# leonavery/KSFD

Measured on AMD Instinct MI355X. Metric: grid-point-updates/sec (implicit step), higher is better.
Workload: dtype f64

## Files before the change

ksfd_amd/csrc/handle.hip.h:

```cpp
#pragma once
#include "spectral_plan.h"
enum { KC_RHS = 0, KC_JVP, KC_MULTIDOT, KC_GSUPDATE, KC_LINCOMB, KC_BASISAXPY, KC_FINISH, KC_REDUCE,
       KC_GFIELD, KC_VELOCITY, KC_MISC, KC_HALO, KC_MG, KC_SPECTRAL };
static const char *kc_names[KSFD_NKCLASS] = { "rhs", "jvp", "multidot", "gs_update", "lincomb", "basis_axpy",
                                              "rosw_finish", "reduce", "gfield", "velocity", "misc", "halo", "mg", "spectral" };
extern "C" const char *ksfd_kernel_class_name(int32_t c) { return (c >= 0 && c < KSFD_NKCLASS) ? kc_names[c] : "?"; }

static thread_local std::string g_create_error;

struct EvPair { hipEvent_t a, b; int cls; };

template <typename T>
struct MGVecs { T *x = nullptr, *b = nullptr, *r = nullptr, *d = nullptr; };

struct MGLevel {
    KGeom G;
    KPhys P;
    KVec kv;
    int64_t vlen = 0;
    int nblk = 1;
    double *coef = nullptr;
    float *dinv = nullptr;
    MGVecs<double> v64;
    MGVecs<float> v32;
    template <typename T> MGVecs<T> &vecs() { if constexpr (std::is_same<T, float>::value) return v32; else return v64; }
    double *Ad = nullptr, *dG = nullptr;
    float *coef32 = nullptr;
    bool f32 = false;
    bool rep = false;
    double *pv = nullptr;
    double pv_norm = 0.0;
    double lam_max = 2.3;
    double ratio = 60.0;
};

struct SpecState {
    bool ok = false, means_valid = false;
    SpecShape shape;
    kcf *W = nullptr, *W2 = nullptr, *twx = nullptr, *twy = nullptr, *twz = nullptr;
    int *spos = nullptr, *skof = nullptr;
    int2 *ytab = nullptr;
    int4 *pairtab = nullptr;
    float *lx = nullptr, *ly = nullptr, *lz = nullptr;
    decltype(&k_spec_rows_fwd<double>) k_rows_fwd64 = nullptr;
    decltype(&k_spec_rows_fwd<float>) k_rows_fwd32 = nullptr;
    decltype(&k_spec_rows_inv) k_rows_inv = nullptr;
    decltype(&k_spec_cols<0>) k_cols = nullptr;
    decltype(&k_spec_cols_split<false>) k_cols_split = nullptr;
    decltype(&k_spec3_y_fwd<false>) k_y_fwd = nullptr;
    decltype(&k_spec3_y_inv<false>) k_y_inv = nullptr;
    decltype(&k_spec3_z<0, false>) k_z = nullptr;
    std::vector<A2APiece> a2a_fwd_s, a2a_fwd_r, a2a_back_s, a2a_back_r;
    double a_rr = 0.0, a_rU[KSFD_MAXL] = { 0 };
    bool user_off = false;
};

struct LUState {
    int64_t n = 0, nnz = 0;
    double *A = nullptr;
    int *piv = nullptr, *perm = nullptr, *info = nullptr;
    long long *col = nullptr;
    double *val = nullptr;
    double *y = nullptr, *z = nullptr;
    std::vector<int> piv_h, perm_h;
    bool valid = false;
    double shift = 0.0;
};

struct MGCoarse {
    int kind = 0;
    int max_unknowns = 0;
    int level = -1;
    LUState lu;
    double *inv = nullptr;
    bool ready = false;
    int info_h = 0;
    int32_t factorizations = 0, solves = 0, fallbacks = 0;
    int32_t graph_solves = 0;
};

struct BandState {
    BandPlan B = {};
    int64_t nnz = 0;
    double *AB = nullptr;
    int *piv = nullptr, *info = nullptr;
    long long *col = nullptr;
    double *val = nullptr;
    double *z = nullptr;
    int threads = 0;
    bool valid = false;
    double shift = 0.0;
};

struct ksfd_handle {
    ksfd_config cfg;
    int32_t lig_group[KSFD_MAXL];
    double lig_w[KSFD_MAXL], lig_s[KSFD_MAXL], lig_gamma[KSFD_MAXL], lig_D[KSFD_MAXL];
    double grp_alpha[KSFD_MAXL], grp_beta[KSFD_MAXL];
    KGeom G;
    KPhys P;
    KPhys Pst[4];
    bool Pst_valid[4] = { false, false, false, false };
    KVec kv;
    int rank = 0, size = 1, device = 0;
    bool ring = false;
    int64_t slow0 = 0;
    hipStream_t st = nullptr;
    hipStream_t st_comm = nullptr;
    hipEvent_t ev_ready = nullptr, ev_halo = nullptr;
    bool overlap = true;
    Transport *tr = nullptr;
    std::string err;

    int64_t vlen = 0;
    double *u = nullptr, *usave = nullptr, *Z = nullptr, *bvec = nullptr, *Y = nullptr, *V = nullptr;
    double *t1 = nullptr, *t2 = nullptr, *t3 = nullptr, *errv = nullptr;
    double *ckpt = nullptr;
    double *bstore = nullptr;
    bool spec_guess = true;
    int guess_max = getenv("KSFD_GUESS_MAX") ? std::max(1, std::min(atoi(getenv("KSFD_GUESS_MAX")), 3)) : 2;
    bool spec_predict = true;
    long long n_predicted = 0;
    long long n_residual = 0;
    long long n_host_sync = 0;
    SpecState spec;
    ksfd_ctl::StepMemo memo, ckpt_memo;
    double spec_from = 0.1;
    bool ckpt_valid = false;
    double *Gb = nullptr, *dGb = nullptr;
    double *coef = nullptr;
    bool use_frozen = true;
    bool coef_fresh = false;
    double *flat = nullptr;
    double *src[4][KSFD_MAXL + 1];
    double *part = nullptr;
    double *dres = nullptr;
    double *hres = nullptr;
    double *hres_dev = nullptr;
    unsigned long long *pub_flag = nullptr, *pub_flag_dev = nullptr, pub_seq = 0;
    unsigned int *pub_count = nullptr;
    bool zero_copy = true;
    int restart_alloc = 0;
    bool restart_grow = true;
    int nblk_vec = 0;
    bool have_err = false;

    int use_fused = 1;
    int yseg = 48;
    int yseg_jvp = 16;
    int zseg = 32;

    bool profiling = false;
    int prof_only = -1;
    std::vector<EvPair> pending;
    std::vector<hipEvent_t> pool;
    ksfd_profile prof;
    double bytes_acc = 0.0;

    double *gm_dev = nullptr;
    double *gm_host = nullptr;
    std::vector<hipEvent_t> gm_ev;
    int async_mode = 0;

    double *Zb = nullptr;
    double *pvec = nullptr;
    int poly_deg = 0;
    double poly_alpha[8];
    double poly_shift = -1.0;
    int poly_max_deg = 6;
    double mg_threshold = 75.0;
    double poly_target = 0.02;
    float *coef32 = nullptr;
    bool rhs_carry = true;
    bool fuse_stage = true;
    bool j3l_attr_set = false, j3l_usable = false;
    bool rhs3d_strip = true;
    bool poly_fp32 = true;

    hipStream_t st_io = nullptr;
    double *snap_dev[2] = { nullptr, nullptr }, *snap_host[2] = { nullptr, nullptr };
    hipEvent_t snap_ready[2] = { nullptr, nullptr }, snap_done[2] = { nullptr, nullptr };
    bool snap_busy[2] = { false, false };
    int snap_next = 0;

    struct RecSpace { bool valid = false; int vb = 0, zb = 0, k = 0, pc = 0; std::vector<double> H; };
    RecSpace rec[4];
    int rec_vtop = 0, rec_ztop = 0;
    int rec_mode = 1;
    int rec_keep = 3;
    bool rhs_dots = true;
    bool rec_mg = false;

    int dr_keep = 0;
    bool dr_carry = false;
    double *dr_P = nullptr, *dr_Phost = nullptr;
    struct DrKept { bool valid = false; int kk = 0, pc = -1; double shift = 0.0, shift_pc = 0.0; std::vector<double> H; };
    DrKept dr;
    ksfd_deflation_stats dr_stats = {};

    LUState lu;
    BandState band;
    MGCoarse mgc;

    std::vector<MGLevel> mg;
    bool sf_auto = true;
    bool mg_fp32 = true;
    bool mg_use32 = false;
    bool mg_graph_f32 = false;
    bool mg_warm_power = true;
    bool mg_fuse = true;
    bool mg_ok = false;
    double mg_shift = -1.0;
    bool mg_coef_valid = false;
    int64_t mg_agg = 0;
    hipGraphExec_t mg_graph = nullptr;
    double mg_graph_shift = -1.0, mg_graph_bytes = 0.0;
    const void *mg_graph_x = nullptr;
    bool capturing = false, mg_use_graph = true;
    int mg_nu = 2, mg_ncoarse = 400, mg_power_its = 8;
    double mg_ratio = 6.0, mg_coarse_tol = 0.3;

    double At[4][4], Ginv[4][4], bt[4], b2t[4], asum[4];
};

#define GAMMA_RA 4.3586652150845900e-01

static int fail(ksfd_handle *h, int code, const char *fmt, ...)
{
    char buf[512];
    va_list ap;
    va_start(ap, fmt);
    vsnprintf(buf, sizeof buf, fmt, ap);
    va_end(ap);
    if (h) h->err = buf; else g_create_error = buf;
    return code;
}
#define HIPCHK(h, call)                                                                                   \
    do {                                                                                                  \
        hipError_t e_ = (call);                                                                           \
        if (e_ != hipSuccess) return fail(h, KSFD_EHIP, "%s failed: %s (%s:%d)", #call, hipGetErrorString(e_), __FILE__, __LINE__); \
    } while (0)

static hipEvent_t ev_get(ksfd_handle *h)
{
    if (!h->pool.empty()) { hipEvent_t e = h->pool.back(); h->pool.pop_back(); return e; }
    hipEvent_t e;
    hipEventCreate(&e);
    return e;
}
struct Scope {
    ksfd_handle *h; EvPair p; bool on;
    Scope(ksfd_handle *h_, int cls, double bytes, double alg = -1.0) : h(h_), on(h_->profiling && !h_->capturing && (h_->prof_only < 0 || h_->prof_only == cls))
    {
        h->bytes_acc += bytes;
        h->prof.bytes[cls] += bytes;
        h->prof.alg_bytes[cls] += alg < 0.0 ? bytes : alg;
        h->prof.launches[cls] += 1;
        if (on) { p.a = ev_get(h); p.b = ev_get(h); p.cls = cls; hipEventRecord(p.a, h->st); }
    }
    ~Scope() { if (on) { hipEventRecord(p.b, h->st); h->pending.push_back(p); } }
};
static void prof_resolve(ksfd_handle *h)
{
    if (h->pending.empty()) return;
    hipStreamSynchronize(h->st);
    for (auto &p : h->pending) {
        float ms = 0.f;
        if (hipEventElapsedTime(&ms, p.a, p.b) == hipSuccess) h->prof.ms[p.cls] += ms;
        h->pool.push_back(p.a);
        h->pool.push_back(p.b);
    }
    h->pending.clear();
}

static inline dim3 vgrid(const ksfd_handle *h) { return dim3(h->nblk_vec, h->G.F); }
static inline double vbytes(const ksfd_handle *h, double nvec) { return nvec * 8.0 * (double)h->G.F * (double)h->G.nloc; }

static void build_tableau(ksfd_handle *h)
{
    static const double A[4][4] = { { 0, 0, 0, 0 }, { 8.7173304301691801e-01, 0, 0, 0 },
                                    { 8.4457060015369423e-01, -1.1299064236484185e-01, 0, 0 }, { 0, 0, 1., 0 } };
    static const double Gm[4][4] = { { GAMMA_RA, 0, 0, 0 }, { -8.7173304301691801e-01, GAMMA_RA, 0, 0 },
                                     { -9.0338057013044082e-01, 5.4180672388095326e-02, GAMMA_RA, 0 },
                                     { 2.4212380706095346e-01, -1.2232505839045147e+00, 5.4526025533510214e-01, GAMMA_RA } };
    static const double b[4] = { 2.4212380706095346e-01, -1.2232505839045147e+00, 1.5452602553351020e+00, GAMMA_RA };
// ... 61 lines not shown
```

ksfd_amd/csrc/krylov.hip.h:

```cpp
#pragma once
#include "krylov_small.h"
static int est_lambda_max(ksfd_handle *h, double shift, int nits)
{
    int rc;
    if (!h->pvec) {
        if (alloc_d(h, &h->pvec, h->vlen)) return KSFD_ENOMEM;
        const int nb = blocks_for(h->vlen);
        hipLaunchKernelGGL(k_hash_fill, dim3(nb), dim3(KSFD_BLOCK), 0, h->st, (long long)h->vlen, h->pvec);
        if ((rc = op_multidot(h, h->pvec, h->pvec, 0))) return rc;
        const double n0 = sqrt(h->hres[0]);
        const double *xs[1] = { h->pvec }; double a[1] = { 1.0 / n0 };
        if ((rc = op_lincomb(h, 1, xs, a, h->pvec))) return rc;
    }
    double lamA = 0.0;
    for (int it = 0; it < nits; it++) {
        if ((rc = op_jvp_frozen_halo(h, h->pvec, 1, shift, h->t3))) return rc;
        if ((rc = op_multidot(h, h->t3, h->t3, 0))) return rc;
        lamA = sqrt(h->hres[0]);
        if (!(lamA > 0.0) || lamA != lamA) return fail(h, KSFD_ENAN, "power iteration on the Jacobian broke down");
        const double *xs[1] = { h->t3 }; double a[1] = { 1.0 / lamA };
        if ((rc = op_lincomb(h, 1, xs, a, h->pvec))) return rc;
    }
    const double est = lamA - shift;
    h->memo.lamJ = est > 0.0 ? est : 0.0;
    return KSFD_OK;
}

static void poly_setup(ksfd_handle *h, double shift)
{
    h->poly_shift = shift;
    h->poly_deg = ksfd_krylov::cheb_setup(h->memo.lamJ, shift, h->poly_target, h->poly_max_deg, h->poly_alpha);
}

static int poly_apply(ksfd_handle *h, double shift, double *v, double *z)
{
    int rc;
    const int d = h->poly_deg;
    const double *al = h->poly_alpha;
    if (h->poly_fp32 && h->coef32 && fused_ok(h)) {
        const float *C = h->coef32;
        float *tf[2] = { reinterpret_cast<float *>(h->t1), reinterpret_cast<float *>(h->t2) };
        const double *nod = nullptr;
        if (d == 1) return jvp2d_halo_t<float, double, double, double>(h, C, v, 4, shift, z, nod, al[0], al[1] / shift);
        if ((rc = jvp2d_halo_t<float, double, double, float>(h, C, v, 4, shift, tf[0], nod, al[d - 1], al[d] / shift))) return rc;
        int cur32 = 0;
        for (int i = d - 2; i >= 1; i--) {
            if ((rc = jvp2d_halo_t<float, float, double, float>(h, C, tf[cur32], 3, shift, tf[cur32 ^ 1], (const double *)v, al[i], 1.0 / shift))) return rc;
            cur32 ^= 1;
        }
        return jvp2d_halo_t<float, float, double, double>(h, C, tf[cur32], 3, shift, z, (const double *)v, al[0], 1.0 / shift);
    }
    double *tmp[2] = { h->t1, h->t2 };
    double *cur = (d == 1) ? z : tmp[0];
    if ((rc = op_jvp_frozen_halo(h, v, 4, shift, cur, nullptr, al[d - 1], al[d] / shift))) return rc;
    int flip = 1;
    for (int i = d - 2; i >= 0; i--) {
        double *nxt = (i == 0) ? z : tmp[flip];
        if ((rc = op_jvp_frozen_halo(h, cur, 3, shift, nxt, v, al[i], 1.0 / shift))) return rc;
        cur = nxt;
        flip ^= 1;
    }
    return KSFD_OK;
}

struct LinStats { int its; double rel; };

static void rec_reset(ksfd_handle *h)
{
    for (auto &r : h->rec) r.valid = false;
    h->rec_vtop = h->rec_ztop = 0;
}

static int rhs_empty(ksfd_handle *h, double bn, double *x, const char *nan_msg, bool *empty)
{
    *empty = !(bn > 0.0);
    if (!*empty) return KSFD_OK;
    if (bn != bn) return fail(h, KSFD_ENAN, "%s", nan_msg);
    HIPCHK(h, hipMemsetAsync(x, 0, sizeof(double) * (size_t)h->vlen, h->st));
    return KSFD_OK;
}

static int apply_AMinv(ksfd_handle *h, const double *ustate, double shift, double shift_pc, int pcmode, double *vj, double *z, double *w)
{
    int rc;
    if (z) {
        if ((rc = pcmode == 1 ? mg_precond(h, shift_pc, vj, z) : pcmode == 3 ? spec_apply(h, shift, vj, z) : poly_apply(h, shift, vj, z))) return rc;
        return op_jvp_frozen_halo(h, z, 1, shift, w);
    }
    if (h->use_frozen) return op_jvp_frozen_halo(h, vj, 1, shift, w);
    return (rc = halo(h, vj)) ? rc : op_jvp(h, ustate, vj, 1, shift, w);
}

static int cgs2_second_pass(ksfd_handle *h, double *w, const double *V, int k, double *hcol, double *d, double *hn)
{
    int rc;
    if ((rc = op_multidot(h, w, V, k))) return rc;
    double s2 = 0.0;
    for (int i = 0; i < k; i++) { d[i] = h->hres[i]; hcol[i] += d[i]; s2 += d[i] * d[i]; }
    double hn2 = h->hres[k] - s2;
    if (hn2 < 0.0) hn2 = 0.0;
    *hn = sqrt(hn2);
    return op_gs_update(h, w, V, k, d, *hn > 0.0 ? 1.0 / *hn : 0.0);
}

static int cgs2_classic(ksfd_handle *h, double *w, const double *V, int k, double *hcol, double *d, double *hn)
{
    int rc;
    for (int i = 0; i < k; i++) hcol[i] = h->hres[i];
    if ((rc = op_gs_update(h, w, V, k, hcol, 1.0))) return rc;
    return cgs2_second_pass(h, w, V, k, hcol, d, hn);
}

static int cgs2_gram(ksfd_handle *h, double *w, const double *V, int j, double *Gm, int ldg, double *hcol, double *d, double *hn)
{
    int rc;
    const int k = j + 1;
    if ((rc = op_multidot_gram(h, w, V, k))) return rc;
    for (int i = 0; i < k; i++) { d[i] = h->hres[i]; Gm[(size_t)i * ldg + j] = Gm[(size_t)j * ldg + i] = h->hres[k + i]; }
    const double ww = h->hres[2 * k];
    if (!(ww == ww)) return fail(h, KSFD_ENAN, "GMRES: Krylov vector is not finite");
    double hn2;
    if (ksfd_krylov::cgs2_algebraic(Gm, ldg, k, d, ww, hcol, &hn2)) {
        *hn = sqrt(hn2);
        return op_gs_update(h, w, V, k, hcol, 1.0 / *hn);
    }
    if ((rc = op_gs_update(h, w, V, k, hcol, 1.0))) return rc;
    return cgs2_second_pass(h, w, V, k, hcol, d, hn);
}

struct GmresRun {
    int pcmode, stage;
    bool use_pc, use_poly;
    bool rec_on, rec_full;
    double shift_pc;
    int vb, zb;
    double *V, *Zq;
    std::vector<int> spaces;
    std::vector<double> g_first;
    double bn, beta;
    const double *rsrc;
    bool x_set = false;
    bool x0_pending = false;
    std::vector<double> xcoef;
};

static int rhs_norm(ksfd_handle *h, GmresRun &R, const double *b)
{
    int rc;
    if (R.rec_on && R.stage > 0)
        for (int q = 0; q < R.stage; q++)
            if (ksfd_krylov::recycle_uses(R.stage, q, h->rec_mode, R.rec_full) && h->rec[q].valid && h->rec[q].pc == R.pcmode) R.spaces.push_back(q);
    if (R.spaces.empty()) {
        if ((rc = op_multidot(h, b, R.V, 0))) return rc;
        R.bn = sqrt(h->hres[0]);
        return KSFD_OK;
    }
    const ksfd_handle::RecSpace &S = h->rec[R.spaces.front()];
    if ((rc = op_multidot(h, b, h->V + (int64_t)S.vb * h->vlen, S.k + 1))) return rc;
    R.g_first.assign(h->hres, h->hres + S.k + 2);
    R.bn = sqrt(R.g_first[S.k + 1]);
    return KSFD_OK;
}

static int recycle_project(ksfd_handle *h, GmresRun &R, const double *b, double *x)
{
    if (R.spaces.empty()) return KSFD_OK;
    int rc;
    const int64_t vs = h->vlen;
    const bool defer_x0 = !R.use_pc;
    bool pc_x0_pending = false;
    double *const rbuf = (x == h->t3) ? R.V : h->t3;
    const int first_space = R.spaces.front(), last_space = R.spaces.back();
    bool have_norm = false;
    for (int q : R.spaces) {
        const ksfd_handle::RecSpace &S = h->rec[q];
        const double *Vs = h->V + (int64_t)S.vb * vs;
        const double *Zs = R.use_poly ? h->Zb + (int64_t)S.zb * vs : Vs;
        std::vector<double> gq_((size_t)S.k + 2), yq_((size_t)S.k + 1), Hy_((size_t)S.k + 2), neg_((size_t)S.k + 2);
        double *gq = gq_.data(), *yq = yq_.data(), *Hy = Hy_.data(), *neg = neg_.data();
        if (q == first_space && R.rsrc == b) {
            for (int i = 0; i <= S.k; i++) gq[i] = R.g_first[i];
        } else {
            if ((rc = op_multidot(h, R.rsrc, Vs, S.k + 1))) return rc;
            for (int i = 0; i <= S.k; i++) gq[i] = h->hres[i];
        }
        ksfd_krylov::hess_lsq(S.H.data(), S.k, gq, yq, Hy);
        if (R.use_pc) {
            if ((rc = op_basis_axpy(h, h->t2, Vs, S.k, yq, pc_x0_pending ? 1.0 : 0.0))) return rc;
            pc_x0_pending = true;
        } else if (defer_x0) {
            for (int i = 0; i < S.k; i++) R.xcoef[(R.use_poly ? S.zb : S.vb) + i] += yq[i];
// ... 339 lines not shown
```

ksfd_amd/csrc/ksfd_hip.hip:

```cpp
#include <hip/hip_runtime.h>
#include <dlfcn.h>
#include <math.h>
#include <stdarg.h>
#include <stdio.h>
#include <stdlib.h>
#include <string.h>
#include <string>
#include <vector>

#include "../../include/ksfd_hip.h"
#include "stencil.hip.h"
#include "mg.hip.h"
#include "spectral.hip.h"
#include "lu.hip.h"
#include "banded.hip.h"
#include "transport.h"
#include "step_control.h"
#include "mg_coarse_plan.h"
#include "mg_agglomerate_plan.h"

#include "handle.hip.h"
#include "ops.hip.h"
#include "spectral_host.hip.h"
#include "mg_host.hip.h"
// ... 43 lines not shown
}

extern "C" int ksfd_create(const ksfd_config *cfg, const ksfd_dist *dist, ksfd_handle **out)
{
    if (!cfg || !out) return fail(nullptr, KSFD_EINVAL, "null argument");
    *out = nullptr;
    if (cfg->dim < 1 || cfg->dim > 3) return fail(nullptr, KSFD_EINVAL, "dim must be 1, 2 or 3");
    for (int a = 0; a < cfg->dim; a++)
        if (cfg->n[a] < 5) return fail(nullptr, KSFD_EINVAL, "n[%d]=%lld < 5: the width-2 periodic star needs >= 5 points", a, (long long)cfg->n[a]);
    ksfd_handle *h = new ksfd_handle();
    memset(h->src, 0, sizeof h->src);
    memset(&h->prof, 0, sizeof h->prof);
    h->cfg = *cfg;
    h->cfg.lig_group = nullptr; h->cfg.lig_w = h->cfg.lig_s = h->cfg.lig_gamma = h->cfg.lig_D = nullptr;
    h->cfg.grp_alpha = h->cfg.grp_beta = nullptr;
    int rc = fill_phys(h, cfg);
    if (rc) { g_create_error = h->err; delete h; return rc; }
    h->rank = dist ? dist->rank : 0;
    h->size = dist ? dist->size : 1;
    h->device = dist ? dist->device : 0;
    if (h->size < 1 || h->rank < 0 || h->rank >= h->size) { delete h; return fail(nullptr, KSFD_EINVAL, "bad rank/size"); }
    h->ring = h->size > 1 || (dist && dist->transport != 0);
    int ndev = 0;
    if (hipGetDeviceCount(&ndev) != hipSuccess || ndev < 1) { delete h; return fail(nullptr, KSFD_EHIP, "no HIP device available (libksfd_hip has no CPU path)"); }
    if (h->device < 0 || h->device >= ndev) { delete h; return fail(nullptr, KSFD_EINVAL, "device %d of %d", h->device, ndev); }
#define CFAIL(code, ...) do { int rc_ = fail(nullptr, code, __VA_ARGS__); ksfd_destroy(h); return rc_; } while (0)
    if (hipSetDevice(h->device) != hipSuccess) CFAIL(KSFD_EHIP, "hipSetDevice(%d) failed", h->device);
    if (hipStreamCreateWithFlags(&h->st, hipStreamNonBlocking) != hipSuccess) CFAIL(KSFD_EHIP, "hipStreamCreate failed");
    if (h->ring && (hipStreamCreateWithFlags(&h->st_comm, hipStreamNonBlocking) != hipSuccess ||
                        hipEventCreateWithFlags(&h->ev_ready, hipEventDisableTiming) != hipSuccess ||
                        hipEventCreateWithFlags(&h->ev_halo, hipEventDisableTiming) != hipSuccess)) CFAIL(KSFD_EHIP, "comm stream/event creation failed");

    KGeom &G = h->G;
    G.dim = cfg->dim; G.F = cfg->nlig + 1;
    const int slow = cfg->dim - 1;
    int64_t nglob = cfg->n[slow];
    if (h->size > 1 && (nglob % h->size != 0 || nglob / h->size < 4))
        CFAIL(KSFD_EINVAL, "slab axis extent %lld must be divisible by %d ranks with >= 4 units each", (long long)nglob, h->size);
    int64_t sloc = nglob / h->size;
    h->slow0 = sloc * h->rank;
    G.ng = h->ring ? 2 : 0;
    G.wrap_slow = !h->ring;
    G.nx = cfg->n[0]; G.ny = cfg->dim >= 2 ? cfg->n[1] : 1; G.nz = cfg->dim >= 3 ? cfg->n[2] : 1;
    if (slow == 0) G.nx = sloc; else if (slow == 1) G.ny = sloc; else G.nz = sloc;
    G.inner = slow == 0 ? 1 : (slow == 1 ? G.nx : G.nx * G.ny);
    G.sloc = sloc;
    G.plane = (sloc + 2 * G.ng) * G.inner;
    G.nloc = sloc * G.inner;
    h->kv.plane = G.plane; h->kv.off = (long long)G.ng * G.inner; h->kv.nloc = G.nloc; h->kv.nf = G.F;
    h->vlen = (int64_t)G.F * G.plane;
    h->nblk_vec = (int)std::min<long long>((G.nloc + KSFD_BLOCK - 1) / KSFD_BLOCK, 2048);
    build_tableau(h);

    h->restart_alloc = ksfd_krylov::RESTART_DEFAULT;
    int fit_local = ksfd_krylov::RESTART_DEFAULT;
    {
        size_t mfree = 0, mtotal = 0;
        if (hipMemGetInfo(&mfree, &mtotal) == hipSuccess && mfree > 0) {
            static const int cap = getenv("KSFD_RESTART_MAX") ? ksfd_krylov::restart_cap(atoi(getenv("KSFD_RESTART_MAX"))) : ksfd_krylov::RESTART_MAX;
            fit_local = ksfd_krylov::restart_fit((double)mfree, 8.0 * (double)h->vlen, cap);
        }
    }
    if (alloc_d(h, &h->dres, 128)) CFAIL(KSFD_ENOMEM, "%s", h->err.c_str());
    if (h->ring) {
        std::string terr;
        h->tr = make_transport(dist, G.F, G.inner, terr);
        if (!h->tr) CFAIL(KSFD_ECOMM, "transport %d: %s", dist->transport, terr.c_str());
        double v = -(double)fit_local;
        if (hipMemcpyAsync(h->dres, &v, sizeof v, hipMemcpyHostToDevice, h->st) != hipSuccess || h->tr->allreduce(h->dres, 1, 1, h->st))
            CFAIL(KSFD_ECOMM, "agreeing on the restart length failed: %s", h->tr->error().c_str());
        if (h->tr->result_on_host()) v = h->tr->host_result()[0];
        else if (hipMemcpyAsync(&v, h->dres, sizeof v, hipMemcpyDeviceToHost, h->st) != hipSuccess || hipStreamSynchronize(h->st) != hipSuccess)
            CFAIL(KSFD_EHIP, "reading the agreed restart length failed");
        fit_local = (int)(-v + 0.5);
    }
    if (fit_local != ksfd_krylov::RESTART_DEFAULT) {
        if (fit_local < ksfd_krylov::RESTART_MIN) CFAIL(KSFD_ENOMEM, "grid too large for this device: a vector is %.2f GB, the solver needs ~47 of them (restart length that fits: %d)", 8.0 * (double)h->vlen / 1e9, fit_local);
        h->restart_alloc = fit_local;
    }
    double **vecs[] = { &h->u, &h->usave, &h->Z, &h->bvec, &h->t1, &h->t2, &h->t3, &h->errv };
    for (double **v : vecs) {
        if (alloc_d(h, v, h->vlen)) CFAIL(KSFD_ENOMEM, "%s", h->err.c_str());
        hipMemsetAsync(*v, 0, sizeof(double) * (size_t)h->vlen, h->st);
    }
    if (alloc_d(h, &h->Y, 4 * h->vlen) || alloc_d(h, &h->V, (int64_t)(h->restart_alloc + 1) * h->vlen) ||
        alloc_d(h, &h->Gb, G.plane) || alloc_d(h, &h->dGb, G.plane) || alloc_d(h, &h->coef, (int64_t)(3 + cfg->nlig) * G.plane) ||
        alloc_d(h, &h->flat, (int64_t)std::max(G.F, 3) * G.nloc) ||
        alloc_d(h, &h->part, (int64_t)(2 * KSFD_MAXDOT + 4) * 4096))
        CFAIL(KSFD_ENOMEM, "%s", h->err.c_str());
    if (hipMalloc((void **)&h->Zb, sizeof(double) * (size_t)h->restart_alloc * (size_t)h->vlen) != hipSuccess) { h->Zb = nullptr; hipGetLastError(); }
    hipMemsetAsync(h->Y, 0, sizeof(double) * (size_t)(4 * h->vlen), h->st);
    hipMemsetAsync(h->V, 0, sizeof(double) * (size_t)((h->restart_alloc + 1) * h->vlen), h->st);
    if (hipHostMalloc((void **)&h->hres, sizeof(double) * 128 + 64, hipHostMallocMapped | hipHostMallocCoherent) != hipSuccess) CFAIL(KSFD_ENOMEM, "hipHostMalloc failed");
    h->pub_flag = reinterpret_cast<unsigned long long *>(h->hres + 128);
    *h->pub_flag = 0;
    if (hipHostGetDevicePointer((void **)&h->hres_dev, h->hres, 0) != hipSuccess || hipMalloc((void **)&h->pub_count, sizeof(unsigned int)) != hipSuccess ||
        hipMemset(h->pub_count, 0, sizeof(unsigned int)) != hipSuccess) { h->zero_copy = false; h->hres_dev = nullptr; }
    else h->pub_flag_dev = reinterpret_cast<unsigned long long *>(h->hres_dev + 128);
    {
        const int m = h->restart_alloc;
        const size_t ndev = (size_t)(m + 1) * (m + 1) + (size_t)(m + 1) * m + 2 * m + (m + 1) + KSFD_MAXDOT + 1 + 2 * (m + 1);
        const size_t nhost = 2 * (m + 1) + (size_t)(m + 1) * m + (m + 1);
        if (alloc_d(h, &h->gm_dev, (int64_t)ndev)) CFAIL(KSFD_ENOMEM, "%s", h->err.c_str());
        if (hipHostMalloc((void **)&h->gm_host, sizeof(double) * nhost, hipHostMallocDefault) != hipSuccess) CFAIL(KSFD_ENOMEM, "hipHostMalloc failed");
        h->gm_ev.resize(m + 1);
        for (auto &e : h->gm_ev) if (hipEventCreateWithFlags(&e, hipEventDisableTiming) != hipSuccess) CFAIL(KSFD_EHIP, "hipEventCreate failed");
    }

    spec_build(h);
    if (mg_build(h)) { mg_free(h); h->mg_ok = false; }
    if ((h->spec.ok || h->mg_ok) && alloc_d(h, &h->bstore, 3 * h->vlen)) { h->bstore = nullptr; h->spec_guess = false; h->err.clear(); }
    if (h->ring) {
        double flags[3] = { h->spec.ok ? 1.0 : 0.0, h->mg_ok ? 1.0 : 0.0, (h->spec_guess && h->bstore) ? 1.0 : 0.0 };
        for (double &f : flags) f = -f;
        if (hipMemcpyAsync(h->dres, flags, sizeof flags, hipMemcpyHostToDevice, h->st) != hipSuccess || h->tr->allreduce(h->dres, 3, 1, h->st))
            CFAIL(KSFD_ECOMM, "agreeing on the available solvers failed: %s", h->tr->error().c_str());
        if (h->tr->result_on_host()) memcpy(flags, h->tr->host_result(), sizeof flags);
        else if (hipMemcpyAsync(flags, h->dres, sizeof flags, hipMemcpyDeviceToHost, h->st) != hipSuccess || hipStreamSynchronize(h->st) != hipSuccess)
            CFAIL(KSFD_EHIP, "reading the agreed solver flags failed");
        if (flags[0] > -0.5 && h->spec.ok) spec_free(h);
        if (flags[1] > -0.5 && h->mg_ok) { mg_free(h); h->mg_ok = false; }
        if (flags[2] > -0.5) h->spec_guess = false;
    }
    if (hipStreamSynchronize(h->st) != hipSuccess) CFAIL(KSFD_EHIP, "stream sync failed in create");
#undef CFAIL
    *out = h;
    return KSFD_OK;
}

extern "C" int ksfd_rccl_unique_id(void *out128)
{
    if (!out128) return KSFD_EINVAL;
    std::string err;
    RcclApi api;
    if (!api.load(err)) return fail(nullptr, KSFD_ECOMM, "%s", err.c_str());
    auto getid = (decltype(&ncclGetUniqueId))dlsym(api.lib, "ncclGetUniqueId");
    if (!getid) return fail(nullptr, KSFD_ECOMM, "librccl lacks ncclGetUniqueId");
    ncclUniqueId id;
    ncclResult_t r = getid(&id);
    if (r != ncclSuccess) return fail(nullptr, KSFD_ECOMM, "ncclGetUniqueId: %s", api.GetErrorString(r));
    memcpy(out128, &id, sizeof id);
    return KSFD_OK;
}

extern "C" int ksfd_update_params(ksfd_handle *h, const ksfd_config *cfg)
{
    if (!h || !cfg) return KSFD_EINVAL;
    if (cfg->dim != h->cfg.dim || cfg->nlig != h->cfg.nlig) return fail(h, KSFD_EINVAL, "update_params cannot change dim/nlig");
    for (int a = 0; a < 3; a++) if (cfg->n[a] != h->cfg.n[a]) return fail(h, KSFD_EINVAL, "update_params cannot change the grid");
    h->cfg = *cfg;
    h->cfg.lig_group = nullptr; h->cfg.lig_w = h->cfg.lig_s = h->cfg.lig_gamma = h->cfg.lig_D = nullptr;
    h->cfg.grp_alpha = h->cfg.grp_beta = nullptr;
    h->coef_fresh = false;
    return fill_phys(h, cfg);
}

extern "C" int ksfd_set_stage_params(ksfd_handle *h, int32_t stage, const ksfd_config *cfg)
{
    if (!h || stage < -1 || stage > 3) return KSFD_EINVAL;
    if (!cfg) {
        for (int s = 0; s < 4; s++) if (stage == -1 || s == stage) h->Pst_valid[s] = false;
        return KSFD_OK;
    }
    if (cfg->dim != h->cfg.dim || cfg->nlig != h->cfg.nlig) return fail(h, KSFD_EINVAL, "set_stage_params cannot change dim/nlig");
    for (int a = 0; a < 3; a++) if (cfg->n[a] != h->cfg.n[a] || cfg->L[a] != h->cfg.L[a]) return fail(h, KSFD_EINVAL, "set_stage_params cannot change the grid");
    for (int s = 0; s < 4; s++) {
        if (stage != -1 && s != stage) continue;
        int rc = fill_phys(h, cfg, &h->Pst[s]);
        if (rc) return rc;
        h->Pst_valid[s] = true;
    }
    return KSFD_OK;
}

extern "C" int ksfd_local_range(const ksfd_handle *h, int64_t *b, int64_t *e)
{
    if (!h) return KSFD_EINVAL;
    if (b) *b = h->slow0;
    if (e) *e = h->slow0 + h->G.sloc;
    return KSFD_OK;
}
extern "C" int64_t ksfd_local_size(const ksfd_handle *h) { return h ? (int64_t)h->G.F * h->G.nloc : 0; }
extern "C" double *ksfd_device_state(ksfd_handle *h) { return h ? h->u : nullptr; }
extern "C" int64_t ksfd_device_plane_stride(const ksfd_handle *h) { return h ? h->G.plane : 0; }
extern "C" int64_t ksfd_device_interior_offset(const ksfd_handle *h) { return h ? (int64_t)h->G.ng * h->G.inner : 0; }

extern "C" int ksfd_set_state(ksfd_handle *h, const double *u, int32_t layout)
{
    if (!h || !u) return KSFD_EINVAL;
    hipSetDevice(h->device);
    int rc = upload(h, u, layout, h->u);
    h->coef_fresh = false;
    if (rc) return rc;
    HIPCHK(h, hipStreamSynchronize(h->st));
    return KSFD_OK;
}
extern "C" int ksfd_snapshot_begin(ksfd_handle *h, int32_t layout, int32_t *slot)
{
    if (!h || !slot) return KSFD_EINVAL;
    if (layout < 0 || layout > 2) return fail(h, KSFD_EINVAL, "bad layout %d", layout);
    hipSetDevice(h->device);
    const KGeom &G = h->G;
    const size_t bytes = sizeof(double) * (size_t)G.F * G.nloc;
    if (!h->st_io) {
        if (hipStreamCreateWithFlags(&h->st_io, hipStreamNonBlocking) != hipSuccess) return fail(h, KSFD_EHIP, "hipStreamCreate (io) failed");
        for (int q = 0; q < 2; q++) {
            if (hipMalloc((void **)&h->snap_dev[q], bytes) != hipSuccess || hipHostMalloc((void **)&h->snap_host[q], bytes, hipHostMallocDefault) != hipSuccess)
                return fail(h, KSFD_ENOMEM, "snapshot staging buffers (%zu bytes each) could not be allocated", bytes);
            if (hipEventCreateWithFlags(&h->snap_ready[q], hipEventDisableTiming) != hipSuccess ||
                hipEventCreateWithFlags(&h->snap_done[q], hipEventDisableTiming) != hipSuccess) return fail(h, KSFD_EHIP, "hipEventCreate failed");
        }
    }
    const int q = h->snap_next;
    h->snap_next ^= 1;
    if (h->snap_busy[q]) HIPCHK(h, hipEventSynchronize(h->snap_done[q]));
    {
        Scope sc(h, KC_MISC, vbytes(h, 2));
        hipLaunchKernelGGL(k_to_host_layout, vgrid(h), dim3(KSFD_BLOCK), 0, h->st, G, layout, (const double *)h->u, G.plane,
                           (long long)G.ng * G.inner, h->snap_dev[q]);
    }
    HIPCHK(h, hipGetLastError());
    HIPCHK(h, hipEventRecord(h->snap_ready[q], h->st));
    HIPCHK(h, hipStreamWaitEvent(h->st_io, h->snap_ready[q], 0));
    HIPCHK(h, hipMemcpyAsync(h->snap_host[q], h->snap_dev[q], bytes, hipMemcpyDeviceToHost, h->st_io));
    HIPCHK(h, hipEventRecord(h->snap_done[q], h->st_io));
    h->snap_busy[q] = true;
    *slot = q;
    return KSFD_OK;
}

extern "C" int ksfd_snapshot_wait(ksfd_handle *h, int32_t slot, const double **host)
{
    if (!h || !host || slot < 0 || slot > 1) return KSFD_EINVAL;
    if (!h->snap_busy[slot]) return fail(h, KSFD_EINVAL, "snapshot slot %d holds nothing", slot);
    hipSetDevice(h->device);
    HIPCHK(h, hipEventSynchronize(h->snap_done[slot]));
    *host = h->snap_host[slot];
    return KSFD_OK;
}

extern "C" int ksfd_checkpoint(ksfd_handle *h, int32_t op)
{
    if (!h || op < 0 || op > 1) return KSFD_EINVAL;
    hipSetDevice(h->device);
    h->dr.valid = false;
    if (op == 0) {
        if (!h->ckpt && alloc_d(h, &h->ckpt, h->vlen)) return KSFD_ENOMEM;
        HIPCHK(h, hipMemcpyAsync(h->ckpt, h->u, sizeof(double) * (size_t)h->vlen, hipMemcpyDeviceToDevice, h->st));
        h->ckpt_memo = h->memo;
        for (MGLevel &L : h->mg) L.pv_norm = 0.0;
        h->ckpt_valid = true;
        return KSFD_OK;
    }
    if (!h->ckpt_valid) return fail(h, KSFD_EINVAL, "no checkpoint has been saved");
    HIPCHK(h, hipMemcpyAsync(h->u, h->ckpt, sizeof(double) * (size_t)h->vlen, hipMemcpyDeviceToDevice, h->st));
    h->coef_fresh = false;
    h->memo = h->ckpt_memo;
    h->spec.means_valid = false;
    h->mg_coef_valid = false; h->mg_shift = -1.0; h->poly_shift = -1.0; h->have_err = false;
    for (MGLevel &L : h->mg) L.pv_norm = 0.0;
    rec_reset(h);
    return KSFD_OK;
}

extern "C" int ksfd_set_state_random(ksfd_handle *h, const int64_t *nc, const double *z, double rho0)
{
    if (!h || !nc || !z) return KSFD_EINVAL;
    hipSetDevice(h->device);
    int64_t n = 1;
    for (int a = 0; a < 3; a++) {
        if (a < h->G.dim ? nc[a] < 1 : nc[a] != 1) return fail(h, KSFD_EINVAL, "coarse grid must be >= 1 per used axis and 1 elsewhere");
        n *= nc[a];
    }
    double *dz = nullptr;
    h->coef_fresh = false;
    if (hipMalloc((void **)&dz, sizeof(double) * (size_t)n) != hipSuccess) return fail(h, KSFD_ENOMEM, "hipMalloc of the coarse samples failed");
    hipError_t e = hipMemcpyAsync(dz, z, sizeof(double) * (size_t)n, hipMemcpyHostToDevice, h->st);
    const KGeom &G = h->G;
    int nb = (int)std::min<long long>((G.nloc + KSFD_BLOCK - 1) / KSFD_BLOCK, 65535);
    if (e == hipSuccess) {
        Scope sc(h, KC_MISC, vbytes(h, 1));
        NL_DISPATCH(h->P.nlig, hipLaunchKernelGGL((k_random_start<NL>), dim3(nb), dim3(KSFD_BLOCK), 0, h->st, G, h->P, (long long)h->cfg.n[G.dim - 1],
                                                  (long long)h->slow0, (long long)nc[0], (long long)nc[1], (long long)nc[2], (const double *)dz, rho0, h->u));
        e = hipGetLastError();
    }
    if (e == hipSuccess) e = hipStreamSynchronize(h->st);
    hipFree(dz);
    if (e != hipSuccess) return fail(h, KSFD_EHIP, "random start: %s", hipGetErrorString(e));
    return KSFD_OK;
}
extern "C" int ksfd_get_state(ksfd_handle *h, double *u, int32_t layout)
{
    if (!h || !u) return KSFD_EINVAL;
    hipSetDevice(h->device);
    return download(h, h->u, layout, u);
}

extern "C" int ksfd_set_source(ksfd_handle *h, int32_t stage, int32_t field, const double *srch, int32_t layout)
{
    if (!h || field < 0 || field >= h->G.F || stage < -1 || stage > 3) return h ? fail(h, KSFD_EINVAL, "bad stage/field") : KSFD_EINVAL;
    if (layout != KSFD_LAYOUT_SOA) return fail(h, KSFD_EINVAL, "sources are single dense planes: pass layout SOA");
    hipSetDevice(h->device);
    for (int s = 0; s < 4; s++) {
        if (stage != -1 && s != stage) continue;
        if (!srch) {
            if (h->src[s][field]) { HIPCHK(h, hipStreamSynchronize(h->st)); hipFree(h->src[s][field]); h->src[s][field] = nullptr; }
            continue;
        }
        if (!h->src[s][field] && alloc_d(h, &h->src[s][field], h->G.nloc)) return KSFD_ENOMEM;
        HIPCHK(h, hipMemcpyAsync(h->src[s][field], srch, sizeof(double) * (size_t)h->G.nloc, hipMemcpyHostToDevice, h->st));
    }
    HIPCHK(h, hipStreamSynchronize(h->st));
    return KSFD_OK;
}

extern "C" int ksfd_rhs(ksfd_handle *h, double t, const double *uh, double *outh, int32_t layout)
{
    (void)t;
    if (!h || !outh) return KSFD_EINVAL;
    hipSetDevice(h->device);
    int rc;
    double *uin = h->u;
    if (uh) { if ((rc = upload(h, uh, layout, h->t1))) return rc; uin = h->t1; }
    if ((rc = halo(h, uin))) return rc;
    if ((rc = op_rhs(h, uin, 0, h->t3))) return rc;
    return download(h, h->t3, layout, outh);
}

extern "C" int ksfd_jvp(ksfd_handle *h, const double *uh, const double *vh, double *outh, int32_t layout)
{
    if (!h || !vh || !outh) return KSFD_EINVAL;
    hipSetDevice(h->device);
    int rc;
    double *uin = h->u;
    if (uh) { if ((rc = upload(h, uh, layout, h->t1))) return rc; uin = h->t1; }
    if ((rc = upload(h, vh, layout, h->t2))) return rc;
    if ((rc = halo(h, uin)) || (rc = halo(h, h->t2))) return rc;
    if (!uh && h->use_frozen) {
        if ((rc = ensure_coef(h, true))) return rc;
        if ((rc = op_jvp_frozen(h, h->t2, 0, 0.0, h->t3))) return rc;
    } else if ((rc = op_jvp(h, uin, h->t2, 0, 0.0, h->t3))) return rc;
    return download(h, h->t3, layout, outh);
}

static int velocity_common(ksfd_handle *h, const double *uin, double *vel_dev, double vmax[3])
{
    const KGeom &G = h->G;
    int rc;
    const double *Gplane = h->Gb;
    if (uin == h->u && h->use_frozen) {
        if ((rc = ensure_coef(h))) return rc;
        Gplane = h->coef + G.plane;
    } else {
        if ((rc = halo(h, (double *)uin))) return rc;
        Scope sc(h, KC_GFIELD, 8.0 * (G.F + 1) * (double)G.plane);
        NL_DISPATCH(h->P.nlig, hipLaunchKernelGGL((k_gfield<NL, false>), dim3(plane_blocks(G)), dim3(KSFD_BLOCK), 0, h->st, G, h->P, uin, (const double *)nullptr, h->Gb, (double *)nullptr));
    }
    int nb = (int)std::min<long long>((G.nloc + KSFD_BLOCK - 1) / KSFD_BLOCK, 1024);
    if (vmax && !vel_dev && G.dim == 2 && (G.nx % 2 == 0) && G.nx >= 4) {
        const int bx = (int)((G.nx / 2 + KSFD_BLOCK - 1) / KSFD_BLOCK), by = (int)std::min<long long>(G.sloc, std::max(1, 2048 / bx));
        nb = bx * by;
        Scope sc(h, KC_VELOCITY, 8.0 * (double)G.nloc);
        hipLaunchKernelGGL(k_velmax2d, dim3(bx, by), dim3(KSFD_BLOCK), 0, h->st, G, h->P, Gplane, h->part);
    } else if (vmax && !vel_dev && G.dim == 3 && (G.nx % 2 == 0) && G.nx >= 4 && G.ny >= 4 && G.nx * G.ny < (1LL << 30)) {
        const int bx = (int)((G.nx / 2 * G.ny + KSFD_BLOCK - 1) / KSFD_BLOCK);
        int zseg = (int)G.sloc;
        while (zseg >= 32 && (long long)bx * ((G.sloc + zseg - 1) / zseg) < 8192) zseg = (zseg + 1) / 2;
        const int by = (int)((G.sloc + zseg - 1) / zseg);
        nb = bx * by;
        if (3LL * nb > part_capacity()) return fail(h, KSFD_EINVAL, "velocity_max: grid too large for the partial-result buffer");
        Scope sc(h, KC_VELOCITY, 8.0 * (double)G.nloc);
        hipLaunchKernelGGL(k_velmax3d, dim3(bx, by), dim3(KSFD_BLOCK), 0, h->st, G, h->P, zseg, Gplane, h->part);
    } else {
        Scope sc(h, KC_VELOCITY, 8.0 * (double)G.nloc * (1 + (vel_dev ? G.dim : 0)));
        hipLaunchKernelGGL(k_velocity, dim3(nb), dim3(KSFD_BLOCK), 0, h->st, G, h->P, Gplane, vel_dev, vmax ? h->part : (double *)nullptr);
    }
    HIPCHK(h, hipGetLastError());
    if (vmax) {
        if ((rc = reduce_rows(h, 3, nb, 1))) return rc;
        for (int a = 0; a < 3; a++) vmax[a] = a < G.dim ? h->hres[a] : 0.0;
    }
    return KSFD_OK;
}

extern "C" int ksfd_velocity(ksfd_handle *h, const double *uh, double *velh, int32_t layout)
{
    if (!h || !velh) return KSFD_EINVAL;
    if (layout != KSFD_LAYOUT_SOA) return fail(h, KSFD_EINVAL, "velocity output is dim dense SoA planes: pass layout SOA for it");
    hipSetDevice(h->device);
    int rc;
    double *uin = h->u;
    if (uh) { if ((rc = upload(h, uh, layout, h->t1))) return rc; uin = h->t1; }
    if ((rc = velocity_common(h, uin, h->flat, nullptr))) return rc;
    HIPCHK(h, hipMemcpyAsync(velh, h->flat, sizeof(double) * (size_t)h->G.dim * h->G.nloc, hipMemcpyDeviceToHost, h->st));
    HIPCHK(h, hipStreamSynchronize(h->st));
    return KSFD_OK;
}

extern "C" int ksfd_velocity_max(ksfd_handle *h, double vmax[3])
{
    if (!h || !vmax) return KSFD_EINVAL;
    hipSetDevice(h->device);
    return velocity_common(h, h->u, nullptr, vmax);
}

extern "C" int ksfd_groom(ksfd_handle *h)
{
    if (!h) return KSFD_EINVAL;
    hipSetDevice(h->device);
    Scope sc(h, KC_MISC, vbytes(h, 2));
    hipLaunchKernelGGL(k_groom, vgrid(h), dim3(KSFD_BLOCK), 0, h->st, h->kv, h->u, h->P.rhomin, h->P.Umin);
    HIPCHK(h, hipGetLastError());
    return KSFD_OK;
}

extern "C" int ksfd_count_worms(ksfd_handle *h, double *total)
{
    if (!h || !total) return KSFD_EINVAL;
    hipSetDevice(h->device);
    {
        Scope sc(h, KC_MISC, 8.0 * (double)h->G.nloc);
        hipLaunchKernelGGL(k_sum_rho, dim3(h->nblk_vec), dim3(KSFD_BLOCK), 0, h->st, h->kv, h->u, h->part);
    }
    HIPCHK(h, hipGetLastError());
    int rc = reduce_rows(h, 1, h->nblk_vec, 0);
    if (rc) return rc;
    *total = h->hres[0];
    return KSFD_OK;
}

extern "C" int ksfd_scale_rho(ksfd_handle *h, double factor)
{
    if (!h) return KSFD_EINVAL;
    hipSetDevice(h->device);
    h->coef_fresh = false;
    Scope sc(h, KC_MISC, 16.0 * (double)h->G.nloc);
    hipLaunchKernelGGL(k_mul_rho, dim3(h->nblk_vec), dim3(KSFD_BLOCK), 0, h->st, h->kv, h->u, (const double *)nullptr, factor);
    HIPCHK(h, hipGetLastError());
    return KSFD_OK;
}

extern "C" int ksfd_mul_rho(ksfd_handle *h, const double *fh)
{
    if (!h || !fh) return KSFD_EINVAL;
    hipSetDevice(h->device);
    HIPCHK(h, hipMemcpyAsync(h->flat, fh, sizeof(double) * (size_t)h->G.nloc, hipMemcpyHostToDevice, h->st));
    h->coef_fresh = false;
    Scope sc(h, KC_MISC, 24.0 * (double)h->G.nloc);
    hipLaunchKernelGGL(k_mul_rho, dim3(h->nblk_vec), dim3(KSFD_BLOCK), 0, h->st, h->kv, h->u, (const double *)h->flat, 1.0);
    HIPCHK(h, hipGetLastError());
    HIPCHK(h, hipStreamSynchronize(h->st));
    return KSFD_OK;
}

extern "C" int ksfd_jacobian_nnz(ksfd_handle *h, int64_t *nrows, int64_t *nnz)
{
    if (!h) return KSFD_EINVAL;
    const int64_t npts = 4 * h->G.dim + 1;
    if (nrows) *nrows = (int64_t)h->G.F * h->G.nloc;
    if (nnz) *nnz = h->G.nloc * ((int64_t)h->G.F * npts + (int64_t)h->P.nlig * (npts + 1));
    return KSFD_OK;
}

extern "C" int ksfd_jacobian_csr(ksfd_handle *h, int64_t *rowptr, int64_t *col, double *val)
{
    if (!h || !rowptr || !col || !val) return KSFD_EINVAL;
    hipSetDevice(h->device);
    int64_t nrows, nnz;
    ksfd_jacobian_nnz(h, &nrows, &nnz);
    int rc;
    if ((rc = ensure_coef(h))) return rc;
    long long *dcol = nullptr;
    double *dval = nullptr;
    if (hipMalloc((void **)&dcol, sizeof(long long) * (size_t)nnz) != hipSuccess ||
        hipMalloc((void **)&dval, sizeof(double) * (size_t)nnz) != hipSuccess) {
        if (dcol) hipFree(dcol);
        return fail(h, KSFD_ENOMEM, "hipMalloc of the CSR staging buffers failed");
    }
    const KGeom &G = h->G;
    int nb = (int)std::min<long long>((G.nloc + KSFD_BLOCK - 1) / KSFD_BLOCK, 65535);
    {
        Scope sc(h, KC_MISC, 16.0 * (double)nnz + 8.0 * (3 + h->P.nlig) * (double)G.nloc);
        NL_DISPATCH(h->P.nlig, hipLaunchKernelGGL((k_jac_csr<NL>), dim3(nb), dim3(KSFD_BLOCK), 0, h->st, G, h->P, (const double *)h->coef,
                                                  (long long)h->cfg.n[G.dim - 1], (long long)h->slow0, dcol, dval));
    }
    hipError_t e = hipGetLastError();
    if (e == hipSuccess) e = hipMemcpyAsync(col, dcol, sizeof(long long) * (size_t)nnz, hipMemcpyDeviceToHost, h->st);
    if (e == hipSuccess) e = hipMemcpyAsync(val, dval, sizeof(double) * (size_t)nnz, hipMemcpyDeviceToHost, h->st);
    if (e == hipSuccess) e = hipStreamSynchronize(h->st);
    hipFree(dcol);
    hipFree(dval);
    if (e != hipSuccess) return fail(h, KSFD_EHIP, "jacobian export: %s", hipGetErrorString(e));
    const int64_t npts = 4 * G.dim + 1, F = G.F, per = F * npts + (F - 1) * (npts + 1);
    for (int64_t p = 0; p < G.nloc; p++) {
        rowptr[p * F] = p * per;
        for (int64_t l = 1; l < F; l++) rowptr[p * F + l] = p * per + F * npts + (l - 1) * (npts + 1);
    }
    rowptr[nrows] = nnz;
    return KSFD_OK;
}


extern "C" void ksfd_default_step_opts(ksfd_step_opts *o)
{
    memset(o, 0, sizeof *o);
    o->rtol = 1e-5; o->atol = 1e-5;
    o->adapt = 1; o->max_reject = 10;
    o->clip_lo = 0.1; o->clip_hi = 5.0;
    o->dt_min = 1e-20; o->dt_max = 1e4;
    o->safety = 0.9; o->reject_safety = 0.5;
    o->ksp_rtol = 1e-6; o->ksp_atol = 1e-50;
    o->ksp_restart = 30; o->ksp_max_it = 2000;
    o->pc_type = 2;
}

static int step_run(ksfd_handle *h, double *t, double *hstep, const ksfd_step_opts *opts, bool direct, bool dr_on, ksfd_step_stats &st)
{
    int rc;
    StepMemo &m = h->memo;
    double hh = *hstep;
    bool prev_accept = !(opts->reserved & 4);
    bool lam_done = false;
    int rejects = 0;
    const int max_rej = opts->max_reject < 0 ? 0x7fffffff : opts->max_reject;
    const bool single = (opts->reserved & 2) != 0;
    {
        Scope sc(h, KC_MISC, vbytes(h, 3));
        hipLaunchKernelGGL(k_groom, vgrid(h), dim3(KSFD_BLOCK), 0, h->st, h->kv, h->u, h->P.rhomin, h->P.Umin, h->usave);
        if (hipGetLastError() != hipSuccess) return fail(h, KSFD_EHIP, "k_groom launch failed");
    }
    if ((rc = halo(h, h->u))) return rc;
    if (h->use_frozen && (rc = ensure_coef(h, true))) return rc;
    h->poly_shift = -1.0;
    m.nsteps++;
    ksfd_ctl::spec_rho_roll(m);
    while (true) {
        AttemptPlan p;
        if ((rc = plan_attempt(h, opts, hh, direct, dr_on, lam_done, p))) return rc;
        const int its_before = st.linear_its;
        bool spec_failed = false;
        rc = step_attempt(h, opts, p, spec_failed, st);
        const int its = st.linear_its - its_before;
        if (p.use_spec && opts->pc_type == 2) ksfd_ctl::spec_backoff_update(m, spec_failed, its, m.nsteps);
        if (!rc && p.use_pc && h->sf_auto) ksfd_ctl::shift_floor_update(m, (double)its, p.shift);
        if (rc == KSFD_ELINEAR && opts->adapt && !single && rejects < max_rej && hh * 0.25 >= opts->dt_min) {
            rejects++;
            st.rejections = rejects;
            prev_accept = false;
            if ((rc = op_copy(h, h->u, h->usave))) return rc;
            hh *= 0.25;
            *hstep = hh;
            if ((rc = halo(h, h->u))) return rc;
            continue;
        }
        if (rc) { op_copy(h, h->u, h->usave); hipStreamSynchronize(h->st); return rc; }
        if ((rc = step_finish(h, opts, &st.wrms))) return rc;
        if (!(st.wrms == st.wrms) || isinf(st.wrms)) {
            op_copy(h, h->u, h->usave); hipStreamSynchronize(h->st);
            h->coef_fresh = h->use_frozen;
            return fail(h, KSFD_ENAN, "non-finite error norm at t=%g h=%g", *t, hh);
        }
        ksfd_ctl::AdaptChoice next = { true, hh };
        if (opts->adapt) next = ksfd_ctl::adapt_basic(hh, st.wrms, prev_accept, opts->safety, opts->reject_safety, opts->clip_lo, opts->clip_hi, opts->dt_min, opts->dt_max);
        prev_accept = next.accept;
        if (next.accept) {
            st.accepted = 1; st.h_used = hh;
            *t += hh;
            *hstep = next.hnext;
            return KSFD_OK;
        }
        rejects++;
        st.rejections = rejects;
        if ((rc = op_copy(h, h->u, h->usave))) return rc;
        h->coef_fresh = h->use_frozen;
        hh = next.hnext;
        *hstep = next.hnext;
        if (single) return KSFD_OK;
        if (rejects > max_rej) return fail(h, KSFD_EREJECT, "step rejected %d times at t=%g", rejects, *t);
        if ((rc = halo(h, h->u))) return rc;
    }
}

extern "C" int ksfd_step(ksfd_handle *h, double *t, double *hstep, const ksfd_step_opts *opts, ksfd_step_stats *stats)
{
    if (!h || !t || !hstep || !opts) return KSFD_EINVAL;
    hipSetDevice(h->device);
    const bool direct = opts->pc_type == 5 || opts->pc_type == 6;
    if (direct) {
        const int g = opts->pc_type == 6 ? banded_guard(h) : direct_guard(h);
        if (g) return g;
    }
    const bool dr_on = h->dr_keep > 0 && !direct;
    if (dr_on) {
        const int m_dr = std::min(opts->ksp_restart > 0 ? opts->ksp_restart : 30, h->restart_alloc);
        if (h->dr_keep > m_dr - 3) return fail(h, KSFD_EINVAL, "deflation: keep = %d needs a restart length of at least %d (ksp_restart %d, basis vectors allocated %d)", h->dr_keep, h->dr_keep + 3, (int)opts->ksp_restart, h->restart_alloc);
    }
    memset(&h->dr_stats, 0, sizeof h->dr_stats);
    if (getenv("KSFD_PC_SIGMA")) { h->memo.mg_shift_floor = atof(getenv("KSFD_PC_SIGMA")); h->sf_auto = false; }
    ksfd_step_stats st;
    memset(&st, 0, sizeof st);
    const StepCounters c0 = stats_begin(h);
    const int32_t coarse0 = h->mgc.solves;
    const int rc = step_run(h, t, hstep, opts, direct, dr_on, st);
    stats_end(h, c0, st);
    if (h->mgc.solves != coarse0) st.pc_used |= 64;
    if (stats) *stats = st;
    return rc;
}

extern "C" int ksfd_get_last_error_vector(ksfd_handle *h, double *eh, int32_t layout)
{
    if (!h || !eh) return KSFD_EINVAL;
    if (!h->have_err) return fail(h, KSFD_EINVAL, "no step has been attempted yet");
    hipSetDevice(h->device);
    return download(h, h->errv, layout, eh);
}

extern "C" int ksfd_set_profiling(ksfd_handle *h, int32_t on)
{
    if (!h) return KSFD_EINVAL;
    prof_resolve(h);
    if (on < 0 || on >= 2 + KSFD_NKCLASS) return KSFD_EINVAL;
    h->profiling = on != 0;
    h->prof_only = on >= 2 ? on - 2 : -1;
    return KSFD_OK;
}
extern "C" int ksfd_get_profile(ksfd_handle *h, ksfd_profile *p, int32_t reset)
{
    if (!h || !p) return KSFD_EINVAL;
    prof_resolve(h);
    *p = h->prof;
    if (reset) memset(&h->prof, 0, sizeof h->prof);
    return KSFD_OK;
}
extern "C" int ksfd_set_mg_params(ksfd_handle *h, int32_t nu, int32_t ncoarse_max, int32_t power_its, double ratio, double coarse_tol)
{
    if (!h) return KSFD_EINVAL;
    if (nu > 0) h->mg_nu = nu;
    if (ncoarse_max > 0) h->mg_ncoarse = ncoarse_max;
    if (power_its > 0) h->mg_power_its = power_its;
    if (ratio > 1.0) h->mg_ratio = ratio;
    if (coarse_tol > 0.0) h->mg_coarse_tol = coarse_tol;
    h->mg_use_graph = power_its != -7 && !h->ring;
    h->mg_shift = -1.0;
    return KSFD_OK;
}
static int mg_coarse_choice(const ksfd_handle *h, int32_t kind, int32_t max_unknowns)
{
    std::vector<long long> unk;
    for (const MGLevel &L : h->mg) unk.push_back((long long)L.G.F * L.G.nloc);
    return ksfd_ctl::mg_coarse_level(unk.data(), h->mg_ok ? (int)unk.size() : 0, kind, max_unknowns, KSFD_MG_DIRECT_MAX);
}
extern "C" int ksfd_set_mg_coarse(ksfd_handle *h, int32_t kind, int32_t max_unknowns)
{
    if (!h) return KSFD_EINVAL;
    if (kind != 0 && kind != 1) return fail(h, KSFD_EINVAL, "mg_coarse: kind %d is neither 0 (Chebyshev) nor 1 (exact solve)", (int)kind);
    if (kind == 1) {
        if (h->ring) return fail(h, KSFD_EINVAL, "mg_coarse: the exact coarse solve is single rank only (this handle has a halo transport)");
        if (!h->mg_ok) return fail(h, KSFD_EINVAL, "mg_coarse: this handle has no multigrid hierarchy");
        if (max_unknowns > KSFD_MG_DIRECT_MAX) return fail(h, KSFD_EINVAL, "mg_coarse: max_unknowns = %d above KSFD_MG_DIRECT_MAX = %d", (int)max_unknowns, KSFD_MG_DIRECT_MAX);
    } else if (!h->mg_ok) return KSFD_OK;
    const int level = mg_coarse_choice(h, kind, max_unknowns);
    if (level < 0) {
        const MGLevel &Lc = h->mg.back();
        return fail(h, KSFD_EINVAL, "mg_coarse: no level below level 0 has at most %d unknowns (the coarsest of %d levels has %lld)",
                    max_unknowns > 0 ? (int)max_unknowns : KSFD_MG_DIRECT_MAX, (int)h->mg.size(), (long long)Lc.G.F * Lc.G.nloc);
    }
    hipSetDevice(h->device);
    if (kind == 1) { int rc = mgc_alloc(h, level); if (rc) return rc; }
    if (kind == h->mgc.kind && level == h->mgc.level) { h->mgc.max_unknowns = kind == 1 ? max_unknowns : 0; return KSFD_OK; }
    h->mgc.kind = kind; h->mgc.level = level; h->mgc.max_unknowns = kind == 1 ? max_unknowns : 0;
    h->mgc.ready = false;
    h->mg_shift = -1.0;
    if (h->mg_graph) { HIPCHK(h, hipStreamSynchronize(h->st)); hipGraphExecDestroy(h->mg_graph); h->mg_graph = nullptr; }
    return KSFD_OK;
}
extern "C" int ksfd_set_mg_agglomerate(ksfd_handle *h, int64_t max_points)
{
    if (!h) return KSFD_EINVAL;
    if (max_points < 0) return fail(h, KSFD_EINVAL, "mg_agglomerate: max_points = %lld is negative", (long long)max_points);
    if (!h->ring) return KSFD_OK;
    if (h->G.dim == 1) return fail(h, KSFD_EINVAL, "mg_agglomerate: 2-D and 3-D slabs only (this handle is 1-D)");
    if (!h->mg_ok) return fail(h, KSFD_EINVAL, "mg_agglomerate: this handle has no multigrid hierarchy");
    hipSetDevice(h->device);
    HIPCHK(h, hipStreamSynchronize(h->st));
    const int64_t before = h->mg_agg;
    int own_rc = KSFD_OK;
    std::string own_err;
    bool failed = false;
    auto rebuild = [&](int64_t agg) -> int {
        mg_free(h);
        h->mg_agg = agg;
        h->mg_coef_valid = false; h->mg_shift = -1.0; h->mg_graph_shift = -1.0;
        h->dr.valid = false;
        own_rc = mg_build(h);
        own_err = h->err;
        if (!own_rc && !h->mg_ok) own_rc = fail(h, KSFD_EINVAL, "mg_agglomerate: the rebuilt hierarchy has fewer than two levels"), own_err = h->err;
        double bad = own_rc ? 1.0 : 0.0;
        if (hipMemcpyAsync(h->dres, &bad, sizeof bad, hipMemcpyHostToDevice, h->st) != hipSuccess || h->tr->allreduce(h->dres, 1, 1, h->st))
            return fail(h, KSFD_ECOMM, "mg_agglomerate: agreeing on the hierarchy failed: %s", h->tr->error().c_str());
        if (h->tr->result_on_host()) bad = h->tr->host_result()[0];
        else if (hipMemcpyAsync(&bad, h->dres, sizeof bad, hipMemcpyDeviceToHost, h->st) != hipSuccess || hipStreamSynchronize(h->st) != hipSuccess)
            return fail(h, KSFD_EHIP, "mg_agglomerate: reading the agreed outcome failed");
        HIPCHK(h, hipStreamSynchronize(h->st));
        failed = bad > 0.5;
        return KSFD_OK;
    };
    int rc = rebuild(max_points);
    if (rc || !failed) return rc;
    const int why_rc = own_rc;
    const std::string why = own_err;
    if (rebuild(before) != KSFD_OK || failed) { mg_free(h); h->mg_agg = 0; }
    if (why_rc) { h->err = why; return why_rc; }
    return fail(h, KSFD_ENOMEM, "mg_agglomerate: another rank could not build the hierarchy with max_points = %lld", (long long)max_points);
}
extern "C" int ksfd_get_mg_coarse_info(ksfd_handle *h, ksfd_mg_coarse_info *info)
{
    if (!h || !info) return KSFD_EINVAL;
    memset(info, 0, sizeof *info);
    if (!h->mg_ok) return fail(h, KSFD_EINVAL, "mg_coarse: this handle has no multigrid hierarchy");
    const MGLevel &L = h->mg[mg_end(h)];
    info->kind = h->mgc.kind; info->level = (int32_t)mg_end(h); info->nlevels = (int32_t)h->mg.size(); info->F = L.G.F;
    info->n[0] = L.G.nx; info->n[1] = L.G.dim >= 2 ? L.G.ny : 1; info->n[2] = L.G.dim >= 3 ? L.G.nz : 1;
    info->unknowns = (int64_t)L.G.F * L.G.nloc;
    info->factorizations = h->mgc.factorizations; info->solves = h->mgc.solves; info->fallbacks = h->mgc.fallbacks;
    return KSFD_OK;
}
extern "C" int ksfd_mg_coarse_apply(ksfd_handle *h, double shift, int32_t op, const double *vh, double *outh)
{
    if (!h || !vh || !outh) return KSFD_EINVAL;
    if (!isfinite(shift)) return fail(h, KSFD_EINVAL, "mg_coarse_apply: non-finite shift");
    if (op != 0 && op != 1) return fail(h, KSFD_EINVAL, "mg_coarse_apply: op %d is neither 0 (operator) nor 1 (solve)", (int)op);
    if (!h->mg_ok) return fail(h, KSFD_EINVAL, "mg_coarse: this handle has no multigrid hierarchy");
    if (op == 1 && h->mgc.kind != 1) return fail(h, KSFD_EINVAL, "mg_coarse_apply: op 1 needs ksfd_set_mg_coarse(kind 1)");
    if (h->ring) return fail(h, KSFD_EINVAL, "mg_coarse_apply: single rank only (this handle has a halo transport)");
    hipSetDevice(h->device);
    int rc;
    if ((rc = ensure_coef(h))) return rc;
    if (!h->mg_coef_valid && (rc = mg_restrict_coefs(h))) return rc;
    MGLevel &L = h->mg[mg_end(h)];
    double *const lb = L.v64.b, *const lx = L.v64.x;
    const size_t nb = sizeof(double) * (size_t)L.G.nloc;
    for (int f = 0; f < L.G.F; f++)
        HIPCHK(h, hipMemcpyAsync(lb + (int64_t)f * L.G.plane + L.kv.off, vh + (int64_t)f * L.G.nloc, nb, hipMemcpyHostToDevice, h->st));
    if (op == 0) rc = mg_op<double>(h, L, lb, 1, shift, lx, nullptr);
    else {
        bool ok = false;
        h->mg_shift = -1.0;
        if ((rc = mgc_setup(h, L, shift, &ok))) return rc;
        if (!ok) return fail(h, KSFD_ELINEAR, "coarse solve: zero or non-finite pivot in column %d of shift*I - J_c (shift %.6g, %lld unknowns)", h->mgc.info_h - 1, shift, (long long)h->mgc.lu.n);
        rc = mgc_apply(h, L, lb, lx);
        h->mgc.ready = false;
    }
    if (rc) return rc;
    for (int f = 0; f < L.G.F; f++)
        HIPCHK(h, hipMemcpyAsync(outh + (int64_t)f * L.G.nloc, lx + (int64_t)f * L.G.plane + L.kv.off, nb, hipMemcpyDeviceToHost, h->st));
    HIPCHK(h, hipStreamSynchronize(h->st));
    return KSFD_OK;
}
template <typename T>
static int mgp_put(ksfd_handle *h, const MGLevel &L, int np, const double *host, T *dev)
{
    HIPCHK(h, hipMemsetAsync(dev, 0, sizeof(T) * (size_t)np * L.G.plane, h->st));
    std::vector<T> tmp((size_t)np * L.G.nloc);
    for (size_t i = 0; i < tmp.size(); i++) tmp[i] = (T)host[i];
    for (int f = 0; f < np; f++)
        HIPCHK(h, hipMemcpyAsync(dev + (int64_t)f * L.G.plane + L.kv.off, tmp.data() + (int64_t)f * L.G.nloc, sizeof(T) * (size_t)L.G.nloc, hipMemcpyHostToDevice, h->st));
    HIPCHK(h, hipStreamSynchronize(h->st));
    return KSFD_OK;
}
template <typename T>
static int mgp_get(ksfd_handle *h, const MGLevel &L, int np, const T *dev, double *host)
{
    std::vector<T> tmp((size_t)np * L.G.nloc);
    for (int f = 0; f < np; f++)
        HIPCHK(h, hipMemcpyAsync(tmp.data() + (int64_t)f * L.G.nloc, dev + (int64_t)f * L.G.plane + L.kv.off, sizeof(T) * (size_t)L.G.nloc, hipMemcpyDeviceToHost, h->st));
    HIPCHK(h, hipStreamSynchronize(h->st));
    for (size_t i = 0; i < tmp.size(); i++) host[i] = (double)tmp[i];
    return KSFD_OK;
}
static int mgp_begin(ksfd_handle *h, bool setup, double shift)
{
    int rc;
    if ((rc = ensure_coef(h))) return rc;
    if (!h->mg_coef_valid && (rc = mg_restrict_coefs(h))) return rc;
    if (setup) {
        for (MGLevel &L : h->mg) L.pv_norm = 0.0;
        h->mg_shift = -1.0;
        if ((rc = mg_setup_shift(h, shift))) return rc;
    }
    return KSFD_OK;
}
static void mgp_end(ksfd_handle *h)
{
    hipStreamSynchronize(h->st);
    h->mg_shift = -1.0;
    h->mg_graph_shift = -1.0;
    if (h->mg_graph) { hipGraphExecDestroy(h->mg_graph); h->mg_graph = nullptr; }
    for (MGLevel &L : h->mg) L.pv_norm = 0.0;
    h->mgc.ready = false;
}
static bool mgp_smoothed(const ksfd_handle *h, size_t l) { return l <= mg_end(h) && !(l == mg_end(h) && h->mgc.kind == 1 && h->mgc.ready); }

extern "C" int ksfd_mg_level_info(ksfd_handle *h, int32_t level, int32_t setup, double shift, ksfd_mg_level_info_t *info)
{
    if (!h || !info) return KSFD_EINVAL;
    memset(info, 0, sizeof *info);
    if (!h->mg_ok) return fail(h, KSFD_EINVAL, "mg_part: this handle has no multigrid hierarchy");
    if (level < 0 || level >= (int)h->mg.size()) return fail(h, KSFD_EINVAL, "mg_part: level %d outside 0 .. %d", (int)level, (int)h->mg.size() - 1);
    if (setup && !isfinite(shift)) return fail(h, KSFD_EINVAL, "mg_part: non-finite shift");
    hipSetDevice(h->device);
    const int rc = mgp_begin(h, setup != 0, shift);
    const MGLevel &L = h->mg[level];
    info->level = level; info->nlevels = (int32_t)h->mg.size(); info->F = L.G.F; info->end_level = (int32_t)mg_end(h);
    info->n[0] = L.G.nx; info->n[1] = L.G.dim >= 2 ? L.G.ny : 1; info->n[2] = L.G.dim >= 3 ? L.G.nz : 1;
    info->sloc = L.G.sloc; info->points = L.G.nloc;
    info->path = (int32_t)mg_path(h, L);
    info->f32 = L.f32 ? 1 : 0;
    const JvpSys Y = mg_sys(h, L);
    info->coef32 = (Y.coef32 ? 2 : 0) | ((Y.coef32 && Y.cls == KC_JVP && mg_path(h, L) == JP_STRIP2D) ? 1 : 0);
    info->can_fuse = mg_can_fuse(h, L) ? 1 : 0;
    if (setup && !rc) {
        info->have_setup = mgp_smoothed(h, (size_t)level) ? 1 : 0;
        if (info->have_setup) { info->lam_max = L.lam_max; info->ratio = L.ratio; }
        if ((size_t)level == mg_end(h) && info->have_setup) info->coarse_sweeps = mg_coarse_sweeps(h, L);
    }
    mgp_end(h);
    return rc;
}

extern "C" int ksfd_mg_part(ksfd_handle *h, int32_t part, int32_t level, int32_t variant, int32_t nu, double shift, double ratio,
                            const double *in0, const double *in1, double *out0, double *out1)
{
    if (!h) return KSFD_EINVAL;
    if (!h->mg_ok) return fail(h, KSFD_EINVAL, "mg_part: this handle has no multigrid hierarchy");
    const int nlev = (int)h->mg.size();
    if (level < 0 || level >= nlev) return fail(h, KSFD_EINVAL, "mg_part: level %d outside 0 .. %d", (int)level, nlev - 1);
    if (!isfinite(shift)) return fail(h, KSFD_EINVAL, "mg_part: non-finite shift");
    MGLevel &L = h->mg[level];
    const bool transfer = part == KSFD_MGP_RESTRICT || part == KSFD_MGP_PROLONG_ADD;
    if (transfer && level + 1 >= nlev) return fail(h, KSFD_EINVAL, "mg_part: level %d has no coarser level", (int)level);
    MGLevel &Lc = h->mg[transfer ? level + 1 : level];
    const bool cf32 = transfer && mg_f32(h, (size_t)level + 1);
    const int F = L.G.F, np = 3 + h->P.nlig;
    bool setup = false, ok = true, need1 = false, need_o1 = false;
    switch (part) {
    case KSFD_MGP_COEF: ok = variant == 0; break;
    case KSFD_MGP_RESTRICT: ok = variant == 0 || (variant == 1 && L.f32) || (variant == 2 && L.G.dim == 2 && Lc.f32); break;
    case KSFD_MGP_PROLONG_ADD: ok = variant == 0 || (variant == 1 && L.f32); need1 = true; break;
    case KSFD_MGP_OPERATOR: ok = variant == 1 || variant == 2 || (variant == 32 && L.f32); need1 = variant != 1; break;
    case KSFD_MGP_DINV: ok = variant == 0; setup = true; break;
    case KSFD_MGP_DINV_APPLY: ok = variant == 0 || (variant == 1 && L.f32); setup = true; need_o1 = true; break;
    case KSFD_MGP_SMOOTH: ok = variant == 0; setup = true; break;
    case KSFD_MGP_CYCLE: ok = level == 0 && (variant == 0 || variant == 1); setup = true; break;
    default: return fail(h, KSFD_EINVAL, "mg_part: unknown part %d", (int)part);
    }
    if (!ok) return fail(h, KSFD_EINVAL, "mg_part %d: level %d has no variant %d", (int)part, (int)level, (int)variant);
    if (part == KSFD_MGP_CYCLE && variant == 1 && !mg_cycle32_ok(h))
        return fail(h, KSFD_EINVAL, "mg_part: this handle has no cycle with fp32 level vectors (2-D strip kernel on level 0, nu = 2, fused smoother, tuning bit 19 clear)");
    if (part == KSFD_MGP_SMOOTH && (nu < 1 || nu > 5)) return fail(h, KSFD_EINVAL, "mg_part: nu = %d outside 1 .. 5", (int)nu);
    if (part == KSFD_MGP_SMOOTH && !(ratio > 1.0)) return fail(h, KSFD_EINVAL, "mg_part: smoothing ratio %.6g not above 1", ratio);
    if ((part != KSFD_MGP_COEF && part != KSFD_MGP_DINV && !in0) || (need1 && !in1) || !out0 || (need_o1 && !out1))
        return fail(h, KSFD_EINVAL, "mg_part %d: missing buffer", (int)part);
    if (setup && part != KSFD_MGP_CYCLE && (size_t)level > mg_end(h)) return fail(h, KSFD_EINVAL, "mg_part %d: level %d lies below the level the cycle ends on", (int)part, (int)level);
    hipSetDevice(h->device);
    int rc;
    if ((rc = mgp_begin(h, setup, shift))) { mgp_end(h); return rc; }
    if (setup && part != KSFD_MGP_CYCLE && !mgp_smoothed(h, (size_t)level)) { mgp_end(h); return fail(h, KSFD_EINVAL, "mg_part %d: level %d is solved exactly and has no smoother", (int)part, (int)level); }
    double *const a = L.rep ? L.v64.b : h->t1, *const b = L.rep ? L.v64.x : h->t2, *const c = L.rep ? L.v64.d : h->t3;
    auto run = [&]() -> int {
        int r;
        switch (part) {
        case KSFD_MGP_COEF: {
            if ((r = mgp_get(h, L, np, (const double *)L.coef, out0))) return r;
            const float *c32 = mg_sys(h, L).coef32;
            if (out1 && c32) return mgp_get(h, L, np, c32, out1);
            return KSFD_OK;
        }
        case KSFD_MGP_RESTRICT: {
            auto go = [&](auto *fine, auto *coarse) -> int {
                if ((r = mgp_put(h, L, F, in0, fine)) || (r = mg_halo(h, L, fine, F))) return r;
                if ((r = mg_launch_restrict(h, L, Lc, F, fine, coarse)) || (r = mg_border_reduce(h, L, Lc, F, coarse))) return r;
                return mgp_get(h, Lc, F, coarse, out0);
            };
            if (variant == 0) return Lc.rep ? go(a, Lc.v64.b) : go(a, b);
            if (variant == 2) return go(a, Lc.v32.b);
            return cf32 ? go(L.v32.r, Lc.v32.b) : go(L.v32.r, Lc.v64.b);
        }
        case KSFD_MGP_PROLONG_ADD: {
            auto go = [&](auto *fine, auto *coarse) -> int {
                if ((r = mgp_put(h, L, F, in0, fine)) || (r = mgp_put(h, Lc, F, in1, coarse)) || (r = mg_halo(h, Lc, coarse, F))) return r;
                if ((r = mg_launch_prolong(h, L, Lc, F, coarse, fine))) return r;
                return mgp_get(h, L, F, fine, out0);
            };
            if (variant == 0) return Lc.rep ? go(a, Lc.v64.x) : go(a, b);
            return cf32 ? go(L.v32.x, Lc.v32.x) : go(L.v32.x, Lc.v64.x);
        }
        case KSFD_MGP_OPERATOR: {
            auto go = [&](auto *v, auto *out, auto *y, int mode) -> int {
                if ((r = mgp_put(h, L, F, in0, v)) || (mode == 2 && (r = mgp_put(h, L, F, in1, y)))) return r;
                if ((r = mg_op(h, L, v, mode, shift, out, mode == 2 ? y : nullptr))) return r;
                return mgp_get(h, L, F, out, out0);
            };
            return variant == 32 ? go(L.v32.x, L.v32.r, L.v32.b, 2) : go(a, b, c, variant);
        }
        case KSFD_MGP_DINV: return mgp_get(h, L, F * F, (const float *)L.dinv, out0);
        case KSFD_MGP_DINV_APPLY: {
            const double scale = nu ? (double)nu : 1.0;
            auto go = [&](auto *z, auto *z2, auto *rcopy) -> int {
                if ((r = mgp_put(h, L, F, in0, a))) return r;
                mg_dinv_apply(h, L, 0.0, (const double *)a, 1.0 / scale, z, z2, rcopy);
                if ((r = mgp_get(h, L, F, z, out0)) || (r = mgp_get(h, L, F, z2, out1))) return r;
                return mgp_get(h, L, F, rcopy, out1 + (int64_t)F * L.G.nloc);
            };
            return variant == 0 ? go(b, c, L.Ad) : go(L.v32.d, L.v32.x, L.v32.b);
        }
        case KSFD_MGP_SMOOTH:
            if ((r = mgp_put(h, L, F, in0, a))) return r;
            if (in1) { if ((r = mgp_put(h, L, F, in1, b))) return r; }
            else HIPCHK(h, hipMemsetAsync(b, 0x7f, sizeof(double) * (size_t)L.vlen, h->st));
            if ((r = mg_smooth(h, L, shift, a, b, nu, !in1, ratio))) return r;
            return mgp_get(h, L, F, (const double *)b, out0);
        default: {
            if ((r = mgp_put(h, L, F, in0, a))) return r;
            HIPCHK(h, hipMemsetAsync(b, 0x7f, sizeof(double) * (size_t)L.vlen, h->st));
            const bool was = h->mg_use32;
            h->mg_use32 = variant == 1;
            r = mg_precond(h, shift, a, b);
            h->mg_use32 = was;
            if (r) return r;
            return mgp_get(h, L, F, (const double *)b, out0);
        }
        }
    };
    rc = run();
    if (!rc && hipGetLastError() != hipSuccess) rc = fail(h, KSFD_EHIP, "mg_part %d: launch failed", (int)part);
    mgp_end(h);
// ... 45 lines not shown
}
extern "C" int ksfd_set_deflation(ksfd_handle *h, int32_t keep, int32_t carry_stages)
{
    if (!h) return KSFD_EINVAL;
    if (keep < 0 || keep > 16) return fail(h, KSFD_EINVAL, "deflation: keep = %d outside 0 (off) .. 16", (int)keep);
    h->dr_keep = keep;
    h->dr_carry = carry_stages != 0;
    h->dr.valid = false;
    return KSFD_OK;
}
extern "C" int ksfd_get_deflation_stats(ksfd_handle *h, ksfd_deflation_stats *s)
{
    if (!h || !s) return KSFD_EINVAL;
    *s = h->dr_stats;
    return KSFD_OK;
}
extern "C" int32_t ksfd_basis_capacity(const ksfd_handle *h) { return h ? h->restart_alloc + 1 : 0; }
extern "C" int ksfd_basis_rotate(ksfd_handle *h, int32_t nin, int32_t nout, const double *P, const double *vin, double *vout, int32_t layout)
{
    if (!h || !P || !vin || !vout) return KSFD_EINVAL;
    if (layout < 0 || layout > 2) return fail(h, KSFD_EINVAL, "bad layout %d", layout);
    if (nin < 1 || nout < 1 || nout > nin || nout > KSFD_ROT_MAXOUT || nin > KSFD_ROT_MAXIN || nin > h->restart_alloc + 1)
        return fail(h, KSFD_EINVAL, "basis_rotate: %d -> %d vectors outside 1 <= nout <= %d, nout <= nin <= min(%d, %d)", (int)nin, (int)nout, KSFD_ROT_MAXOUT, KSFD_ROT_MAXIN, h->restart_alloc + 1);
    hipSetDevice(h->device);
    h->dr.valid = false;
    rec_reset(h);
    int rc;
    const int64_t nl = (int64_t)h->G.F * h->G.nloc;
    for (int i = 0; i < nin; i++) {
        if ((rc = upload(h, vin + (int64_t)i * nl, layout, h->V + (int64_t)i * h->vlen))) return rc;
        HIPCHK(h, hipStreamSynchronize(h->st));
    }
    std::vector<double> Pp((size_t)nin * KSFD_ROT_MAXOUT, 0.0);
    for (int i = 0; i < nin; i++) for (int j = 0; j < nout; j++) Pp[(size_t)i * KSFD_ROT_MAXOUT + j] = P[(size_t)i * nout + j];
    if ((rc = op_basis_rotate(h, h->V, nin, nout, Pp.data(), KSFD_ROT_MAXOUT))) return rc;
    for (int i = 0; i < nin; i++)
        if ((rc = download(h, h->V + (int64_t)i * h->vlen, layout, vout + (int64_t)i * nl))) return rc;
    return KSFD_OK;
}
extern "C" int ksfd_krylov_op(ksfd_handle *h, int32_t op, int32_t k, int32_t want_norm, const double *coef, double alpha, double beta,
                              const double *vecs, double *out_vecs, double *scalars, int32_t layout)
{
    if (!h) return KSFD_EINVAL;
    if (layout < 0 || layout > 2) return fail(h, KSFD_EINVAL, "bad layout %d", layout);
    const int cap = h->restart_alloc + 1;
    const int kdev = std::min(KSFD_ASYNC_MAXK, h->restart_alloc);
    int kmin = 1, kmax = 0, nvec = 0, nscal = 0;
    bool need_coef = true;
    switch (op) {
    case KSFD_KOP_LINCOMB: kmax = std::min(6, cap); nvec = k; nscal = want_norm ? 1 : 0; break;
    case KSFD_KOP_MULTIDOT: kmin = 0; kmax = cap - 1; nvec = k + 1; nscal = k + 1; need_coef = false; break;
    case KSFD_KOP_MULTIDOT_GRAM: kmax = std::min(32, cap - 1); nvec = k + 1; nscal = 2 * k + 1; need_coef = false; break;
    case KSFD_KOP_GS_UPDATE: kmax = cap - 1; nvec = k + 1; break;
    case KSFD_KOP_BASIS_AXPY: kmax = cap - 1; nvec = k + 1; nscal = want_norm ? 1 : 0; break;
    case KSFD_KOP_GS_UPDATE_DEV: kmax = kdev; nvec = k + 1; break;
    case KSFD_KOP_GMRES_COEF: kmax = kdev; nvec = 0; nscal = 1; break;
    default: return fail(h, KSFD_EINVAL, "krylov_op: unknown operation %d", (int)op);
    }
    if (k < kmin || k > kmax) return fail(h, KSFD_EINVAL, "krylov_op %d: k = %d outside %d .. %d (basis capacity %d)", (int)op, (int)k, kmin, kmax, cap);
    if ((need_coef && !coef) || (nvec && (!vecs || !out_vecs)) || (nscal && !scalars)) return fail(h, KSFD_EINVAL, "krylov_op %d: missing buffer", (int)op);
    if (want_norm && op != KSFD_KOP_LINCOMB && op != KSFD_KOP_BASIS_AXPY) return fail(h, KSFD_EINVAL, "krylov_op %d has no norm epilogue", (int)op);
    hipSetDevice(h->device);
    h->dr.valid = false;
    rec_reset(h);
    int rc;
    const GmDev D = gm_dev_block(h);
    if (op == KSFD_KOP_GMRES_COEF) {
        const double *row = coef;
        double *so = scalars;
        HIPCHK(h, hipMemsetAsync(D.coef, 0, sizeof(double) * KSFD_MAXDOT, h->st));
        HIPCHK(h, hipMemsetAsync(D.H, 0, sizeof(double) * (size_t)D.ld * k, h->st));
        for (int j = 0; j < k; j++) {
            const int nrow = 2 * (j + 1) + 1;
            HIPCHK(h, hipMemcpyAsync(h->dres, row, sizeof(double) * nrow, hipMemcpyHostToDevice, h->st));
            launch_gmres_coef(h, D, j, beta);
            HIPCHK(h, hipGetLastError());
            HIPCHK(h, hipMemcpyAsync(so, D.coef, sizeof(double) * k, hipMemcpyDeviceToHost, h->st));
            HIPCHK(h, hipMemcpyAsync(so + k, D.scale, sizeof(double), hipMemcpyDeviceToHost, h->st));
            HIPCHK(h, hipMemcpyAsync(so + k + 1, D.mon + 2 * j, 2 * sizeof(double), hipMemcpyDeviceToHost, h->st));
            HIPCHK(h, hipStreamSynchronize(h->st));
            row += nrow; so += k + 3;
        }
        for (int c = 0; c < k; c++) HIPCHK(h, hipMemcpyAsync(so + (size_t)c * (k + 1), D.H + (size_t)D.ld * c, sizeof(double) * (k + 1), hipMemcpyDeviceToHost, h->st));
        HIPCHK(h, hipMemcpyAsync(so + (size_t)k * (k + 1), D.g, sizeof(double) * (k + 1), hipMemcpyDeviceToHost, h->st));
        HIPCHK(h, hipStreamSynchronize(h->st));
        return KSFD_OK;
    }
    const int64_t nl = (int64_t)h->G.F * h->G.nloc, vs = h->vlen;
    for (int i = 0; i < nvec; i++) {
        if ((rc = upload(h, vecs + (int64_t)i * nl, layout, h->V + (int64_t)i * vs))) return rc;
        HIPCHK(h, hipStreamSynchronize(h->st));
    }
    double *const w = h->V + (int64_t)k * vs;
    switch (op) {
    case KSFD_KOP_LINCOMB: {
        const double *xs[6];
        for (int t = 0; t < k; t++) xs[t] = h->V + (int64_t)t * vs;
        rc = op_lincomb(h, k, xs, coef, h->V, want_norm != 0);
    } break;
    case KSFD_KOP_MULTIDOT: rc = op_multidot(h, w, h->V, k); break;
    case KSFD_KOP_MULTIDOT_GRAM: rc = op_multidot_gram(h, w, h->V, k); break;
    case KSFD_KOP_GS_UPDATE: rc = op_gs_update(h, w, h->V, k, coef, alpha); break;
    case KSFD_KOP_BASIS_AXPY: rc = op_basis_axpy(h, w, h->V, k, coef, beta, want_norm != 0); break;
    default: {
        HIPCHK(h, hipMemcpyAsync(D.coef, coef, sizeof(double) * k, hipMemcpyHostToDevice, h->st));
        HIPCHK(h, hipMemcpyAsync(D.scale, &alpha, sizeof(double), hipMemcpyHostToDevice, h->st));
        launch_gs_update_dev(h, w, h->V, k, D.coef, D.scale);
        HIPCHK(h, hipGetLastError());
        HIPCHK(h, hipStreamSynchronize(h->st));
        rc = KSFD_OK;
    } break;
    }
    if (rc) return rc;
    for (int i = 0; i < nscal; i++) scalars[i] = h->hres[i];
    for (int i = 0; i < nvec; i++)
        if ((rc = download(h, h->V + (int64_t)i * vs, layout, out_vecs + (int64_t)i * nl))) return rc;
    return KSFD_OK;
}
extern "C" int ksfd_set_spectral_params(ksfd_handle *h, double from_stiffness, int32_t enable)
{
    if (!h) return KSFD_EINVAL;
    if (from_stiffness > 0.0) h->spec_from = from_stiffness;
    if (enable == 0) h->spec.user_off = true;
    else if (enable > 0) { h->spec.user_off = false; h->memo.spec_bad_until = 0; h->memo.spec_backoff = 8; }
    return KSFD_OK;
}
extern "C" int ksfd_synchronize(ksfd_handle *h)
{
    if (!h) return KSFD_EINVAL;
    hipSetDevice(h->device);
    HIPCHK(h, hipStreamSynchronize(h->st));
    return KSFD_OK;
}
extern "C" int ksfd_set_tuning(ksfd_handle *h, int32_t use_fused, int32_t yseg, int32_t yseg_jvp)
{
    if (!h) return KSFD_EINVAL;
    if (use_fused >= 0) {
        h->use_fused = use_fused & 1; h->use_frozen = !(use_fused & 2); h->overlap = !(use_fused & 4);
        h->async_mode = (use_fused & 8) ? 1 : 0;
        h->rec_mode = (use_fused & 16) ? 0 : ((use_fused & 32) ? 2 : 1);
        if ((use_fused >> 6) & 7) h->rec_keep = std::min((use_fused >> 6) & 7, 4);
        h->poly_fp32 = !(use_fused & 512);
        h->fuse_stage = !(use_fused & 1024);
        h->zero_copy = !(use_fused & 2048) && h->hres_dev;
        h->rhs3d_strip = !(use_fused & 8192);
        h->spec_guess = !(use_fused & 16384);
        h->rhs_carry = !(use_fused & 32768);
        h->spec_predict = !(use_fused & 65536);
        h->restart_grow = !(use_fused & 131072);
        h->mg_warm_power = !(use_fused & 262144);
        h->mg_fp32 = !(use_fused & 524288);
        h->rec_mg = (use_fused & 1048576) != 0;
        h->rhs_dots = !(use_fused & 2097152);
        if (h->mg_fuse != !(use_fused & 4096)) { h->mg_fuse = !(use_fused & 4096); h->mg_shift = -1.0; if (h->mg_graph) { hipGraphExecDestroy(h->mg_graph); h->mg_graph = nullptr; } }
    }
    if (yseg > 0) h->yseg = yseg;
    if (yseg_jvp > 0) h->yseg_jvp = yseg_jvp;
    return KSFD_OK;
}

extern "C" int ksfd_bench_kernel(ksfd_handle *h, int32_t cls, int32_t reps, double *avg_ms, double *bytes_per_launch)
{
    if (!h || reps < 1 || !avg_ms) return KSFD_EINVAL;
    hipSetDevice(h->device);
    hipEvent_t a, b;
    HIPCHK(h, hipEventCreate(&a));
    HIPCHK(h, hipEventCreate(&b));
    const bool was = h->profiling;
    h->profiling = false;
    int rc = KSFD_OK;
    double by = 0.0;
    auto one = [&]() -> int {
        const double b0 = h->bytes_acc;
        int r = KSFD_OK;
        double coef[KSFD_MAXDOT] = { 0 };
        switch (cls) {
        case KC_RHS: r = op_rhs(h, h->u, -1, h->t3); break;
        case KC_JVP: r = h->use_frozen ? op_jvp_frozen(h, h->Y, 1, 1.0, h->t3) : op_jvp(h, h->u, h->Y, 1, 1.0, h->t3); break;
        case KC_MULTIDOT: {
            Scope sc(h, KC_MULTIDOT, vbytes(h, 9));
            VW_DISPATCH(h, hipLaunchKernelGGL((k_multidot<8, VW>), dim3(vec2(h) ? (h->nblk_vec + 1) / 2 : h->nblk_vec), dim3(KSFD_BLOCK), 0, h->st, h->kv, (const double *)h->t3, (const double *)h->V, h->vlen, 8, h->part));
        } break;
        case KC_GSUPDATE: r = op_gs_update(h, h->t3, h->V, 8, coef, 1.0); break;
        case KC_SPECTRAL: r = spec_apply(h, 10.0, h->Y, h->t3); break;
        case KC_LINCOMB: { const double *xs[3] = { h->u, h->Y, h->Y + h->vlen }; double aa[3] = { 1.0, 0.5, 0.25 }; r = op_lincomb(h, 3, xs, aa, h->t3); } break;
        case KSFD_BENCH_ROTATE: {
            std::vector<double> Pb((size_t)31 * KSFD_ROT_MAXOUT, 0.0);
            for (int j = 0; j < 11; j++) Pb[(size_t)j * KSFD_ROT_MAXOUT + j] = 1.0;
            r = op_basis_rotate(h, h->V, 31, 11, Pb.data(), KSFD_ROT_MAXOUT);
        } break;
        case KSFD_BENCH_ROTATE_COMPOSED: {
            for (int i = 0; i < 31; i++) coef[i] = 1.0 / 31.0;
            for (int j = 0; j < 11 && !r; j++) r = op_basis_axpy(h, h->Zb + (int64_t)j * h->vlen, h->V, 31, coef, 0.0);
        } break;
        case KSFD_BENCH_BAND_FACTOR: r = banded_factor(h, h->band.shift); break;
        case KSFD_BENCH_BAND_SOLVE: r = banded_solve(h, h->Y, h->t3); break;
        case KSFD_BENCH_MGC_SETUP: { bool ok = false; MGLevel &L = h->mg[mg_end(h)]; r = mgc_setup(h, L, 1.0, &ok); if (!r && !ok) r = fail(h, KSFD_ELINEAR, "bench_kernel: the coarse factorization is flagged"); } break;
        case KSFD_BENCH_MGC_APPLY: { MGLevel &L = h->mg[mg_end(h)]; r = mgc_apply(h, L, L.v64.b, L.v64.x); } break;
        case KSFD_BENCH_MGC_FACTOR_COLUMNS: {
            MGLevel &L = h->mg[mg_end(h)];
            const LUSys Y{ &L.G, &L.P, L.coef, (long long)L.G.sloc, 0, KC_MG };
            h->mgc.ready = false;
            if (!(r = lu_assemble(h, h->mgc.lu, Y, 1.0))) r = lu_factor_blocks(h, h->mgc.lu, KC_MG, false);
        } break;
        default: r = fail(h, KSFD_EINVAL, "bench_kernel: class %d not benchable", cls);
        }
        by = h->bytes_acc - b0;
        return r;
    };
    if ((cls == KSFD_BENCH_ROTATE || cls == KSFD_BENCH_ROTATE_COMPOSED) && (h->restart_alloc < 30 || !h->Zb)) { rc = fail(h, KSFD_EINVAL, "bench_kernel: the rotation benchmark needs 31 basis vectors and the flexible basis"); goto done; }
    if (cls == KSFD_BENCH_ROTATE || cls == KSFD_BENCH_ROTATE_COMPOSED) { h->dr.valid = false; rec_reset(h); }
    if (cls == KSFD_BENCH_BAND_FACTOR || cls == KSFD_BENCH_BAND_SOLVE) {
        if ((rc = banded_guard(h))) goto done;
        if (!h->band.valid) { rc = fail(h, KSFD_EINVAL, "bench_kernel: the banded benchmark needs a factorization (ksfd_banded_apply first)"); goto done; }
        if ((rc = ensure_coef(h, true))) goto done;
    }
    if (cls >= KSFD_BENCH_MGC_SETUP && cls <= KSFD_BENCH_MGC_FACTOR_COLUMNS) {
        if (h->mgc.kind != 1 || !h->mg_ok) { rc = fail(h, KSFD_EINVAL, "bench_kernel: the coarse-solve benchmark needs ksfd_set_mg_coarse(kind 1)"); goto done; }
        if ((rc = ensure_coef(h)) || (!h->mg_coef_valid && (rc = mg_restrict_coefs(h)))) goto done;
        h->mg_shift = -1.0;
        if (cls == KSFD_BENCH_MGC_APPLY) { bool ok = false; if ((rc = mgc_setup(h, h->mg[mg_end(h)], 1.0, &ok))) goto done; if (!ok) { rc = fail(h, KSFD_ELINEAR, "bench_kernel: the coarse factorization is flagged"); goto done; } }
    }
    if ((rc = halo(h, h->u))) goto done;
    if (h->use_frozen && (cls == KC_JVP || cls == KC_SPECTRAL) && (rc = ensure_coef(h, true))) goto done;
    if (cls == KC_SPECTRAL && (rc = spec_means(h))) goto done;
    for (int i = 0; i < 3 && !rc; i++) rc = one();
    if (rc) goto done;
    hipEventRecord(a, h->st);
    for (int i = 0; i < reps && !rc; i++) rc = one();
    hipEventRecord(b, h->st);
    if (hipEventSynchronize(b) != hipSuccess) rc = fail(h, KSFD_EHIP, "event sync failed");
    if (!rc) {
        float ms = 0.f;
        hipEventElapsedTime(&ms, a, b);
        *avg_ms = ms / reps;
        if (bytes_per_launch) *bytes_per_launch = by;
    }
done:
    h->profiling = was;
    hipEventDestroy(a);
    hipEventDestroy(b);
    return rc;
}
```

ksfd_amd/csrc/mg_host.hip.h:

```cpp
#pragma once
static void mgc_free(ksfd_handle *h);
static int mgc_setup(ksfd_handle *h, MGLevel &L, double shift, bool *ok);
static int mgc_apply(ksfd_handle *h, MGLevel &L, const double *b, double *x);

static inline size_t mg_end(const ksfd_handle *h) { return h->mgc.kind == 1 ? (size_t)h->mgc.level : h->mg.size() - 1; }
static inline bool mg_f32(const ksfd_handle *h, size_t l) { return h->mg[l].f32 && !(h->mgc.kind == 1 && l == (size_t)h->mgc.level); }

static JvpSys mg_sys(const ksfd_handle *h, const MGLevel &L)
{
    const bool l0 = &L == &h->mg[0];
    return { &L.G, &L.P, L.coef, l0 ? (h->poly_fp32 ? h->coef32 : nullptr) : L.coef32, L.dG, l0 ? KC_JVP : KC_MG };
}
static JvpPath mg_path(const ksfd_handle *h, const MGLevel &L) { const JvpPath p = jvp_path(h, L.G, h->P.nlig, JVP_NX_LEVEL); return p == JP_LDS3D ? JP_STRIP3D : p; }

static void mg_free(ksfd_handle *h)
{
    mgc_free(h);
    h->mgc = MGCoarse();
    if (h->mg_graph) { hipGraphExecDestroy(h->mg_graph); h->mg_graph = nullptr; }
    for (size_t l = 0; l < h->mg.size(); l++) {
        MGLevel &L = h->mg[l];
        void *bufs[] = { L.dinv, l ? L.coef : nullptr, L.coef32, L.Ad, L.dG, L.pv, L.v64.x, L.v64.b, L.v64.r, L.v64.d, L.v32.x, L.v32.b, L.v32.r, L.v32.d };
        for (void *b : bufs) if (b) hipFree(b);
    }
// ... 311 lines not shown
        S.rr = V.r; S.x_has_d = 0;
    }
    S.x64 = x64;
    return mg_op<T>(h, L, V.d, 6, shift, nullptr, nullptr, &S);
}

static int mg_smooth(ksfd_handle *h, MGLevel &L, double shift, const double *b, double *x, int nu, bool zero_init, double ratio)
{
    if (nu == 2 && mg_can_fuse(h, L)) return mg_smooth_fused(h, L, shift, b, x, zero_init, ratio);
    int rc;
    const int F = L.G.F;
    const int nb = point_blocks(L.G);
    const MGCheb C = mg_cheb(L.lam_max, ratio);
    const long long off = L.kv.off;
    double *const r = L.v64.r, *const d = L.v64.d;
    const double *res = b;
    if (!zero_init) {
        if ((rc = mg_op(h, L, x, 2, shift, r, b))) return rc;
        res = r;
    }
    mg_dinv_apply(h, L, 8.0 * ((zero_init ? 3 : 2) * F + 0.5 * F * F) * L.G.nloc, res, 1.0 / C.theta, d, zero_init ? x : (double *)nullptr);
    bool x_has_d = zero_init;
    double rho = C.rho0;
    for (int k = 1; k < nu; k++) {
        if ((rc = mg_op<double>(h, L, d, 1, shift, L.Ad, nullptr))) return rc;
        const double rhon = C.next(rho);
        const double *rsrc = (zero_init && k == 1) ? b : r;
        if (k == nu - 1) {
            Scope sc(h, KC_MG, 8.0 * (5 * F + 0.5 * F * F) * L.G.nloc);
            NL_DISPATCH(h->P.nlig, hipLaunchKernelGGL((k_cheb_last<NL>), dim3(nb), dim3(KSFD_BLOCK), 0, h->st, L.G.nloc, L.G.plane, (const float *)(L.dinv + off), x + off, rsrc + off, (const double *)(d + off), (const double *)(L.Ad + off), rhon * rho, 2.0 * rhon / C.delta, x_has_d ? 1 : 0));
            x_has_d = true;
        } else {
            if (rsrc != r) HIPCHK(h, hipMemcpyAsync(r, b, sizeof(double) * (size_t)L.vlen, hipMemcpyDeviceToDevice, h->st));
            if (x_has_d && k == 1) {
                HIPCHK(h, hipMemsetAsync(x, 0, sizeof(double) * (size_t)L.vlen, h->st));
            }
            Scope sc(h, KC_MG, 8.0 * (7 * F + 0.5 * F * F) * L.G.nloc);
            NL_DISPATCH(h->P.nlig, hipLaunchKernelGGL((k_cheb_step<NL>), dim3(nb), dim3(KSFD_BLOCK), 0, h->st, L.G.nloc, L.G.plane, (const float *)(L.dinv + off), x + off, r + off, d + off, (const double *)(L.Ad + off), rhon * rho, 2.0 * rhon / C.delta));
            x_has_d = false;
        }
        rho = rhon;
    }
    if (!x_has_d) {
        const double *xs[2] = { x, d };
        KLin LL;
        for (int t = 0; t < 6; t++) { LL.x[t] = t < 2 ? xs[t] : nullptr; LL.a[t] = t < 2 ? 1.0 : 0.0; }
        Scope sc(h, KC_MG, 24.0 * L.vlen);
        hipLaunchKernelGGL((k_lincomb<2, 1>), dim3(L.nblk, F), dim3(KSFD_BLOCK), 0, h->st, L.kv, LL, x);
    }
    HIPCHK(h, hipGetLastError());
    return KSFD_OK;
}

template <typename T>
static int mg_vcycle(ksfd_handle *h, size_t l, double shift, const T *b, T *x, const double *b64 = nullptr, double *x64 = nullptr);

static int mg_coarse_sweeps(const ksfd_handle *h, const MGLevel &L)
{
    const int sweeps = (int)ceil(0.5 * sqrt(L.ratio) * log(2.0 / h->mg_coarse_tol));
    return std::min(std::max(sweeps, 4), h->mg_ncoarse);
}

template <typename T, typename TC>
static int mg_coarse_correction_in(ksfd_handle *h, size_t l, double shift, T *x)
{
    int rc;
    MGLevel &L = h->mg[l], &Lc = h->mg[l + 1];
    MGVecs<T> &V = L.vecs<T>();
    MGVecs<TC> &Vc = Lc.vecs<TC>();
    const int F = L.G.F;
    const double sf = sizeof(T), sk = sizeof(TC);
    if ((rc = mg_halo(h, L, V.r, F))) return rc;
    {
        Scope sc(h, KC_MG, F * (sf * L.G.nloc + sk * Lc.G.nloc));
        if ((rc = mg_launch_restrict(h, L, Lc, F, (const T *)V.r, Vc.b))) return rc;
    }
    if ((rc = mg_border_reduce(h, L, Lc, F, Vc.b))) return rc;
    if ((rc = mg_vcycle<TC>(h, l + 1, shift, Vc.b, Vc.x))) return rc;
    if ((rc = mg_halo(h, Lc, Vc.x, F))) return rc;
    {
        Scope sc(h, KC_MG, F * (2.0 * sf * L.G.nloc + sk * Lc.G.nloc));
        if ((rc = mg_launch_prolong(h, L, Lc, F, (const TC *)Vc.x, x))) return rc;
    }
    HIPCHK(h, hipGetLastError());
    return KSFD_OK;
}
template <typename T>
static int mg_coarse_correction(ksfd_handle *h, size_t l, double shift, T *x)
{
    if constexpr (std::is_same<T, float>::value) if (mg_f32(h, l + 1)) return mg_coarse_correction_in<T, float>(h, l, shift, x);
    return mg_coarse_correction_in<T, double>(h, l, shift, x);
}

template <typename Body>
static int mg_coarse_graph(ksfd_handle *h, double shift, const void *xkey, bool f32, Body body)
{
    int rc;
    if (!h->mg_graph || h->mg_graph_shift != shift || h->mg_graph_x != xkey || h->mg_graph_f32 != f32) {
        if (h->mg_graph) { hipGraphExecDestroy(h->mg_graph); h->mg_graph = nullptr; }
        hipGraph_t g = nullptr;
        const double b0 = h->bytes_acc;
        const int32_t s0 = h->mgc.solves;
        HIPCHK(h, hipStreamBeginCapture(h->st, hipStreamCaptureModeThreadLocal));
        h->capturing = true;
        rc = body();
        h->capturing = false;
        hipError_t e = hipStreamEndCapture(h->st, &g);
        if (rc) { if (g) hipGraphDestroy(g); return rc; }
        if (e != hipSuccess || !g) return fail(h, KSFD_EHIP, "hipStreamEndCapture: %s", hipGetErrorString(e));
        e = hipGraphInstantiate(&h->mg_graph, g, nullptr, nullptr, 0);
        hipGraphDestroy(g);
        if (e != hipSuccess) { h->mg_graph = nullptr; return fail(h, KSFD_EHIP, "hipGraphInstantiate: %s", hipGetErrorString(e)); }
        h->mg_graph_bytes = h->bytes_acc - b0;
        h->bytes_acc = b0;
        h->mgc.graph_solves = h->mgc.solves - s0;
        h->mgc.solves = s0;
        h->mg_graph_shift = shift;
        h->mg_graph_x = xkey;
        h->mg_graph_f32 = f32;
    }
    Scope sc(h, KC_MG, h->mg_graph_bytes);
    HIPCHK(h, hipGraphLaunch(h->mg_graph, h->st));
    h->mgc.solves += h->mgc.graph_solves;
    return KSFD_OK;
}

template <typename T>
static int mg_vcycle(ksfd_handle *h, size_t l, double shift, const T *b, T *x, const double *b64, double *x64)
{
    int rc;
    constexpr bool f32 = std::is_same<T, float>::value;
    MGLevel &L = h->mg[l];
    if constexpr (!f32) if (l == mg_end(h)) {
        if (h->mgc.kind == 1 && h->mgc.ready) return mgc_apply(h, L, b, x);
        return mg_smooth(h, L, shift, b, x, mg_coarse_sweeps(h, L), true, L.ratio);
    }
    auto smooth = [&](bool zero_init) {
        if constexpr (f32) return mg_smooth_fused(h, L, shift, b, x, zero_init, h->mg_ratio, zero_init ? b64 : nullptr, zero_init ? nullptr : x64);
        else return mg_smooth(h, L, shift, b, x, h->mg_nu, zero_init, h->mg_ratio);
    };
    if ((rc = smooth(true))) return rc;
    if ((rc = mg_op<T>(h, L, x, 2, shift, L.vecs<T>().r, b))) return rc;
    if (l == 0 && h->mg_use_graph && !h->capturing) {
        if ((rc = mg_coarse_graph(h, shift, x, f32, [&]() { return mg_coarse_correction(h, 0, shift, x); }))) return rc;
    } else if ((rc = mg_coarse_correction(h, l, shift, x))) return rc;
    return smooth(false);
}

static bool mg_cycle32_ok(const ksfd_handle *h) { return h->mg_fp32 && h->mg[0].f32 && h->mg_nu == 2 && mg_can_fuse(h, h->mg[0]); }

static int mg_precond(ksfd_handle *h, double shift, const double *in, double *out)
{
    int rc;
    if (!h->mg_coef_valid && (rc = mg_restrict_coefs(h))) return rc;
    if (h->mg_shift != shift && (rc = mg_setup_shift(h, shift))) return rc;
    MGVecs<float> &V = h->mg[0].v32;
    if (h->mg_use32 && mg_cycle32_ok(h)) return mg_vcycle<float>(h, 0, shift, V.b, V.x, in, out);
    return mg_vcycle<double>(h, 0, shift, in, out);
}
```

ksfd_amd/csrc/ops.hip.h:

```cpp
#pragma once
static int halo(ksfd_handle *h, double *vec)
{
    if (!h->ring) return KSFD_OK;
    Scope sc(h, KC_HALO, 4.0 * 2.0 * 8.0 * h->G.F * (double)h->G.inner * 2.0);
    int rc = h->tr->exchange(vec, h->G.F, h->G.plane, h->G.inner, h->G.sloc, h->G.ng, h->st);
    if (rc) return fail(h, KSFD_ECOMM, "halo exchange failed: %s", h->tr->error().c_str());
    return KSFD_OK;
}

static int spin_for(ksfd_handle *h, unsigned long long seq)
{
    for (unsigned long long spins = 1;; spins++) {
        if (__atomic_load_n(h->pub_flag, __ATOMIC_ACQUIRE) == seq) return KSFD_OK;
        if ((spins & 0xffff) == 0) {
            hipError_t e = hipStreamQuery(h->st);
            if (e == hipSuccess) {
                if (__atomic_load_n(h->pub_flag, __ATOMIC_ACQUIRE) == seq) return KSFD_OK;
                return fail(h, KSFD_EHIP, "reduction finished without publishing its result");
            }
            if (e != hipErrorNotReady) return fail(h, KSFD_EHIP, "stream error while waiting for a reduction: %s", hipGetErrorString(e));
        }
    }
}

// ... 64 lines not shown
    static const long long t_jvp = getenv("KSFD_WAVES_JVP") ? atoll(getenv("KSFD_WAVES_JVP")) : 4096;
    static const long long t_rhs = getenv("KSFD_WAVES_RHS") ? atoll(getenv("KSFD_WAVES_RHS")) : 6144;
    return strips_for(h->G, jvp ? h->yseg_jvp : h->yseg, jvp ? t_jvp : t_rhs);
}

static K3D k3d_for(const KGeom &G, int rows, int sync, int zseg, long long block_target)
{
    K3D K;
    K.rows = rows; K.sync = sync;
    K.nstrips = (int)((G.nx + KSFD_STRIP_OUT - 1) / KSFD_STRIP_OUT);
    K.nygrp = (int)((G.ny + rows - 1) / rows);
    const long long fit = std::max<long long>((long long)K.nstrips * K.nygrp * G.sloc / block_target, 2);
    K.zseg = (int)std::min<long long>(zseg, fit);
    K.nzseg = (int)((G.sloc + K.zseg - 1) / K.zseg);
    K.nblocks = round8((long long)K.nstrips * K.nygrp * K.nzseg);
    return K;
}
static int rows3d(const ksfd_handle *h)
{
    static const int env = getenv("KSFD_ROWS3D") ? atoi(getenv("KSFD_ROWS3D")) : 0;
    return (env == 8 && h->P.nlig == 1) ? 8 : 4;
}
static K3D make_k3d(const ksfd_handle *h)
{
    static const int sync_env = getenv("KSFD_SYNC3D") ? atoi(getenv("KSFD_SYNC3D")) : 1;
    const int rows = rows3d(h);
    return k3d_for(h->G, rows, sync_env && (h->G.ny % rows == 0), h->zseg, rows == 8 ? 512 : 1024);
}

struct JvpSys {
    const KGeom *G; const KPhys *P;
    const double *coef;
    const float *coef32;
    double *dG;
    int cls;
};
static JvpSys jvp_sys(const ksfd_handle *h) { return { &h->G, &h->P, h->coef, h->poly_fp32 ? h->coef32 : nullptr, h->dGb, KC_JVP }; }

enum JvpPath { JP_STRIP2D, JP_LDS3D, JP_STRIP3D, JP_GENERIC };
static const int JVP_NX_GRID = 4;
static const int JVP_NX_LEVEL = 16;
static JvpPath jvp_path(const ksfd_handle *h, const KGeom &G, int nlig, int min_nx)
{
    static const int j3l_env = getenv("KSFD_J3L") ? atoi(getenv("KSFD_J3L")) : 1;
    if (!h->use_fused || G.dim < 2 || (G.nx % 2) || G.nx < min_nx || nlig > 4) return JP_GENERIC;
    if (G.dim == 2) return G.sloc >= 4 ? JP_STRIP2D : JP_GENERIC;
    return (j3l_env && nlig <= 2 && G.ny % KSFD_J3L_ROWS == 0) ? JP_LDS3D : JP_STRIP3D;
}
static bool fused_ok(const ksfd_handle *h) { return jvp_path(h, h->G, h->P.nlig, JVP_NX_GRID) == JP_STRIP2D; }
static bool strip3d_ok(const ksfd_handle *h) { const JvpPath p = jvp_path(h, h->G, h->P.nlig, JVP_NX_GRID); return p == JP_LDS3D || p == JP_STRIP3D; }

static JvpPath grid_path(ksfd_handle *h)
{
    const JvpPath p = jvp_path(h, h->G, h->P.nlig, JVP_NX_GRID);
    if (p == JP_LDS3D && !h->j3l_attr_set) {
        auto reg = [](const void *k, size_t lds) { return hipFuncSetAttribute(k, hipFuncAttributeMaxDynamicSharedMemorySize, (int)lds) == hipSuccess; };
        h->j3l_usable = h->P.nlig == 1 ? reg((const void *)k_jvp3d_lds<1, double>, ksfd_j3l_lds_bytes<1>()) && reg((const void *)k_jvp3d_lds<1, float>, ksfd_j3l_lds_bytes<1>())
                                       : reg((const void *)k_jvp3d_lds<2, double>, ksfd_j3l_lds_bytes<2>()) && reg((const void *)k_jvp3d_lds<2, float>, ksfd_j3l_lds_bytes<2>());
        h->j3l_attr_set = true;
        if (!h->j3l_usable) hipGetLastError();
    }
    return (p == JP_LDS3D && !h->j3l_usable) ? JP_STRIP3D : p;
}
static bool j3l_ok(ksfd_handle *h) { return grid_path(h) == JP_LDS3D; }
static K3D make_k3d_lds(const ksfd_handle *h) { return k3d_for(h->G, KSFD_J3L_ROWS, 0, h->zseg, 1024); }

static inline long long part_capacity() { return (long long)(2 * KSFD_MAXDOT + 4) * 4096; }
static long long strip_waves(const ksfd_handle *h, bool jvp = false) { const KStrips K = make_strips(h, jvp); return (long long)K.nstrips * K.nseg; }
static long long k3d_waves(ksfd_handle *h) { const K3D K = j3l_ok(h) ? make_k3d_lds(h) : make_k3d(h); return (long long)K.nblocks * K.rows; }

template <typename TO>
static void j3l_launch(ksfd_handle *h, const K3D &K, const double *v, int mode, double shift, TO *out, const double *yadd, double alpha, double beta, double *normpart)
{
    const KGeom &G = h->G;
    if (h->P.nlig == 1) hipLaunchKernelGGL((k_jvp3d_lds<1, TO>), dim3(K.nblocks), dim3(KSFD_J3L_ROWS * KSFD_WAVE), ksfd_j3l_lds_bytes<1>(), h->st, G, h->P, K, (const double *)h->coef, v, mode, shift, out, yadd, alpha, beta, normpart);
    else hipLaunchKernelGGL((k_jvp3d_lds<2, TO>), dim3(K.nblocks), dim3(KSFD_J3L_ROWS * KSFD_WAVE), ksfd_j3l_lds_bytes<2>(), h->st, G, h->P, K, (const double *)h->coef, v, mode, shift, out, yadd, alpha, beta, normpart);
}

static KSrc src_of(const ksfd_handle *h, int stage)
{
    KSrc s;
    for (int c = 0; c <= KSFD_MAXL; c++) s.p[c] = (stage >= 0 && c < h->G.F) ? h->src[stage][c] : nullptr;
    return s;
}

static void dg_pass(ksfd_handle *h, const JvpSys &Y, const double *v, int cls = KC_GFIELD)
{
    const KGeom &G = *Y.G;
    auto launch = [&] { NL_DISPATCH(Y.P->nlig, hipLaunchKernelGGL((k_dg_frozen<NL>), dim3(plane_blocks(G)), dim3(KSFD_BLOCK), 0, h->st, G, Y.coef, v, Y.dG)); };
    if (cls < 0) return launch();
    Scope sc(h, cls, 8.0 * (2 + Y.P->nlig + G.F) * (double)G.plane);
    launch();
}

template <bool SMOOTH, typename TC, typename TV, typename TY, typename TO, typename TS>
static void jvp2d_launch(ksfd_handle *h, const JvpSys &Y, const KStrips &K, const TC *C, const TV *v, int mode, double shift, TO *out, const TY *yadd, double alpha, double beta, const KSmoothT<TS> &sm, double *normpart)
{
    static_assert(SMOOTH || std::is_same<TS, double>::value, "no smoother: pass KSmooth{}");
    NL_DISPATCH(Y.P->nlig, if constexpr (NL <= 4) hipLaunchKernelGGL((k_jvp2d_frozen<NL, TC, TV, TY, TO, 1, SMOOTH, TS>), dim3(K.nblocks), dim3(KSFD_BLOCK), 0, h->st,
                                                                     *Y.G, *Y.P, K, C, v, mode, shift, out, yadd, alpha, beta, sm, normpart));
}
template <typename TO>
static void jvp3d_launch(ksfd_handle *h, const JvpSys &Y, const K3D &K, const double *v, int mode, double shift, TO *out, const double *yadd, double alpha, double beta, double *normpart)
{
    if (K.rows == 8) hipLaunchKernelGGL((k_jvp3d_frozen<1, TO, 8>), dim3(K.nblocks), dim3(8 * KSFD_WAVE), 0, h->st, *Y.G, *Y.P, K, Y.coef, v, (const double *)Y.dG, mode, shift, out, yadd, alpha, beta, normpart);
    else NL_DISPATCH(Y.P->nlig, if constexpr (NL <= 4) hipLaunchKernelGGL((k_jvp3d_frozen<NL, TO>), dim3(K.nblocks), dim3(KSFD_BLOCK), 0, h->st, *Y.G, *Y.P, K, Y.coef, v, (const double *)Y.dG, mode, shift, out, yadd, alpha, beta, normpart));
}
static void jvpgen_launch(ksfd_handle *h, const JvpSys &Y, int nblocks, const double *v, int mode, double shift, double *out, const double *yadd, double alpha, double beta, const KSmooth &sm)
{
    NL_DISPATCH(Y.P->nlig, hipLaunchKernelGGL((k_jvp_generic<NL>), dim3(nblocks), dim3(KSFD_BLOCK), 0, h->st, *Y.G, *Y.P, Y.coef, v, Y.coef + Y.G->plane, (const double *)Y.dG, mode, shift, out, yadd, alpha, beta, sm));
}

struct JvpBytes { double impl, alg; };
template <typename TC = double, typename TV = double, typename TY = double, typename TO = double>
static JvpBytes jvp_bytes(const KGeom &G, int mode, double ncoef, double extra = 0.0)
{
    const double y = (mode == 2 || mode == 3) ? G.F : 0;
    return { ncoef * sizeof(TC) + G.F * (double)(sizeof(TV) + sizeof(TO)) + y * (double)sizeof(TY) + extra, 8.0 * (3.0 * G.F + y) };
}

template <typename Exchange, typename Launch>
static int with_halo_overlap(ksfd_handle *h, const KStrips &K, double *normpart, Exchange exchange, Launch launch)
{
    int rc;
    const bool ovl = h->overlap && K.nseg >= 3;
    if (ovl) {
        HIPCHK(h, hipEventRecord(h->ev_ready, h->st));
        if ((rc = launch(strips_sub(K, 1, 1, K.nseg - 2), (double)(K.nseg - 2) / K.nseg, normpart))) return rc;
        HIPCHK(h, hipStreamWaitEvent(h->st_comm, h->ev_ready, 0));
    }
    if (exchange(ovl ? h->st_comm : h->st)) return fail(h, KSFD_ECOMM, "halo exchange failed: %s", h->tr->error().c_str());
    if (!ovl) return launch(K, 1.0, normpart);
    HIPCHK(h, hipEventRecord(h->ev_halo, h->st_comm));
    HIPCHK(h, hipStreamWaitEvent(h->st, h->ev_halo, 0));
    return launch(strips_sub(K, 0, K.nseg - 1, 2), 2.0 / K.nseg, normpart ? normpart + (long long)K.nstrips * (K.nseg - 2) : nullptr);
}

static int op_rhs(ksfd_handle *h, const double *u, int stage, double *out, const KComb *cmb = nullptr, bool want_norm = false, double *halo_vec = nullptr,
                  int ndots = 0, const double *dotv = nullptr)
{
    const KGeom &G = h->G;
    KSrc S = src_of(h, stage);
    const KPhys &PP = (stage >= 0 && stage < 4 && h->Pst_valid[stage]) ? h->Pst[stage] : h->P;
    if (!h->ring) halo_vec = nullptr;
    if (fused_ok(h)) {
        KStrips K = make_strips(h);
        KComb C = cmb ? *cmb : KComb{};
        const long long nwaves = strip_waves(h);
        const bool fused_norm = want_norm && nwaves * (1 + ndots) <= part_capacity();
        KDots D = KDots{};
        if (fused_norm && ndots > 0) { D.n = std::min(ndots, 2); D.stride = nwaves; for (int q = 0; q < D.n; q++) D.v[q] = dotv + (int64_t)q * h->vlen; }
        bool carry = h->rhs_carry && C.nout > 0 && C.nout == C.nin;
        for (int j = 0; j < C.nout && carry; j++) carry = C.yin[j] == C.yout[j];
        auto launch = [&](const KStrips &Kx, double frac, double *np) -> int {
            Scope sc(h, KC_RHS, vbytes(h, 2 + C.nin + (carry ? 0 : C.nout) + D.n) * frac, vbytes(h, 2 + C.nin + C.nout + D.n) * frac);
            if (carry) { NL_DISPATCH(h->P.nlig, if constexpr (NL <= 4) hipLaunchKernelGGL((k_rhs2d_fused<NL, true>), dim3(Kx.nblocks), dim3(KSFD_BLOCK), 0, h->st, G, PP, Kx, u, S, out, C, np, D)); }
            else { NL_DISPATCH(h->P.nlig, if constexpr (NL <= 4) hipLaunchKernelGGL((k_rhs2d_fused<NL>), dim3(Kx.nblocks), dim3(KSFD_BLOCK), 0, h->st, G, PP, Kx, u, S, out, C, np, D)); }
            return KSFD_OK;
        };
        double *np = fused_norm ? h->part : (double *)nullptr;
        int rc = !halo_vec ? launch(K, 1.0, np) : with_halo_overlap(h, K, np, [&](hipStream_t st) {
            Scope sc(h, KC_HALO, 4.0 * 2.0 * 8.0 * G.F * (double)G.inner * 2.0);
            return h->tr->exchange(halo_vec, G.F, G.plane, G.inner, G.sloc, G.ng, st);
        }, launch);
        if (rc) return rc;
        HIPCHK(h, hipGetLastError());
        if (fused_norm) return reduce_rows(h, 1 + D.n, (int)nwaves, 0);
        if (want_norm) return fail(h, KSFD_EINVAL, "op_rhs: fused norm needs the strip kernels");
        return KSFD_OK;
    }
    if (halo_vec) { int rc = halo(h, halo_vec); if (rc) return rc; }
    if (strip3d_ok(h) && h->rhs3d_strip) {
        if (want_norm) return fail(h, KSFD_EINVAL, "op_rhs: fused norm is a 2-D feature");
        KComb C = cmb ? *cmb : KComb{};
        const double *uin = u;
        const double *Gplane = h->Gb;
        const bool reuse_G = C.nin == 0 && u == h->u && h->coef_fresh && h->use_frozen && h->coef && &PP == &h->P;
        if (reuse_G) Gplane = h->coef + G.plane;
        else {
            Scope sc(h, KC_GFIELD, 8.0 * ((1 + C.nin) * G.F + (C.nin ? G.F : 0) + 1) * (double)G.plane, C.nin ? vbytes(h, 2 + C.nin) : 0.0);
            NL_DISPATCH(h->P.nlig, if constexpr (NL <= 4) hipLaunchKernelGGL((k_gfield_comb<NL>), dim3(plane_blocks(G)), dim3(KSFD_BLOCK), 0, h->st, G, PP, u, C, C.nin ? h->Z : (double *)nullptr, h->Gb));
        }
        if (C.nin) uin = h->Z;
        K3D K = make_k3d(h);
        Scope sc(h, KC_RHS, 8.0 * (2.0 * G.F + 1 + C.nout * G.F) * (double)G.nloc, vbytes(h, 2 + C.nout));
        if (K.rows == 8) hipLaunchKernelGGL((k_rhs3d_strip<1, 8>), dim3(K.nblocks), dim3(8 * KSFD_WAVE), 0, h->st, G, PP, K, uin, Gplane, S, out, C);
        else NL_DISPATCH(h->P.nlig, if constexpr (NL <= 4) hipLaunchKernelGGL((k_rhs3d_strip<NL>), dim3(K.nblocks), dim3(KSFD_BLOCK), 0, h->st, G, PP, K, uin, Gplane, S, out, C));
    } else {
        {
            Scope sc(h, KC_GFIELD, 8.0 * (G.F + 1) * (double)G.plane);
            NL_DISPATCH(h->P.nlig, hipLaunchKernelGGL((k_gfield<NL, false>), dim3(plane_blocks(G)), dim3(KSFD_BLOCK), 0, h->st, G, PP, u, (const double *)nullptr, h->Gb, (double *)nullptr));
        }
        Scope sc(h, KC_RHS, vbytes(h, 2) + 8.0 * (double)G.nloc, vbytes(h, 2));
        NL_DISPATCH(h->P.nlig, hipLaunchKernelGGL((k_rhs_generic<NL>), dim3(point_blocks(G)), dim3(KSFD_BLOCK), 0, h->st, G, PP, u, h->Gb, S, out));
    }
    HIPCHK(h, hipGetLastError());
    return KSFD_OK;
}

static int op_jvp(ksfd_handle *h, const double *u, const double *v, int mode, double shift, double *out)
{
    const KGeom &G = h->G;
    if (fused_ok(h)) {
        KStrips K = make_strips(h, true);
        Scope sc(h, KC_JVP, vbytes(h, 3));
        NL_DISPATCH(h->P.nlig, if constexpr (NL <= 4) hipLaunchKernelGGL((k_jvp2d_fused<NL>), dim3(K.nblocks), dim3(KSFD_BLOCK), 0, h->st, G, h->P, K, u, v, mode, shift, out));
    } else {
        {
            Scope sc(h, KC_GFIELD, 8.0 * (2 * G.F + 2) * (double)G.plane);
            NL_DISPATCH(h->P.nlig, hipLaunchKernelGGL((k_gfield<NL, true>), dim3(plane_blocks(G)), dim3(KSFD_BLOCK), 0, h->st, G, h->P, u, v, h->Gb, h->dGb));
        }
        Scope sc(h, KC_JVP, vbytes(h, 3) + 16.0 * (double)G.nloc, vbytes(h, 3));
        NL_DISPATCH(h->P.nlig, hipLaunchKernelGGL((k_jvp_generic<NL>), dim3(point_blocks(G)), dim3(KSFD_BLOCK), 0, h->st, G, h->P, u, v, h->Gb, h->dGb, mode, shift, out));
    }
    HIPCHK(h, hipGetLastError());
    return KSFD_OK;
}

static int op_jcoef(ksfd_handle *h, const double *u, bool want_means = false)
{
    const KGeom &G = h->G;
    const int nbp = plane_blocks(G);
    if (!h->coef32 && h->poly_fp32 && fused_ok(h) && h->P.nlig <= 4 && G.plane % 2 == 0 && G.inner % 2 == 0 &&
        hipMalloc((void **)&h->coef32, sizeof(float) * (size_t)(3 + h->P.nlig) * G.plane) != hipSuccess) { h->coef32 = nullptr; h->poly_fp32 = false; }
    float *c32 = h->poly_fp32 ? h->coef32 : nullptr;
    want_means = want_means && (long long)(1 + h->P.nlig) * nbp <= part_capacity();
    {
    Scope sc(h, KC_GFIELD, (8.0 * (G.F + 3 + h->P.nlig) + (c32 ? 4.0 * (3 + h->P.nlig) : 0.0)) * (double)G.plane);
    NL_DISPATCH(h->P.nlig, hipLaunchKernelGGL((k_jcoef<NL>), dim3(nbp), dim3(KSFD_BLOCK), 0, h->st, G, h->P, u, h->coef, c32, want_means ? h->part : (double *)nullptr));
    }
    HIPCHK(h, hipGetLastError());
    if (want_means) {
        int rc = reduce_rows(h, 1 + h->P.nlig, nbp, 0);
        if (rc) return rc;
        const double ntot = (double)h->cfg.n[0] * (double)h->cfg.n[1] * (double)h->cfg.n[2];
        h->spec.a_rr = h->hres[0] / ntot;
        for (int l = 0; l < h->P.nlig; l++) h->spec.a_rU[l] = h->hres[1 + l] / ntot;
    }
    return KSFD_OK;
}

static int ensure_coef(ksfd_handle *h, bool ghosts_done = false)
{
    if (h->coef_fresh) return KSFD_OK;
    int rc;
    if (!ghosts_done && (rc = halo(h, h->u))) return rc;
    if ((rc = op_jcoef(h, h->u, h->spec.ok))) return rc;
    h->coef_fresh = true;
    h->mg_coef_valid = false; h->mg_shift = -1.0;
    h->spec.means_valid = h->spec.ok && (long long)(1 + h->P.nlig) * plane_blocks(h->G) <= part_capacity();
    return KSFD_OK;
}

template <typename TC, typename TV, typename TY, typename TO>
static int jvp2d_launch_t(ksfd_handle *h, const KStrips &K, double frac, const TC *C, const TV *v, int mode, double shift, TO *out, const TY *yadd, double alpha, double beta, double *normpart = nullptr)
{
    const KGeom &G = h->G;
    const JvpBytes B = jvp_bytes<TC, TV, TY, TO>(G, mode, 3 + h->P.nlig);
    Scope sc(h, KC_JVP, B.impl * (double)G.nloc * frac, B.alg * (double)G.nloc * frac);
    jvp2d_launch<false>(h, jvp_sys(h), K, C, v, mode, shift, out, yadd, alpha, beta, KSmooth{}, normpart);
    HIPCHK(h, hipGetLastError());
    return KSFD_OK;
}

template <typename TC, typename TV, typename TY, typename TO>
static int jvp2d_halo_t(ksfd_handle *h, const TC *C, TV *v, int mode, double shift, TO *out, const TY *yadd, double alpha, double beta, double *normpart = nullptr)
{
    const KGeom &G = h->G;
    auto launch = [&](const KStrips &Kx, double frac, double *np) { return jvp2d_launch_t(h, Kx, frac, C, v, mode, shift, out, yadd, alpha, beta, np); };
    if (!h->ring) return launch(make_strips(h, true), 1.0, normpart);
    const long long scale = sizeof(double) / sizeof(TV);
    return with_halo_overlap(h, make_strips(h, true), normpart, [&](hipStream_t st) {
        Scope sc(h, KC_HALO, 4.0 * 2.0 * sizeof(TV) * G.F * (double)G.inner * 2.0);
        return h->tr->exchange(reinterpret_cast<double *>(v), G.F, G.plane / scale, G.inner / scale, G.sloc, G.ng, st);
    }, launch);
}

static int op_jvp_frozen(ksfd_handle *h, const double *v, int mode, double shift, double *out, const double *yadd = nullptr, double alpha = 0.0, double beta = 0.0)
{
    const KGeom &G = h->G;
    const JvpSys Y = jvp_sys(h);
    const JvpBytes B = jvp_bytes(G, mode, 3 + h->P.nlig), Bdg = jvp_bytes(G, mode, 3);
    const JvpPath path = grid_path(h);
    if (path == JP_STRIP2D) return jvp2d_launch_t(h, make_strips(h, true), 1.0, Y.coef, v, mode, shift, out, yadd, alpha, beta);
    if (path == JP_LDS3D) {
        Scope sc(h, KC_JVP, B.impl * (double)G.nloc, B.alg * (double)G.nloc);
        j3l_launch<double>(h, make_k3d_lds(h), v, mode, shift, out, yadd, alpha, beta, nullptr);
    } else {
        dg_pass(h, Y, v);
        Scope sc(h, KC_JVP, Bdg.impl * (double)G.nloc, Bdg.alg * (double)G.nloc);
        if (path == JP_STRIP3D) jvp3d_launch<double>(h, Y, make_k3d(h), v, mode, shift, out, yadd, alpha, beta, nullptr);
        else jvpgen_launch(h, Y, point_blocks(G), v, mode, shift, out, yadd, alpha, beta, KSmooth{});
    }
    HIPCHK(h, hipGetLastError());
    return KSFD_OK;
}

static int op_jvp_frozen_halo(ksfd_handle *h, double *v, int mode, double shift, double *out, const double *yadd = nullptr, double alpha = 0.0, double beta = 0.0)
{
    if (!h->ring) return op_jvp_frozen(h, v, mode, shift, out, yadd, alpha, beta);
    if (!h->overlap || !fused_ok(h) || make_strips(h, true).nseg < 3 || h->P.nlig > 4) {
        const int rc = halo(h, v);
        return rc ? rc : op_jvp_frozen(h, v, mode, shift, out, yadd, alpha, beta);
    }
    return jvp2d_halo_t<double, double, double, double>(h, (const double *)h->coef, v, mode, shift, out, yadd, alpha, beta);
}

static int op_residual32(ksfd_handle *h, const double *x, double shift, const double *b, float *r32)
{
    const KGeom &G = h->G;
    const long long nwaves = G.dim == 3 ? k3d_waves(h) : strip_waves(h, true);
    if (nwaves > part_capacity()) return fail(h, KSFD_EINVAL, "op_residual32: too many waves for the fused norm");
    if (G.dim == 3) {
        const JvpSys Y = jvp_sys(h);
        const bool j3l = j3l_ok(h);
        if (!j3l) dg_pass(h, Y, x);
        const JvpBytes B = j3l ? jvp_bytes<double, double, double, float>(G, 2, 3 + h->P.nlig, 8.0 * G.F) : jvp_bytes<double, double, double, float>(G, 2, 3);
        Scope sc(h, KC_JVP, B.impl * (double)G.nloc, B.alg * (double)G.nloc);
        if (j3l) j3l_launch<float>(h, make_k3d_lds(h), x, 2, shift, r32, b, 0.0, 0.0, h->part);
        else jvp3d_launch<float>(h, Y, make_k3d(h), x, 2, shift, r32, b, 0.0, 0.0, h->part);
    } else if (int rc = jvp2d_halo_t(h, h->coef, const_cast<double *>(x), 2, shift, r32, b, 0.0, 0.0, h->part)) return rc;
    HIPCHK(h, hipGetLastError());
    return reduce_rows(h, 1, (int)nwaves, 0);
}

static inline bool vec2(const ksfd_handle *h) { return (h->G.nloc % 2 == 0) && (h->kv.off % 2 == 0) && (h->G.plane % 2 == 0); }
static inline dim3 vgridw(const ksfd_handle *h, int vw) { return dim3((h->nblk_vec + vw - 1) / vw, h->G.F); }
#define VW_DISPATCH(h, CALL) do { if (vec2(h)) { constexpr int VW = 2; CALL; } else { constexpr int VW = 1; CALL; } } while (0)
#define KB_DISPATCH(k, CALL)                                                                       \
    do {                                                                                           \
        if ((k) <= 4) { constexpr int KB = 4; CALL; }                                              \
        else if ((k) <= 8) { constexpr int KB = 8; CALL; }                                         \
        else if ((k) <= 16) { constexpr int KB = 16; CALL; }                                       \
        else { constexpr int KB = 32; CALL; }                                                      \
    } while (0)
#define NT_DISPATCH(nt, CALL)                                                                      \
    switch (nt) {                                                                                  \
    case 1: { constexpr int NT = 1; CALL; } break;                                                 \
    case 2: { constexpr int NT = 2; CALL; } break;                                                 \
    case 3: { constexpr int NT = 3; CALL; } break;                                                 \
    case 4: { constexpr int NT = 4; CALL; } break;                                                 \
    case 5: { constexpr int NT = 5; CALL; } break;                                                 \
    default: { constexpr int NT = 6; CALL; } break;                                                \
    }

static int op_lincomb(ksfd_handle *h, int nt, const double *const *x, const double *a, double *out, bool want_norm = false)
{
    double *part = want_norm ? h->part : nullptr;
    KLin L;
    for (int t = 0; t < 6; t++) { L.x[t] = t < nt ? x[t] : nullptr; L.a[t] = t < nt ? a[t] : 0.0; }
    Scope sc(h, KC_LINCOMB, vbytes(h, nt + 1));
    NT_DISPATCH(nt, VW_DISPATCH(h, hipLaunchKernelGGL((k_lincomb<NT, VW>), vgridw(h, VW), dim3(KSFD_BLOCK), 0, h->st, h->kv, L, out, part)));
    HIPCHK(h, hipGetLastError());
    if (want_norm) { const dim3 gr = vgridw(h, vec2(h) ? 2 : 1); return reduce_rows(h, 1, (int)(gr.x * gr.y), 0); }
    return KSFD_OK;
}

static int op_multidot(ksfd_handle *h, const double *w, const double *V, int k)
{
    if (k > 32) {
        std::vector<double> acc((size_t)k + 1);
        for (int c0 = 0; c0 < k; c0 += 32) {
            const int kc = std::min(32, k - c0);
            int rc = op_multidot(h, w, V + (int64_t)c0 * h->vlen, kc);
            if (rc) return rc;
            for (int i = 0; i < kc; i++) acc[c0 + i] = h->hres[i];
            acc[k] = h->hres[kc];
        }
        if (k + 1 > 128) return fail(h, KSFD_EINVAL, "op_multidot: %d vectors exceed the result buffer", k);
        for (int i = 0; i <= k; i++) h->hres[i] = acc[i];
        return KSFD_OK;
    }
    const int nb = vec2(h) ? (h->nblk_vec + 1) / 2 : h->nblk_vec;
    {
        Scope sc(h, KC_MULTIDOT, vbytes(h, k + 1));
        KB_DISPATCH(k, VW_DISPATCH(h, hipLaunchKernelGGL((k_multidot<KB, VW>), dim3(nb), dim3(KSFD_BLOCK), 0, h->st, h->kv, w, V, h->vlen, k, h->part)));
    }
    HIPCHK(h, hipGetLastError());
    return reduce_rows(h, k + 1, nb, 0);
}

static int op_multidot_gram(ksfd_handle *h, const double *w, const double *V, int k)
{
    const int nb = vec2(h) ? (h->nblk_vec + 1) / 2 : h->nblk_vec;
    {
        Scope sc(h, KC_MULTIDOT, vbytes(h, k + 1));
        KB_DISPATCH(k, VW_DISPATCH(h, hipLaunchKernelGGL((k_multidot_gram<KB, VW>), dim3(nb), dim3(KSFD_BLOCK), 0, h->st, h->kv, w, V, h->vlen, k, h->part)));
    }
    HIPCHK(h, hipGetLastError());
    return reduce_rows(h, 2 * k + 1, nb, 0);
}

static int op_gs_update(ksfd_handle *h, double *w, const double *V, int k, const double *coef, double scale)
{
    if (k > 32) {
        for (int c0 = 0; c0 < k; c0 += 32) {
            const int kc = std::min(32, k - c0);
            int rc = op_gs_update(h, w, V + (int64_t)c0 * h->vlen, kc, coef + c0, c0 + kc == k ? scale : 1.0);
            if (rc) return rc;
        }
        return KSFD_OK;
    }
    KCoef C;
// ... 83 lines not shown
```

ksfd_amd/csrc/pointwise.hip.h:

```cpp
#pragma once
#include <hip/hip_runtime.h>
#include "params.h"

#define KSFD_WAVE 64
#define KSFD_BLOCK 256
#define KSFD_MAXDOT 34

__device__ __forceinline__ double ksfd_clamp(double x, double lo) { return !(x >= lo) ? lo : x; }

__device__ __forceinline__ double ksfd_rcp(double x)
{
    double r = __builtin_amdgcn_rcp(x);
    r = fma(fma(-x, r, 1.0), r, r);
    r = fma(fma(-x, r, 1.0), r, r);
    return r;
}
__device__ __forceinline__ double ksfd_div(double a, double x)
{
    const double r = ksfd_rcp(x);
    const double q = a * r;
    return fma(fma(-x, q, a), r, q);
}
__device__ __forceinline__ double ksfd_log(double x)
{
// ... 229 lines not shown
        const int i = threadIdx.x;
        const bool live = (i < k) || (i >= KMAX && i < KMAX + k) || (i == 2 * KMAX);
        if (live) {
            double s = 0.0;
            for (int q = 0; q < KSFD_BLOCK / KSFD_WAVE; q++) s += red[q][i];
            const int row = (i == 2 * KMAX) ? 2 * k : (i >= KMAX ? k + (i - KMAX) : i);
            part[(long long)row * gridDim.x + blockIdx.x] = s;
        }
    }
}

__global__ void __launch_bounds__(KSFD_BLOCK) k_reduce_rows(const double *__restrict__ part, int nblk, int op,
                                                            double *__restrict__ out, double *pub = nullptr,
                                                            unsigned int *count = nullptr, unsigned long long *flag = nullptr,
                                                            unsigned long long seq = 0)
{
    __shared__ double red[KSFD_BLOCK / KSFD_WAVE];
    const double *row = part + (long long)blockIdx.x * nblk;
    double s = op ? -1.0e300 : 0.0;
    for (int b0 = threadIdx.x; b0 < nblk; b0 += 8 * blockDim.x) {
        double t[8];
#pragma unroll
        for (int q = 0; q < 8; q++) { const int b = b0 + q * blockDim.x; t[q] = b < nblk ? row[b] : (op ? -1.0e300 : 0.0); }
#pragma unroll
        for (int q = 0; q < 8; q++) s = op ? fmax(s, t[q]) : s + t[q];
    }
    s = op ? ksfd_wave_max(s) : ksfd_wave_sum(s);
    if ((threadIdx.x & (KSFD_WAVE - 1)) == 0) red[threadIdx.x / KSFD_WAVE] = s;
    __syncthreads();
    if (threadIdx.x == 0) {
        double t = red[0];
        for (int q = 1; q < KSFD_BLOCK / KSFD_WAVE; q++) t = op ? fmax(t, red[q]) : t + red[q];
        out[blockIdx.x] = t;
        if (pub) {
            __hip_atomic_store(pub + blockIdx.x, t, __ATOMIC_RELAXED, __HIP_MEMORY_SCOPE_SYSTEM);
            __threadfence_system();
            if (atomicAdd(count, 1u) == gridDim.x - 1) {
                *count = 0;
                __threadfence_system();
                __hip_atomic_store(flag, seq, __ATOMIC_RELEASE, __HIP_MEMORY_SCOPE_SYSTEM);
            }
        }
    }
}

__global__ void k_publish(const double *__restrict__ res, int n, double *pub, unsigned long long *flag, unsigned long long seq)
{
    if (threadIdx.x < n) __hip_atomic_store(pub + threadIdx.x, res[threadIdx.x], __ATOMIC_RELAXED, __HIP_MEMORY_SCOPE_SYSTEM);
    __threadfence_system();
    __syncthreads();
    if (threadIdx.x == 0) __hip_atomic_store(flag, seq, __ATOMIC_RELEASE, __HIP_MEMORY_SCOPE_SYSTEM);
}

struct KCoef {
    double h[KSFD_MAXDOT];
};
template <int KMAX, int VW>
__global__ void __launch_bounds__(KSFD_BLOCK) k_gs_update(KVec g, double *__restrict__ w,
                                                          const double *__restrict__ V, long long vstride, int k,
                                                          KCoef C, double scale)
{
    const long long base = (long long)blockIdx.y * g.plane + g.off;
    const long long stride = (long long)gridDim.x * blockDim.x * VW;
    for (long long p = ((long long)blockIdx.x * blockDim.x + threadIdx.x) * VW; p < g.nloc; p += stride) {
        typename KPack<VW>::T s = kload<VW>(w + base + p);
#pragma unroll
        for (int i = 0; i < KMAX; i++)
            if (i < k) {
                const typename KPack<VW>::T vv = kload<VW>(V + (long long)i * vstride + base + p);
#pragma unroll
                for (int e = 0; e < VW; e++) kset(s, e, kget(s, e) - C.h[i] * kget(vv, e));
            }
#pragma unroll
        for (int e = 0; e < VW; e++) kset(s, e, kget(s, e) * scale);
        kstore<VW>(w + base + p, s);
    }
}

template <int KMAX, int VW>
__global__ void __launch_bounds__(KSFD_BLOCK) k_basis_axpy(KVec g, double *__restrict__ x,
                                                           const double *__restrict__ V, long long vstride, int k,
                                                           KCoef C, double beta, double *part = nullptr)
{
    const long long base = (long long)blockIdx.y * g.plane + g.off;
    const long long stride = (long long)gridDim.x * blockDim.x * VW;
    double nrm = 0.0;
    for (long long p = ((long long)blockIdx.x * blockDim.x + threadIdx.x) * VW; p < g.nloc; p += stride) {
        typename KPack<VW>::T s;
        if (beta == 0.0) {
#pragma unroll
            for (int e = 0; e < VW; e++) kset(s, e, 0.0);
        } else {
            s = kload<VW>(x + base + p);
#pragma unroll
            for (int e = 0; e < VW; e++) kset(s, e, beta * kget(s, e));
        }
#pragma unroll
        for (int i = 0; i < KMAX; i++)
            if (i < k && C.h[i] != 0.0) {
                const typename KPack<VW>::T vv = kload<VW>(V + (long long)i * vstride + base + p);
#pragma unroll
                for (int e = 0; e < VW; e++) kset(s, e, kget(s, e) + C.h[i] * kget(vv, e));
            }
        kstore<VW>(x + base + p, s);
#pragma unroll
        for (int e = 0; e < VW; e++) nrm += kget(s, e) * kget(s, e);
    }
    if (part) ksfd_block_sum_to(nrm, part + (long long)blockIdx.y * gridDim.x + blockIdx.x);
}

#define KSFD_ROT_MAXIN 121
#define KSFD_ROT_MAXOUT 18
template <int NOUT, int VW>
__global__ void __launch_bounds__(KSFD_BLOCK) k_basis_rotate(KVec g, double *V, long long vstride, int nin, int nout,
                                                             const double *__restrict__ P, int ldp)
{
    __shared__ double sP[KSFD_ROT_MAXIN * NOUT];
    for (int q = threadIdx.x; q < nin * NOUT; q += blockDim.x) {
        const int i = q / NOUT, j = q - i * NOUT;
        sP[q] = j < nout ? P[i * ldp + j] : 0.0;
    }
    __syncthreads();
    const long long base = (long long)blockIdx.y * g.plane + g.off;
    const long long stride = (long long)gridDim.x * blockDim.x * VW;
    for (long long p = ((long long)blockIdx.x * blockDim.x + threadIdx.x) * VW; p < g.nloc; p += stride) {
        double acc[NOUT][VW];
#pragma unroll
        for (int j = 0; j < NOUT; j++)
#pragma unroll
            for (int e = 0; e < VW; e++) acc[j][e] = 0.0;
        const double *src = V + base + p;
#pragma unroll 4
        for (int i = 0; i < nin; i++) {
            const typename KPack<VW>::T vv = kload<VW>(src + (long long)i * vstride);
            const double *row = sP + i * NOUT;
#pragma unroll
            for (int j = 0; j < NOUT; j++) {
                const double c = row[j];
#pragma unroll
                for (int e = 0; e < VW; e++) acc[j][e] = fma(c, kget(vv, e), acc[j][e]);
            }
        }
#pragma unroll
        for (int j = 0; j < NOUT; j++)
            if (j < nout) {
                typename KPack<VW>::T s;
#pragma unroll
                for (int e = 0; e < VW; e++) kset(s, e, acc[j][e]);
                kstore<VW>(V + (long long)j * vstride + base + p, s);
            }
    }
}

__global__ void __launch_bounds__(KSFD_BLOCK) k_rosw_finish(KVec g, double *__restrict__ u,
                                                            const double *__restrict__ Y, long long ystride,
                                                            double bt0, double bt1, double bt2, double bt3,
                                                            double e0, double e1, double e2, double e3,
                                                            double atol, double rtol, double *__restrict__ errout,
                                                            double *__restrict__ part)
{
    __shared__ double red[KSFD_BLOCK / KSFD_WAVE];
    double acc = 0.0;
    const long long stride = (long long)gridDim.x * blockDim.x;
    for (int c = 0; c < g.nf; c++) {
        const long long base = (long long)c * g.plane + g.off;
        for (long long p = (long long)blockIdx.x * blockDim.x + threadIdx.x; p < g.nloc; p += stride) {
            const double y0 = Y[base + p], y1 = Y[ystride + base + p], y2 = Y[2 * ystride + base + p],
                         y3 = Y[3 * ystride + base + p];
            const double un = u[base + p] + (bt0 * y0 + bt1 * y1 + bt2 * y2 + bt3 * y3);
            const double er = e0 * y0 + e1 * y1 + e2 * y2 + e3 * y3;
            const double tol = atol + rtol * fmax(fabs(un), fabs(un + er));
            const double q = er / tol;
            acc += q * q;
            u[base + p] = un;
            if (errout) errout[base + p] = er;
        }
    }
    acc = ksfd_wave_sum(acc);
    if ((threadIdx.x & (KSFD_WAVE - 1)) == 0) red[threadIdx.x / KSFD_WAVE] = acc;
    __syncthreads();
    if (threadIdx.x == 0) {
        double t = 0.0;
        for (int q = 0; q < KSFD_BLOCK / KSFD_WAVE; q++) t += red[q];
        part[blockIdx.x] = t;
    }
}

__global__ void __launch_bounds__(KSFD_BLOCK) k_groom(KVec g, double *__restrict__ u, double rhomin, double Umin, double *__restrict__ copy = nullptr)
{
    const long long base = (long long)blockIdx.y * g.plane + g.off;
    const double lo = blockIdx.y == 0 ? rhomin : Umin;
    const long long stride = (long long)gridDim.x * blockDim.x;
    for (long long p = (long long)blockIdx.x * blockDim.x + threadIdx.x; p < g.nloc; p += stride) {
        const double v = ksfd_clamp(u[base + p], lo);
        u[base + p] = v;
        if (copy) copy[base + p] = v;
    }
}

__global__ void __launch_bounds__(KSFD_BLOCK) k_sum_rho(KVec g, const double *__restrict__ u, double *__restrict__ part)
{
    __shared__ double red[KSFD_BLOCK / KSFD_WAVE];
    double acc = 0.0;
    const long long stride = (long long)gridDim.x * blockDim.x;
    for (long long p = (long long)blockIdx.x * blockDim.x + threadIdx.x; p < g.nloc; p += stride) acc += u[g.off + p];
    acc = ksfd_wave_sum(acc);
    if ((threadIdx.x & (KSFD_WAVE - 1)) == 0) red[threadIdx.x / KSFD_WAVE] = acc;
    __syncthreads();
    if (threadIdx.x == 0) {
        double t = 0.0;
        for (int q = 0; q < KSFD_BLOCK / KSFD_WAVE; q++) t += red[q];
        part[blockIdx.x] = t;
    }
}

__global__ void __launch_bounds__(KSFD_BLOCK) k_mul_rho(KVec g, double *__restrict__ u, const double *__restrict__ f,
                                                        double scalar)
{
    const long long stride = (long long)gridDim.x * blockDim.x;
    for (long long p = (long long)blockIdx.x * blockDim.x + threadIdx.x; p < g.nloc; p += stride)
        u[g.off + p] *= f ? f[p] : scalar;
}

__device__ __forceinline__ long long ksfd_host_index(const KGeom &G, int layout, int c, long long p)
{
    if (layout == 0) return c + (long long)G.F * p;
    if (layout == 1) return (long long)c * G.nloc + p;
    long long i = p % G.nx, r = p / G.nx;
    if (G.dim == 1) return (long long)c * G.nx + i;
    long long j = r % G.ny, k = r / G.ny;
    if (G.dim == 2) return ((long long)c * G.nx + i) * G.ny + j;
    return (((long long)c * G.nx + i) * G.ny + j) * G.nz + k;
}
__global__ void __launch_bounds__(KSFD_BLOCK) k_from_host_layout(KGeom G, int layout, const double *__restrict__ flat,
                                                                 double *__restrict__ dev, long long devplane,
                                                                 long long devoff)
{
    const int c = blockIdx.y;
    const long long stride = (long long)gridDim.x * blockDim.x;
    for (long long p = (long long)blockIdx.x * blockDim.x + threadIdx.x; p < G.nloc; p += stride)
        dev[(long long)c * devplane + devoff + p] = flat[ksfd_host_index(G, layout, c, p)];
}
__global__ void __launch_bounds__(KSFD_BLOCK) k_to_host_layout(KGeom G, int layout, const double *__restrict__ dev,
                                                               long long devplane, long long devoff,
                                                               double *__restrict__ flat)
{
    const int c = blockIdx.y;
    const long long stride = (long long)gridDim.x * blockDim.x;
    for (long long p = (long long)blockIdx.x * blockDim.x + threadIdx.x; p < G.nloc; p += stride)
        flat[ksfd_host_index(G, layout, c, p)] = dev[(long long)c * devplane + devoff + p];
}


#define KSFD_ASYNC_MAXK 32
static_assert(KSFD_ASYNC_MAXK <= KSFD_MAXDOT, "k_gmres_coef keeps k coefficients in KSFD_MAXDOT slots");
static_assert(KSFD_ASYNC_MAXK <= 32, "k_multidot_gram and k_gs_update_dev are instantiated for at most 32 basis vectors (KB_DISPATCH)");
__global__ void k_gmres_coef(int j, int m, double beta, const double *__restrict__ dres, double *__restrict__ Gm,
                             double *__restrict__ H, double *__restrict__ cs, double *__restrict__ sn,
                             double *__restrict__ g, double *__restrict__ coef, double *__restrict__ scale,
                             double *__restrict__ mon)
{
    if (threadIdx.x != 0 || blockIdx.x != 0) return;
    const int k = j + 1, ld = m + 1;
    if (j == 0) { for (int i = 0; i <= m; i++) g[i] = 0.0; g[0] = beta; }
    const double *d = dres, *gr = dres + k;
    const double ww = dres[2 * k];
    for (int i = 0; i < k; i++) { Gm[i * ld + j] = gr[i]; Gm[j * ld + i] = gr[i]; }
    double c[KSFD_MAXDOT];
    double cd = 0.0, cGc = 0.0;
    for (int i = 0; i < k; i++) {
        double s = 0.0;
        for (int l = 0; l < k; l++) s += ((i == l ? 1.0 : 0.0) - Gm[i * ld + l]) * d[l];
        c[i] = d[i] + s;
    }
    for (int i = 0; i < k; i++) {
        cd += c[i] * d[i];
        double s = 0.0;
        for (int l = 0; l < k; l++) s += Gm[i * ld + l] * c[l];
        cGc += c[i] * s;
    }
    double hn2 = ww - 2.0 * cd + cGc;
    if (!(hn2 > 0.0)) hn2 = (hn2 != hn2) ? hn2 : 0.0;
    const double hn = sqrt(hn2);
    for (int i = 0; i < k; i++) coef[i] = c[i];
    *scale = hn > 0.0 ? 1.0 / hn : 0.0;
    double *Hc = H + (size_t)ld * j;
    for (int i = 0; i < k; i++) Hc[i] = c[i];
    Hc[k] = hn;
    for (int i = 0; i < j; i++) {
        const double t = cs[i] * Hc[i] + sn[i] * Hc[i + 1];
        Hc[i + 1] = -sn[i] * Hc[i] + cs[i] * Hc[i + 1];
        Hc[i] = t;
    }
    const double den = hypot(Hc[j], Hc[j + 1]);
    cs[j] = den > 0.0 ? Hc[j] / den : 1.0;
    sn[j] = den > 0.0 ? Hc[j + 1] / den : 0.0;
    Hc[j] = den;
    Hc[j + 1] = 0.0;
    g[j + 1] = -sn[j] * g[j];
    g[j] = cs[j] * g[j];
    mon[2 * j] = fabs(g[j + 1]);
    mon[2 * j + 1] = hn;
}

template <int KMAX, int VW>
__global__ void __launch_bounds__(KSFD_BLOCK) k_gs_update_dev(KVec g, double *__restrict__ w,
                                                              const double *__restrict__ V, long long vstride, int k,
                                                              const double *__restrict__ coef,
                                                              const double *__restrict__ scale)
{
    const long long base = (long long)blockIdx.y * g.plane + g.off;
    const long long stride = (long long)gridDim.x * blockDim.x * VW;
    double cf[KMAX];
#pragma unroll
    for (int i = 0; i < KMAX; i++) cf[i] = i < k ? coef[i] : 0.0;
    const double sc = *scale;
    for (long long p = ((long long)blockIdx.x * blockDim.x + threadIdx.x) * VW; p < g.nloc; p += stride) {
        typename KPack<VW>::T s = kload<VW>(w + base + p);
#pragma unroll
        for (int i = 0; i < KMAX; i++)
            if (i < k) {
                const typename KPack<VW>::T vv = kload<VW>(V + (long long)i * vstride + base + p);
#pragma unroll
                for (int e = 0; e < VW; e++) kset(s, e, kget(s, e) - cf[i] * kget(vv, e));
            }
#pragma unroll
        for (int e = 0; e < VW; e++) kset(s, e, kget(s, e) * sc);
        kstore<VW>(w + base + p, s);
    }
}
```

ksfd_amd/csrc/stencil.hip.h:

```cpp
#pragma once
#include <type_traits>
#include "pointwise.hip.h"

struct KSrc {
    const double *p[KSFD_MAXL + 1];
};

struct KComb {
    int nin, nout;
    const double *yin[3], *yout[3];
    double ain[3], aout[3];
};

struct KDots {
    int n;
    long long stride;
    const double *v[2];
};

template <typename TS = double>
struct KSmoothT {
    const float *dinv;
    const TS *rr;
    TS *x, *out2;
// ... 314 lines not shown
            for (int q = 0; q < KSFD_BLOCK / KSFD_WAVE; q++) m = fmax(m, red[q][threadIdx.x]);
            part[(long long)threadIdx.x * gridDim.x + blockIdx.x] = m;
        }
    }
}

#define KSFD_STRIP_OUT 124

struct KStrips {
    int nstrips;
    int nseg;
    int yseg;
    int nblocks;
    int seg0;
    int seg_stride;
};

__device__ __forceinline__ int ksfd_xcd_remap(int b, int nblocks)
{
    const int per = nblocks >> 3;
    return (b & 7) * per + (b >> 3);
}

__device__ __forceinline__ long long ksfd_rowoff(const KGeom &G, long long r)
{
    if (G.wrap_slow) {
        if (r < 0) r += G.sloc;
        else if (r >= G.sloc) r -= G.sloc;
        return r * G.nx;
    }
    return (r + G.ng) * G.nx;
}

__device__ __forceinline__ double2 ksfd_ld2(const double *p) { return *reinterpret_cast<const double2 *>(p); }
__device__ __forceinline__ void ksfd_st2(double *p, double a, double b)
{
    *reinterpret_cast<double2 *>(p) = make_double2(a, b);
}
__device__ __forceinline__ double2 ksfd_ld2(const float *p)
{
    const float2 t = *reinterpret_cast<const float2 *>(p);
    return make_double2((double)t.x, (double)t.y);
}
__device__ __forceinline__ void ksfd_st2(float *p, double a, double b)
{
    *reinterpret_cast<float2 *>(p) = make_float2((float)a, (float)b);
}

struct KX {
    double l0, l1, r0, r1;
};
__device__ __forceinline__ double ksfd_lane_from_left(double a)
{
    int lo = __double2loint(a), hi = __double2hiint(a);
    lo = __builtin_amdgcn_update_dpp(lo, lo, 0x138, 0xf, 0xf, false);
    hi = __builtin_amdgcn_update_dpp(hi, hi, 0x138, 0xf, 0xf, false);
    return __hiloint2double(hi, lo);
}
__device__ __forceinline__ double ksfd_lane_from_right(double a)
{
    int lo = __double2loint(a), hi = __double2hiint(a);
    lo = __builtin_amdgcn_update_dpp(lo, lo, 0x130, 0xf, 0xf, false);
    hi = __builtin_amdgcn_update_dpp(hi, hi, 0x130, 0xf, 0xf, false);
    return __hiloint2double(hi, lo);
}
__device__ __forceinline__ KX ksfd_xnb(double a0, double a1)
{
    KX x;
    x.l0 = ksfd_lane_from_left(a0);
    x.l1 = ksfd_lane_from_left(a1);
    x.r0 = ksfd_lane_from_right(a0);
    x.r1 = ksfd_lane_from_right(a1);
    return x;
}
__device__ __forceinline__ void ksfd_dx(double a0, double a1, const KX &x, double &d1_0, double &d1_1)
{
    d1_0 = KSFD_D1(x.l0, x.l1, a1, x.r0);
    d1_1 = KSFD_D1(x.l1, a0, x.r0, x.r1);
}
__device__ __forceinline__ void ksfd_dxx(double a0, double a1, const KX &x, double &d2_0, double &d2_1)
{
    d2_0 = KSFD_D2(x.l0, x.l1, a0, a1, x.r0);
    d2_1 = KSFD_D2(x.l1, a0, a1, x.r0, x.r1);
}
struct KXf {
    float l0, l1, r0, r1;
};
__device__ __forceinline__ float ksfd_lane_from_left(float a)
{
    int v = __float_as_int(a);
    v = __builtin_amdgcn_update_dpp(v, v, 0x138, 0xf, 0xf, false);
    return __int_as_float(v);
}
__device__ __forceinline__ float ksfd_lane_from_right(float a)
{
    int v = __float_as_int(a);
    v = __builtin_amdgcn_update_dpp(v, v, 0x130, 0xf, 0xf, false);
    return __int_as_float(v);
}
__device__ __forceinline__ KXf ksfd_xnb(float a0, float a1)
{
    KXf x;
    x.l0 = ksfd_lane_from_left(a0);
    x.l1 = ksfd_lane_from_left(a1);
    x.r0 = ksfd_lane_from_right(a0);
    x.r1 = ksfd_lane_from_right(a1);
    return x;
}
__device__ __forceinline__ void ksfd_dx(float a0, float a1, const KXf &x, double &d1_0, double &d1_1)
{
    d1_0 = KSFD_D1((double)x.l0, (double)x.l1, (double)a1, (double)x.r0);
    d1_1 = KSFD_D1((double)x.l1, (double)a0, (double)x.r0, (double)x.r1);
}
__device__ __forceinline__ void ksfd_dxx(float a0, float a1, const KXf &x, double &d2_0, double &d2_1)
{
    d2_0 = KSFD_D2((double)x.l0, (double)x.l1, (double)a0, (double)a1, (double)x.r0);
    d2_1 = KSFD_D2((double)x.l1, (double)a0, (double)a1, (double)x.r0, (double)x.r1);
}
__device__ __forceinline__ double2 ksfd_ldw(const double *p) { return *reinterpret_cast<const double2 *>(p); }
__device__ __forceinline__ float2 ksfd_ldw(const float *p) { return *reinterpret_cast<const float2 *>(p); }

struct KWaveJob {
    long long wid;
    long long c0;
    long long r0, r1;
    bool store;
    bool valid;
    bool up;
    __device__ __forceinline__ long long row(long long q) const { return up ? q : (r0 + r1 - 1 - q); }
};
__device__ __forceinline__ KWaveJob ksfd_wave_job(const KGeom &G, const KStrips &S)
{
    KWaveJob J;
    const int lane = threadIdx.x & (KSFD_WAVE - 1);
    const long long wid = (long long)ksfd_xcd_remap(blockIdx.x, S.nblocks) * (KSFD_BLOCK / KSFD_WAVE) + (threadIdx.x >> 6);
    J.wid = wid;
    J.valid = wid < (long long)S.nstrips * S.nseg;
    const int strip = (int)(wid % S.nstrips);
    const long long seg = S.seg0 + (wid / S.nstrips) * S.seg_stride;
    const long long half = G.nx >> 1;
    const long long xs = 2 * ((long long)strip * half / S.nstrips);
    const long long xe = 2 * ((long long)(strip + 1) * half / S.nstrips);
    long long c = xs - 2 + 2 * lane;
    c %= G.nx;
    if (c < 0) c += G.nx;
    J.c0 = c;
    J.store = lane >= 1 && lane <= (int)((xe - xs) >> 1);
    J.r0 = seg * S.yseg;
    J.r1 = J.r0 + S.yseg < G.sloc ? J.r0 + S.yseg : G.sloc;
    J.up = (seg & 1) == 0;
    return J;
}

template <int NL, bool CARRY = false>
__global__ void __launch_bounds__(KSFD_BLOCK) k_rhs2d_fused(KGeom G, KPhys P, KStrips S, const double *__restrict__ u,
                                                            KSrc src, double *__restrict__ out, KComb cmb = KComb{},
                                                            double *__restrict__ normpart = nullptr, KDots dots = KDots{})
{
    const KWaveJob J = ksfd_wave_job(G, S);
    if (!J.valid) return;
    double nacc = 0.0, dacc[2] = { 0.0, 0.0 };
    double rw[5][2], gw[5][2], uw[NL][5][2];
    double nr[2], nu[NL][2];
    __shared__ double2 cring[CARRY ? KSFD_BLOCK / KSFD_WAVE : 1][CARRY ? 4 : 1][CARRY ? NL + 1 : 1][CARRY ? KSFD_WAVE : 1];
    const int cw = CARRY ? (threadIdx.x >> 6) : 0, cl = CARRY ? (threadIdx.x & (KSFD_WAVE - 1)) : 0;
    int nload = 0;

    auto load_row = [&](long long r) {
        const long long o = ksfd_rowoff(G, r) + J.c0;
        double2 t = ksfd_ld2(u + o);
        nr[0] = t.x; nr[1] = t.y;
#pragma unroll
        for (int l = 0; l < NL; l++) {
            double2 q = ksfd_ld2(u + (long long)(l + 1) * G.plane + o);
            nu[l][0] = q.x; nu[l][1] = q.y;
        }
        double2 co[NL + 1];
#pragma unroll
        for (int c = 0; c <= NL; c++) co[c] = make_double2(0.0, 0.0);
        for (int j = 0; j < cmb.nin; j++) {
            const double a = cmb.ain[j], ao = CARRY ? cmb.aout[j] : 0.0;
            double2 y = ksfd_ld2(cmb.yin[j] + o);
            nr[0] += a * y.x; nr[1] += a * y.y;
            if (CARRY) { co[0].x += ao * y.x; co[0].y += ao * y.y; }
#pragma unroll
            for (int l = 0; l < NL; l++) {
                double2 q = ksfd_ld2(cmb.yin[j] + (long long)(l + 1) * G.plane + o);
                nu[l][0] += a * q.x; nu[l][1] += a * q.y;
                if (CARRY) { co[l + 1].x += ao * q.x; co[l + 1].y += ao * q.y; }
            }
        }
        if (CARRY) {
#pragma unroll
            for (int c = 0; c <= NL; c++) cring[cw][nload & 3][c][cl] = co[c];
        }
        nload++;
    };
    auto push_row = [&]() {
#pragma unroll
        for (int s = 0; s < 4; s++) {
#pragma unroll
            for (int e = 0; e < 2; e++) {
                rw[s][e] = rw[s + 1][e];
                gw[s][e] = gw[s + 1][e];
#pragma unroll
                for (int l = 0; l < NL; l++) uw[l][s][e] = uw[l][s + 1][e];
            }
        }
#pragma unroll
        for (int e = 0; e < 2; e++) {
            double U[NL], GU[NL], gr;
            double rho = ksfd_clamp(nr[e], P.rhomin);
#pragma unroll
            for (int l = 0; l < NL; l++) { U[l] = ksfd_clamp(nu[l][e], P.Umin); uw[l][4][e] = U[l]; }
            ksfd_G<NL, false>(P, rho, U, gw[4][e], gr, GU);
            rw[4][e] = rho;
        }
    };

    for (int q = -2; q <= 1; q++) { load_row(J.row(J.r0 + q)); push_row(); }
    load_row(J.row(J.r0 + 2));
    for (long long r = J.r0; r < J.r1; r++) {
        push_row();
        if (r + 1 < J.r1) load_row(J.row(r + 3));
        const KX xr = ksfd_xnb(rw[2][0], rw[2][1]);
        const KX xg = ksfd_xnb(gw[2][0], gw[2][1]);
        double d1rx[2], d1gx[2], d2gx[2];
        ksfd_dx(rw[2][0], rw[2][1], xr, d1rx[0], d1rx[1]);
        ksfd_dx(gw[2][0], gw[2][1], xg, d1gx[0], d1gx[1]);
        ksfd_dxx(gw[2][0], gw[2][1], xg, d2gx[0], d2gx[1]);
        double res[NL + 1][2];
#pragma unroll
        for (int e = 0; e < 2; e++) {
            const double d1ry = KSFD_D1(rw[0][e], rw[1][e], rw[3][e], rw[4][e]) * P.inv_h[1];
            const double d1gy = KSFD_D1(gw[0][e], gw[1][e], gw[3][e], gw[4][e]) * P.inv_h[1];
            const double d2gy = KSFD_D2(gw[0][e], gw[1][e], gw[2][e], gw[3][e], gw[4][e]) * P.inv_h2[1];
            res[0][e] = (d1rx[e] * P.inv_h[0]) * (d1gx[e] * P.inv_h[0]) + d1ry * d1gy +
                        rw[2][e] * (d2gx[e] * P.inv_h2[0] + d2gy);
        }
#pragma unroll
        for (int l = 0; l < NL; l++) {
            const KX xu = ksfd_xnb(uw[l][2][0], uw[l][2][1]);
            double d2ux[2];
            ksfd_dxx(uw[l][2][0], uw[l][2][1], xu, d2ux[0], d2ux[1]);
#pragma unroll
            for (int e = 0; e < 2; e++) {
                const double d2uy = KSFD_D2(uw[l][0][e], uw[l][1][e], uw[l][2][e], uw[l][3][e], uw[l][4][e]) * P.inv_h2[1];
                res[l + 1][e] = -P.lig_gamma[l] * uw[l][2][e] + P.lig_s[l] * rw[2][e] +
                                P.lig_D[l] * (d2ux[e] * P.inv_h2[0] + d2uy);
            }
        }
        if (J.store) {
            const long long pi = J.row(r) * G.nx + J.c0;
            const long long o = (long long)G.ng * G.inner + pi;
#pragma unroll
            for (int c = 0; c <= NL; c++) {
                double a = res[c][0], b = res[c][1];
                if (src.p[c]) { double2 s = ksfd_ld2(src.p[c] + pi); a += s.x; b += s.y; }
                if (CARRY) { const double2 cc = cring[cw][(int)(r - J.r0 + 2) & 3][c][cl]; a += cc.x; b += cc.y; }
                else for (int j = 0; j < cmb.nout; j++) {
                    const double2 y = ksfd_ld2(cmb.yout[j] + (long long)c * G.plane + o);
                    a += cmb.aout[j] * y.x; b += cmb.aout[j] * y.y;
                }
                ksfd_st2(out + (long long)c * G.plane + o, a, b);
                nacc += a * a + b * b;
#pragma unroll
                for (int q = 0; q < 2; q++)
                    if (q < dots.n) { const double2 y = ksfd_ld2(dots.v[q] + (long long)c * G.plane + o); dacc[q] += a * y.x + b * y.y; }
            }
        }
    }
    if (normpart) {
        nacc = ksfd_wave_sum(nacc);
        if ((threadIdx.x & (KSFD_WAVE - 1)) == 0) normpart[J.wid] = nacc;
        for (int q = 0; q < dots.n; q++) {
            const double t = ksfd_wave_sum(dacc[q]);
            if ((threadIdx.x & (KSFD_WAVE - 1)) == 0) normpart[(long long)(1 + q) * dots.stride + J.wid] = t;
        }
    }
}

template <int NL>
__global__ void __launch_bounds__(KSFD_BLOCK) k_jvp2d_fused(KGeom G, KPhys P, KStrips S, const double *__restrict__ u,
                                                            const double *__restrict__ v, int mode, double shift,
                                                            double *__restrict__ out)
{
    const KWaveJob J = ksfd_wave_job(G, S);
    if (!J.valid) return;
    double rw[5][2], gw[5][2], vw[5][2], ew[5][2], zw[NL][5][2];
    double nr[2], nv[2], nu[NL][2], nz[NL][2];

    auto load_row = [&](long long r) {
        const long long o = ksfd_rowoff(G, r) + J.c0;
        double2 t = ksfd_ld2(u + o), w = ksfd_ld2(v + o);
        nr[0] = t.x; nr[1] = t.y; nv[0] = w.x; nv[1] = w.y;
#pragma unroll
        for (int l = 0; l < NL; l++) {
            double2 q = ksfd_ld2(u + (long long)(l + 1) * G.plane + o);
            double2 z = ksfd_ld2(v + (long long)(l + 1) * G.plane + o);
            nu[l][0] = q.x; nu[l][1] = q.y; nz[l][0] = z.x; nz[l][1] = z.y;
        }
    };
    auto push_row = [&]() {
#pragma unroll
        for (int s = 0; s < 4; s++) {
#pragma unroll
            for (int e = 0; e < 2; e++) {
                rw[s][e] = rw[s + 1][e]; gw[s][e] = gw[s + 1][e];
                vw[s][e] = vw[s + 1][e]; ew[s][e] = ew[s + 1][e];
#pragma unroll
                for (int l = 0; l < NL; l++) zw[l][s][e] = zw[l][s + 1][e];
            }
        }
#pragma unroll
        for (int e = 0; e < 2; e++) {
            double U[NL], GU[NL], gr;
            double rho = ksfd_clamp(nr[e], P.rhomin);
#pragma unroll
            for (int l = 0; l < NL; l++) U[l] = ksfd_clamp(nu[l][e], P.Umin);
            ksfd_G<NL, true>(P, rho, U, gw[4][e], gr, GU);
            double d = gr * nv[e];
#pragma unroll
            for (int l = 0; l < NL; l++) { d += GU[l] * nz[l][e]; zw[l][4][e] = nz[l][e]; }
            rw[4][e] = rho; vw[4][e] = nv[e]; ew[4][e] = d;
        }
    };

    for (int q = -2; q <= 1; q++) { load_row(J.row(J.r0 + q)); push_row(); }
    load_row(J.row(J.r0 + 2));
    for (long long r = J.r0; r < J.r1; r++) {
        push_row();
        if (r + 1 < J.r1) load_row(J.row(r + 3));
        const KX xr = ksfd_xnb(rw[2][0], rw[2][1]);
        const KX xg = ksfd_xnb(gw[2][0], gw[2][1]);
        const KX xv = ksfd_xnb(vw[2][0], vw[2][1]);
        const KX xe = ksfd_xnb(ew[2][0], ew[2][1]);
        double d1r[2], d1g[2], d1v[2], d1e[2], d2g[2], d2e[2];
        ksfd_dx(rw[2][0], rw[2][1], xr, d1r[0], d1r[1]);
        ksfd_dx(gw[2][0], gw[2][1], xg, d1g[0], d1g[1]);
        ksfd_dx(vw[2][0], vw[2][1], xv, d1v[0], d1v[1]);
        ksfd_dx(ew[2][0], ew[2][1], xe, d1e[0], d1e[1]);
        ksfd_dxx(gw[2][0], gw[2][1], xg, d2g[0], d2g[1]);
        ksfd_dxx(ew[2][0], ew[2][1], xe, d2e[0], d2e[1]);
        double res[NL + 1][2];
#pragma unroll
        for (int e = 0; e < 2; e++) {
            const double ih0 = P.inv_h[0], ih1 = P.inv_h[1];
            const double yr = KSFD_D1(rw[0][e], rw[1][e], rw[3][e], rw[4][e]) * ih1;
            const double yg = KSFD_D1(gw[0][e], gw[1][e], gw[3][e], gw[4][e]) * ih1;
            const double yv = KSFD_D1(vw[0][e], vw[1][e], vw[3][e], vw[4][e]) * ih1;
            const double ye = KSFD_D1(ew[0][e], ew[1][e], ew[3][e], ew[4][e]) * ih1;
            const double lapG = d2g[e] * P.inv_h2[0] + KSFD_D2(gw[0][e], gw[1][e], gw[2][e], gw[3][e], gw[4][e]) * P.inv_h2[1];
            const double lapE = d2e[e] * P.inv_h2[0] + KSFD_D2(ew[0][e], ew[1][e], ew[2][e], ew[3][e], ew[4][e]) * P.inv_h2[1];
            const double jr = (d1v[e] * ih0) * (d1g[e] * ih0) + (d1r[e] * ih0) * (d1e[e] * ih0) + yv * yg + yr * ye +
                              vw[2][e] * lapG + rw[2][e] * lapE;
            res[0][e] = mode ? shift * vw[2][e] - jr : jr;
        }
#pragma unroll
        for (int l = 0; l < NL; l++) {
            const KX xz = ksfd_xnb(zw[l][2][0], zw[l][2][1]);
            double d2z[2];
            ksfd_dxx(zw[l][2][0], zw[l][2][1], xz, d2z[0], d2z[1]);
#pragma unroll
            for (int e = 0; e < 2; e++) {
                const double lap = d2z[e] * P.inv_h2[0] +
                                   KSFD_D2(zw[l][0][e], zw[l][1][e], zw[l][2][e], zw[l][3][e], zw[l][4][e]) * P.inv_h2[1];
                const double ju = -P.lig_gamma[l] * zw[l][2][e] + P.lig_s[l] * vw[2][e] + P.lig_D[l] * lap;
                res[l + 1][e] = mode ? shift * zw[l][2][e] - ju : ju;
// ... 835 lines not shown
```

ksfd_amd/csrc/step.hip.h:

```cpp
#pragma once
using ksfd_ctl::StepMemo;

struct AttemptPlan {
    double hh, shift, stiff;
    bool direct, dr_on;
    bool banded;
    bool use_spec, use_pc, use_poly, use_async;
    bool fuse_stage;
    bool guess_on;
};

struct StageRhs {
    double *b;
    double bnorm2 = -1.0;
    bool dots_done = false;
    double dot[2] = { 0.0, 0.0 };
};

struct StepCounters { double bytes; int64_t rhs, jvp, launches; long long sync, pred, resid; };

static int64_t launches_total(const ksfd_handle *h)
{
    int64_t n = 0;
    for (int c = 0; c < KSFD_NKCLASS; c++) n += h->prof.launches[c];
// ... 46 lines not shown
        if (!lam_done) {
            if (ksfd_ctl::lam_due(m)) {
                const double before = m.lamJ;
                if ((rc = est_lambda_max(h, p.shift, ksfd_ctl::lam_power_its(before)))) return rc;
                ksfd_ctl::lam_estimated(m, before);
            }
            lam_done = true;
        }
        if (h->poly_shift != p.shift) poly_setup(h, p.shift);
        p.use_poly = h->poly_deg >= 1 && h->poly_max_deg >= 1;
    }
    p.use_async = ksfd_ctl::pipelined_allowed(in, r, p.use_poly);
    h->mg_use32 = opts->ksp_rtol >= 1e-7;
    p.fuse_stage = (fused_ok(h) || (strip3d_ok(h) && h->rhs3d_strip)) && h->P.nlig <= 4 && h->fuse_stage;
    p.guess_on = (p.use_spec || p.use_pc) && p.fuse_stage && h->spec_guess && h->bstore;
    return KSFD_OK;
}

static int stage_rhs(ksfd_handle *h, const AttemptPlan &p, int i, StageRhs &r)
{
    int rc;
    const int64_t vs = h->vlen;
    r.b = (p.guess_on && i < 3) ? h->bstore + (int64_t)i * vs : h->bvec;
    if (p.fuse_stage) {
        KComb cmb = KComb{};
        for (int j = 0; j < i; j++) {
            if (h->At[i][j] != 0.0) { cmb.yin[cmb.nin] = h->Y + (int64_t)j * vs; cmb.ain[cmb.nin++] = h->At[i][j]; }
            if (h->Ginv[i][j] != 0.0) { cmb.yout[cmb.nout] = h->Y + (int64_t)j * vs; cmb.aout[cmb.nout++] = -h->Ginv[i][j] / p.hh; }
        }
        const int gdot_j0 = std::max(0, i - h->guess_max), gdot_n = (p.guess_on && i > 0 && h->rhs_dots) ? i - gdot_j0 : 0;
        const bool rhs_norm = p.use_spec && fused_ok(h) && (!(p.guess_on && i > 0) || (gdot_n > 0 && gdot_n <= 2 && strip_waves(h) * (1 + gdot_n) <= part_capacity()));
        r.dots_done = rhs_norm && gdot_n > 0;
        if ((rc = op_rhs(h, h->u, i, r.b, &cmb, rhs_norm, i > 0 ? h->Y + (int64_t)(i - 1) * vs : nullptr, r.dots_done ? gdot_n : 0,
                         r.dots_done ? h->bstore + (int64_t)gdot_j0 * vs : nullptr))) return rc;
        if (rhs_norm) r.bnorm2 = h->hres[0];
        if (r.dots_done) for (int j = 0; j < gdot_n; j++) r.dot[j] = h->hres[1 + j];
        return KSFD_OK;
    }
    const double *zin = h->u;
    if (i > 0) {
        const double *xs[5]; double a[5]; int nt = 0;
        xs[nt] = h->u; a[nt++] = 1.0;
        for (int j = 0; j < i; j++) if (h->At[i][j] != 0.0) { xs[nt] = h->Y + (int64_t)j * vs; a[nt++] = h->At[i][j]; }
        if (nt > 1) {
            if ((rc = op_lincomb(h, nt, xs, a, h->Z))) return rc;
            if ((rc = halo(h, h->Z))) return rc;
            zin = h->Z;
        }
    }
    if ((rc = op_rhs(h, zin, i, h->bvec))) return rc;
    if (i > 0) {
        const double *xs[5]; double a[5]; int nt = 0;
        xs[nt] = h->bvec; a[nt++] = 1.0;
        for (int j = 0; j < i; j++) if (h->Ginv[i][j] != 0.0) { xs[nt] = h->Y + (int64_t)j * vs; a[nt++] = -h->Ginv[i][j] / p.hh; }
        if (nt > 1 && (rc = op_lincomb(h, nt, xs, a, h->bvec))) return rc;
    }
    return KSFD_OK;
}

static int stage_gram_guess(ksfd_handle *h, int i, StageRhs &r, double gb[4][4], SpecGuess &sg)
{
    int rc;
    const int64_t vs = h->vlen;
    if (i == 0) {
        if (r.bnorm2 < 0.0) { if ((rc = op_multidot(h, r.b, r.b, 0))) return rc; r.bnorm2 = h->hres[0]; }
        gb[0][0] = r.bnorm2;
        return KSFD_OK;
    }
    const int j0 = std::max(0, i - h->guess_max), ng = i - j0;
    if (r.dots_done) {
        for (int j = 0; j < ng; j++) gb[i][j0 + j] = gb[j0 + j][i] = r.dot[j];
        gb[i][i] = r.bnorm2;
    } else {
        if ((rc = op_multidot(h, r.b, h->bstore + (int64_t)j0 * vs, ng))) return rc;
        for (int j = 0; j < ng; j++) gb[i][j0 + j] = gb[j0 + j][i] = h->hres[j];
        gb[i][i] = r.bnorm2 = h->hres[ng];
    }
    double cf[3];
    if (ksfd_ctl::stage_guess(gb, i, j0, ng, cf))
        for (int j = 0; j < ng; j++) if (cf[j] != 0.0) { sg.Y[sg.n] = h->Y + (int64_t)(j0 + j) * vs; sg.b[sg.n] = h->bstore + (int64_t)(j0 + j) * vs; sg.c[sg.n++] = cf[j]; }
    return KSFD_OK;
}

static int stage_solve(ksfd_handle *h, const ksfd_step_opts *opts, const AttemptPlan &p, int i, const StageRhs &r, const SpecGuess &sg,
                       bool &spec_failed, ksfd_step_stats &st)
{
    int rc;
    const double shift = p.shift;
    double *xi = h->Y + (int64_t)i * h->vlen;
    LinStats ls;
    if (p.direct) {
        rc = p.banded ? banded_stage(h, shift, r.b, xi, opts, &ls) : direct_stage(h, shift, r.b, xi, opts, &ls);
        st.pc_used |= p.banded ? 32 : 16;
    } else if (p.use_spec) {
        const bool skip = spec_failed && opts->pc_type == 2;
        if (!skip) {
            rc = spec_solve(h, shift, r.b, xi, opts, &ls, r.bnorm2, ksfd_ctl::spec_gmres_cap(opts->pc_type, h->memo.spec_backoff), sg.n ? &sg : nullptr);
            st.pc_used |= 8;
        }
        if (skip || (rc == KSFD_ELINEAR && opts->pc_type == 2)) {
            if (!skip) st.linear_its += ls.its;
            spec_failed = true;
            const bool mg_here = ksfd_ctl::spec_fallback_mg(h->mg_ok, p.stiff);
            rc = gmres(h, h->u, shift, r.b, xi, opts, &ls, mg_here ? 1 : 0);
            st.pc_used |= mg_here ? 2 : 1;
        }
    } else if (p.use_pc && sg.n) {
        const double *xs[3]; double a[3];
        for (int j = 0; j < sg.n; j++) { xs[j] = sg.Y[j]; a[j] = sg.c[j]; }
        if ((rc = op_lincomb(h, sg.n, xs, a, xi)) || (rc = halo(h, xi)) || (rc = op_jvp_frozen(h, xi, 2, shift, h->Z, r.b))) return rc;
        const double tol = std::max(opts->ksp_rtol * sqrt(r.bnorm2), opts->ksp_atol);
        rc = p.dr_on ? gmres_dr(h, h->u, shift, h->Z, h->t3, opts, &ls, 1, i, tol)
                     : gmres(h, h->u, shift, h->Z, h->t3, opts, &ls, 1, i, tol);
        if (!rc) { const double *x2[2] = { xi, h->t3 }; double a2[2] = { 1.0, 1.0 }; rc = op_lincomb(h, 2, x2, a2, xi); }
        st.pc_used |= 2;
    } else {
        const int pc = p.use_pc ? 1 : (p.use_poly ? 2 : 0);
        rc = p.use_async ? gmres_async(h, shift, r.b, xi, opts, &ls)
             : p.dr_on ? gmres_dr(h, h->u, shift, r.b, xi, opts, &ls, pc, i)
                       : gmres(h, h->u, shift, r.b, xi, opts, &ls, pc, i);
        st.pc_used |= p.use_pc ? 2 : (p.use_poly ? 4 : 1);
    }
    st.linear_its += ls.its;
    st.ksp_resid = ls.rel;
    {
        static const bool stage_trace = getenv("KSFD_STAGE_TRACE") != nullptr;
        if (stage_trace) fprintf(stderr, "[stage %d] its %d rel %.2e guess %d\n", i, ls.its, ls.rel, sg.n);
    }
    if (rc == KSFD_ELINEAR && !p.direct && !p.use_pc && h->mg_ok && h->use_frozen && opts->pc_type) {
        rc = gmres(h, h->u, shift, r.b, xi, opts, &ls, 1);
        st.pc_used |= 2;
        st.linear_its += ls.its;
        st.ksp_resid = ls.rel;
    }
    return rc;
}

static int step_attempt(ksfd_handle *h, const ksfd_step_opts *opts, const AttemptPlan &p, bool &spec_failed, ksfd_step_stats &st)
{
    int rc = KSFD_OK;
    double gb[4][4];
    if (p.direct && !(rc = ensure_coef(h, true))) rc = p.banded ? banded_factor(h, p.shift) : direct_factor(h, p.shift);
    for (int i = 0; i < 4 && !rc; i++) {
        StageRhs r;
        SpecGuess sg;
        sg.n = 0;
        if ((rc = stage_rhs(h, p, i, r))) break;
        if (p.guess_on && (rc = stage_gram_guess(h, i, r, gb, sg))) break;
        rc = stage_solve(h, opts, p, i, r, sg, spec_failed, st);
    }
    return rc;
}

static int step_finish(ksfd_handle *h, const ksfd_step_opts *opts, double *wrms)
{
    int rc;
    {
        Scope sc(h, KC_FINISH, vbytes(h, 7));
        hipLaunchKernelGGL(k_rosw_finish, dim3(h->nblk_vec), dim3(KSFD_BLOCK), 0, h->st, h->kv, h->u, h->Y, h->vlen,
                           h->bt[0], h->bt[1], h->bt[2], h->bt[3], h->b2t[0] - h->bt[0], h->b2t[1] - h->bt[1],
                           h->b2t[2] - h->bt[2], h->b2t[3] - h->bt[3], opts->atol, opts->rtol, h->errv, h->part);
    }
    h->have_err = true;
    h->coef_fresh = false;
    if ((rc = reduce_rows(h, 1, h->nblk_vec, 0))) return rc;
    const double ntot = (double)h->G.F * (double)h->cfg.n[0] * (double)h->cfg.n[1] * (double)h->cfg.n[2];
    *wrms = sqrt(h->hres[0] / ntot);
    return KSFD_OK;
}
```

Baseline: 1.771 billion.

## Double-buffer state, skip redundant groom, lazy error field, reuse frozen G plane

The Rosenbrock finish now writes the new state into a second buffer and swaps pointers on accept. This replaces the usave copy, the restore copies and the extra halo exchanges on reject. It also counts points below the floor, so the next step can skip its clamp (groom) pass when nothing fell below. The error field is no longer written every step and is materialized lazily only when requested, and the fp32 coefficient copy is made on demand by a separate cast kernel. When the frozen Jacobian coefficients are fresh for u, the RHS kernel reuses the precomputed G plane instead of recomputing it, at the cost of more bookkeeping flags that must stay consistent.

```diff
diff --git a/ksfd_amd/csrc/handle.hip.h b/ksfd_amd/csrc/handle.hip.h
--- a/ksfd_amd/csrc/handle.hip.h
+++ b/ksfd_amd/csrc/handle.hip.h
@@ -131,6 +131,12 @@
     double *coef = nullptr;
     bool use_frozen = true;
     bool coef_fresh = false;
+    bool coef32_fresh = false;
+    bool floor_ok = false;
+    bool ckpt_floor_ok = false;
+    bool err_pending = false;
+    bool old_boundary = false;
+    bool rhs_gplane = true;
     double *flat = nullptr;
     double *src[4][KSFD_MAXL + 1];
     double *part = nullptr;
diff --git a/ksfd_amd/csrc/krylov.hip.h b/ksfd_amd/csrc/krylov.hip.h
--- a/ksfd_amd/csrc/krylov.hip.h
+++ b/ksfd_amd/csrc/krylov.hip.h
@@ -37,6 +37,7 @@
     int rc;
     const int d = h->poly_deg;
     const double *al = h->poly_alpha;
+    if ((rc = ensure_coef32(h))) return rc;
     if (h->poly_fp32 && h->coef32 && fused_ok(h)) {
         const float *C = h->coef32;
         float *tf[2] = { reinterpret_cast<float *>(h->t1), reinterpret_cast<float *>(h->t2) };
diff --git a/ksfd_amd/csrc/ksfd_hip.hip b/ksfd_amd/csrc/ksfd_hip.hip
--- a/ksfd_amd/csrc/ksfd_hip.hip
+++ b/ksfd_amd/csrc/ksfd_hip.hip
@@ -219,6 +219,7 @@
     h->cfg.lig_group = nullptr; h->cfg.lig_w = h->cfg.lig_s = h->cfg.lig_gamma = h->cfg.lig_D = nullptr;
     h->cfg.grp_alpha = h->cfg.grp_beta = nullptr;
     h->coef_fresh = false;
+    h->floor_ok = h->ckpt_floor_ok = false;
     return fill_phys(h, cfg);
 }
 
@@ -248,7 +249,7 @@
     return KSFD_OK;
 }
 extern "C" int64_t ksfd_local_size(const ksfd_handle *h) { return h ? (int64_t)h->G.F * h->G.nloc : 0; }
-extern "C" double *ksfd_device_state(ksfd_handle *h) { return h ? h->u : nullptr; }
+extern "C" double *ksfd_device_state(ksfd_handle *h) { if (h) h->floor_ok = false; return h ? h->u : nullptr; }
 extern "C" int64_t ksfd_device_plane_stride(const ksfd_handle *h) { return h ? h->G.plane : 0; }
 extern "C" int64_t ksfd_device_interior_offset(const ksfd_handle *h) { return h ? (int64_t)h->G.ng * h->G.inner : 0; }
 
@@ -258,6 +259,7 @@
     hipSetDevice(h->device);
     int rc = upload(h, u, layout, h->u);
     h->coef_fresh = false;
+    h->floor_ok = false;
     if (rc) return rc;
     HIPCHK(h, hipStreamSynchronize(h->st));
     return KSFD_OK;
@@ -315,6 +317,7 @@
         if (!h->ckpt && alloc_d(h, &h->ckpt, h->vlen)) return KSFD_ENOMEM;
         HIPCHK(h, hipMemcpyAsync(h->ckpt, h->u, sizeof(double) * (size_t)h->vlen, hipMemcpyDeviceToDevice, h->st));
         h->ckpt_memo = h->memo;
+        h->ckpt_floor_ok = h->floor_ok;
         for (MGLevel &L : h->mg) L.pv_norm = 0.0;
         h->ckpt_valid = true;
         return KSFD_OK;
@@ -322,9 +325,10 @@
     if (!h->ckpt_valid) return fail(h, KSFD_EINVAL, "no checkpoint has been saved");
     HIPCHK(h, hipMemcpyAsync(h->u, h->ckpt, sizeof(double) * (size_t)h->vlen, hipMemcpyDeviceToDevice, h->st));
     h->coef_fresh = false;
+    h->floor_ok = h->ckpt_floor_ok;
     h->memo = h->ckpt_memo;
     h->spec.means_valid = false;
-    h->mg_coef_valid = false; h->mg_shift = -1.0; h->poly_shift = -1.0; h->have_err = false;
+    h->mg_coef_valid = false; h->mg_shift = -1.0; h->poly_shift = -1.0; h->have_err = false; h->err_pending = false;
     for (MGLevel &L : h->mg) L.pv_norm = 0.0;
     rec_reset(h);
     return KSFD_OK;
@@ -341,6 +345,7 @@
     }
     double *dz = nullptr;
     h->coef_fresh = false;
+    h->floor_ok = false;
     if (hipMalloc((void **)&dz, sizeof(double) * (size_t)n) != hipSuccess) return fail(h, KSFD_ENOMEM, "hipMalloc of the coarse samples failed");
     hipError_t e = hipMemcpyAsync(dz, z, sizeof(double) * (size_t)n, hipMemcpyHostToDevice, h->st);
     const KGeom &G = h->G;
@@ -478,6 +483,7 @@
     Scope sc(h, KC_MISC, vbytes(h, 2));
     hipLaunchKernelGGL(k_groom, vgrid(h), dim3(KSFD_BLOCK), 0, h->st, h->kv, h->u, h->P.rhomin, h->P.Umin);
     HIPCHK(h, hipGetLastError());
+    h->floor_ok = true;
     return KSFD_OK;
 }
 
@@ -501,6 +507,7 @@
     if (!h) return KSFD_EINVAL;
     hipSetDevice(h->device);
     h->coef_fresh = false;
+    h->floor_ok = false;
     Scope sc(h, KC_MISC, 16.0 * (double)h->G.nloc);
     hipLaunchKernelGGL(k_mul_rho, dim3(h->nblk_vec), dim3(KSFD_BLOCK), 0, h->st, h->kv, h->u, (const double *)nullptr, factor);
     HIPCHK(h, hipGetLastError());
@@ -513,6 +520,7 @@
     hipSetDevice(h->device);
     HIPCHK(h, hipMemcpyAsync(h->flat, fh, sizeof(double) * (size_t)h->G.nloc, hipMemcpyHostToDevice, h->st));
     h->coef_fresh = false;
+    h->floor_ok = false;
     Scope sc(h, KC_MISC, 24.0 * (double)h->G.nloc);
     hipLaunchKernelGGL(k_mul_rho, dim3(h->nblk_vec), dim3(KSFD_BLOCK), 0, h->st, h->kv, h->u, (const double *)h->flat, 1.0);
     HIPCHK(h, hipGetLastError());
@@ -591,10 +599,11 @@
     int rejects = 0;
     const int max_rej = opts->max_reject < 0 ? 0x7fffffff : opts->max_reject;
     const bool single = (opts->reserved & 2) != 0;
-    {
-        Scope sc(h, KC_MISC, vbytes(h, 3));
-        hipLaunchKernelGGL(k_groom, vgrid(h), dim3(KSFD_BLOCK), 0, h->st, h->kv, h->u, h->P.rhomin, h->P.Umin, h->usave);
+    if (!h->floor_ok || h->old_boundary) {
+        Scope sc(h, KC_MISC, vbytes(h, 2));
+        hipLaunchKernelGGL(k_groom, vgrid(h), dim3(KSFD_BLOCK), 0, h->st, h->kv, h->u, h->P.rhomin, h->P.Umin);
         if (hipGetLastError() != hipSuccess) return fail(h, KSFD_EHIP, "k_groom launch failed");
+        h->floor_ok = true;
     }
     if ((rc = halo(h, h->u))) return rc;
     if (h->use_frozen && (rc = ensure_coef(h, true))) return rc;
@@ -606,6 +615,7 @@
         if ((rc = plan_attempt(h, opts, hh, direct, dr_on, lam_done, p))) return rc;
         const int its_before = st.linear_its;
         bool spec_failed = false;
+        if (h->err_pending) { h->err_pending = false; h->have_err = false; }
         rc = step_attempt(h, opts, p, spec_failed, st);
         const int its = st.linear_its - its_before;
         if (p.use_spec && opts->pc_type == 2) ksfd_ctl::spec_backoff_update(m, spec_failed, its, m.nsteps);
@@ -614,23 +624,24 @@
             rejects++;
             st.rejections = rejects;
             prev_accept = false;
-            if ((rc = op_copy(h, h->u, h->usave))) return rc;
             hh *= 0.25;
             *hstep = hh;
-            if ((rc = halo(h, h->u))) return rc;
             continue;
         }
-        if (rc) { op_copy(h, h->u, h->usave); hipStreamSynchronize(h->st); return rc; }
-        if ((rc = step_finish(h, opts, &st.wrms))) return rc;
+        if (rc) { hipStreamSynchronize(h->st); return rc; }
+        double below = 0.0;
+        if ((rc = step_finish(h, opts, &st.wrms, &below))) return rc;
         if (!(st.wrms == st.wrms) || isinf(st.wrms)) {
-            op_copy(h, h->u, h->usave); hipStreamSynchronize(h->st);
-            h->coef_fresh = h->use_frozen;
+            hipStreamSynchronize(h->st);
             return fail(h, KSFD_ENAN, "non-finite error norm at t=%g h=%g", *t, hh);
         }
         ksfd_ctl::AdaptChoice next = { true, hh };
         if (opts->adapt) next = ksfd_ctl::adapt_basic(hh, st.wrms, prev_accept, opts->safety, opts->reject_safety, opts->clip_lo, opts->clip_hi, opts->dt_min, opts->dt_max);
         prev_accept = next.accept;
         if (next.accept) {
+            std::swap(h->u, h->usave);
+            h->coef_fresh = false;
+            h->floor_ok = below == 0.0;
             st.accepted = 1; st.h_used = hh;
             *t += hh;
             *hstep = next.hnext;
@@ -638,13 +649,10 @@
         }
         rejects++;
         st.rejections = rejects;
-        if ((rc = op_copy(h, h->u, h->usave))) return rc;
-        h->coef_fresh = h->use_frozen;
         hh = next.hnext;
         *hstep = next.hnext;
         if (single) return KSFD_OK;
         if (rejects > max_rej) return fail(h, KSFD_EREJECT, "step rejected %d times at t=%g", rejects, *t);
-        if ((rc = halo(h, h->u))) return rc;
     }
 }
 
@@ -680,6 +688,8 @@
     if (!h || !eh) return KSFD_EINVAL;
     if (!h->have_err) return fail(h, KSFD_EINVAL, "no step has been attempted yet");
     hipSetDevice(h->device);
+    int rc = err_materialize(h);
+    if (rc) return rc;
     return download(h, h->errv, layout, eh);
 }
 
@@ -849,7 +859,7 @@
 static int mgp_begin(ksfd_handle *h, bool setup, double shift)
 {
     int rc;
-    if ((rc = ensure_coef(h))) return rc;
+    if ((rc = ensure_coef(h)) || (rc = ensure_coef32(h))) return rc;
     if (!h->mg_coef_valid && (rc = mg_restrict_coefs(h))) return rc;
     if (setup) {
         for (MGLevel &L : h->mg) L.pv_norm = 0.0;
@@ -1201,6 +1211,8 @@
         h->mg_fp32 = !(use_fused & 524288);
         h->rec_mg = (use_fused & 1048576) != 0;
         h->rhs_dots = !(use_fused & 2097152);
+        h->old_boundary = (use_fused & 4194304) != 0;
+        h->rhs_gplane = !(use_fused & 8388608);
         if (h->mg_fuse != !(use_fused & 4096)) { h->mg_fuse = !(use_fused & 4096); h->mg_shift = -1.0; if (h->mg_graph) { hipGraphExecDestroy(h->mg_graph); h->mg_graph = nullptr; } }
     }
     if (yseg > 0) h->yseg = yseg;
diff --git a/ksfd_amd/csrc/mg_host.hip.h b/ksfd_amd/csrc/mg_host.hip.h
--- a/ksfd_amd/csrc/mg_host.hip.h
+++ b/ksfd_amd/csrc/mg_host.hip.h
@@ -487,6 +487,7 @@
 static int mg_precond(ksfd_handle *h, double shift, const double *in, double *out)
 {
     int rc;
+    if ((rc = ensure_coef32(h))) return rc;
     if (!h->mg_coef_valid && (rc = mg_restrict_coefs(h))) return rc;
     if (h->mg_shift != shift && (rc = mg_setup_shift(h, shift))) return rc;
     MGVecs<float> &V = h->mg[0].v32;
diff --git a/ksfd_amd/csrc/ops.hip.h b/ksfd_amd/csrc/ops.hip.h
--- a/ksfd_amd/csrc/ops.hip.h
+++ b/ksfd_amd/csrc/ops.hip.h
@@ -240,9 +240,11 @@
         if (fused_norm && ndots > 0) { D.n = std::min(ndots, 2); D.stride = nwaves; for (int q = 0; q < D.n; q++) D.v[q] = dotv + (int64_t)q * h->vlen; }
         bool carry = h->rhs_carry && C.nout > 0 && C.nout == C.nin;
         for (int j = 0; j < C.nout && carry; j++) carry = C.yin[j] == C.yout[j];
+        const bool reuse_G = h->rhs_gplane && C.nin == 0 && C.nout == 0 && u == h->u && h->coef_fresh && h->use_frozen && h->coef && &PP == &h->P;
         auto launch = [&](const KStrips &Kx, double frac, double *np) -> int {
-            Scope sc(h, KC_RHS, vbytes(h, 2 + C.nin + (carry ? 0 : C.nout) + D.n) * frac, vbytes(h, 2 + C.nin + C.nout + D.n) * frac);
-            if (carry) { NL_DISPATCH(h->P.nlig, if constexpr (NL <= 4) hipLaunchKernelGGL((k_rhs2d_fused<NL, true>), dim3(Kx.nblocks), dim3(KSFD_BLOCK), 0, h->st, G, PP, Kx, u, S, out, C, np, D)); }
+            Scope sc(h, KC_RHS, (vbytes(h, 2 + C.nin + (carry ? 0 : C.nout) + D.n) + (reuse_G ? 8.0 * (double)G.nloc : 0.0)) * frac, vbytes(h, 2 + C.nin + C.nout + D.n) * frac);
+            if (reuse_G) { NL_DISPATCH(h->P.nlig, if constexpr (NL <= 4) hipLaunchKernelGGL((k_rhs2d_fused<NL, false, true>), dim3(Kx.nblocks), dim3(KSFD_BLOCK), 0, h->st, G, PP, Kx, u, S, out, C, np, D, (const double *)(h->coef + G.plane))); }
+            else if (carry) { NL_DISPATCH(h->P.nlig, if constexpr (NL <= 4) hipLaunchKernelGGL((k_rhs2d_fused<NL, true>), dim3(Kx.nblocks), dim3(KSFD_BLOCK), 0, h->st, G, PP, Kx, u, S, out, C, np, D)); }
             else { NL_DISPATCH(h->P.nlig, if constexpr (NL <= 4) hipLaunchKernelGGL((k_rhs2d_fused<NL>), dim3(Kx.nblocks), dim3(KSFD_BLOCK), 0, h->st, G, PP, Kx, u, S, out, C, np, D)); }
             return KSFD_OK;
         };
@@ -305,13 +307,20 @@
     return KSFD_OK;
 }
 
+static bool coef32_alloc(ksfd_handle *h)
+{
+    const KGeom &G = h->G;
+    if (!h->coef32 && h->poly_fp32 && fused_ok(h) && h->P.nlig <= 4 && G.plane % 2 == 0 && G.inner % 2 == 0 &&
+        hipMalloc((void **)&h->coef32, sizeof(float) * (size_t)(3 + h->P.nlig) * G.plane) != hipSuccess) { h->coef32 = nullptr; h->poly_fp32 = false; (void)hipGetLastError(); }
+    return h->poly_fp32 && h->coef32;
+}
+
 static int op_jcoef(ksfd_handle *h, const double *u, bool want_means = false)
 {
     const KGeom &G = h->G;
     const int nbp = plane_blocks(G);
-    if (!h->coef32 && h->poly_fp32 && fused_ok(h) && h->P.nlig <= 4 && G.plane % 2 == 0 && G.inner % 2 == 0 &&
-        hipMalloc((void **)&h->coef32, sizeof(float) * (size_t)(3 + h->P.nlig) * G.plane) != hipSuccess) { h->coef32 = nullptr; h->poly_fp32 = false; }
-    float *c32 = h->poly_fp32 ? h->coef32 : nullptr;
+    float *c32 = h->old_boundary && coef32_alloc(h) ? h->coef32 : nullptr;
+    h->coef32_fresh = c32 != nullptr;
     want_means = want_means && (long long)(1 + h->P.nlig) * nbp <= part_capacity();
     {
     Scope sc(h, KC_GFIELD, (8.0 * (G.F + 3 + h->P.nlig) + (c32 ? 4.0 * (3 + h->P.nlig) : 0.0)) * (double)G.plane);
@@ -337,6 +346,19 @@
     h->coef_fresh = true;
     h->mg_coef_valid = false; h->mg_shift = -1.0;
     h->spec.means_valid = h->spec.ok && (long long)(1 + h->P.nlig) * plane_blocks(h->G) <= part_capacity();
+    return KSFD_OK;
+}
+
+static int ensure_coef32(ksfd_handle *h)
+{
+    if (!coef32_alloc(h) || h->coef32_fresh) return KSFD_OK;
+    const long long n = (long long)(3 + h->P.nlig) * h->G.plane;
+    {
+        Scope sc(h, KC_GFIELD, 12.0 * (double)n);
+        hipLaunchKernelGGL(k_coef32, dim3(blocks_for(n / 2)), dim3(KSFD_BLOCK), 0, h->st, n, (const double *)h->coef, h->coef32);
+    }
+    HIPCHK(h, hipGetLastError());
+    h->coef32_fresh = true;
     return KSFD_OK;
 }
 
diff --git a/ksfd_amd/csrc/pointwise.hip.h b/ksfd_amd/csrc/pointwise.hip.h
--- a/ksfd_amd/csrc/pointwise.hip.h
+++ b/ksfd_amd/csrc/pointwise.hip.h
@@ -405,49 +405,71 @@
     }
 }
 
-__global__ void __launch_bounds__(KSFD_BLOCK) k_rosw_finish(KVec g, double *__restrict__ u,
+__device__ __forceinline__ double ksfd_rosw_err(double e0, double e1, double e2, double e3, double y0, double y1, double y2, double y3)
+{
+    return e0 * y0 + e1 * y1 + e2 * y2 + e3 * y3;
+}
+__global__ void __launch_bounds__(KSFD_BLOCK) k_rosw_finish(KVec g, const double *__restrict__ u, double *__restrict__ unew_out,
                                                             const double *__restrict__ Y, long long ystride,
                                                             double bt0, double bt1, double bt2, double bt3,
                                                             double e0, double e1, double e2, double e3,
-                                                            double atol, double rtol, double *__restrict__ errout,
-                                                            double *__restrict__ part)
-{
-    __shared__ double red[KSFD_BLOCK / KSFD_WAVE];
-    double acc = 0.0;
+                                                            double atol, double rtol, double rhomin, double Umin,
+                                                            double *__restrict__ errout, double *__restrict__ part)
+{
+    __shared__ double red[2][KSFD_BLOCK / KSFD_WAVE];
+    double acc = 0.0, below = 0.0;
     const long long stride = (long long)gridDim.x * blockDim.x;
     for (int c = 0; c < g.nf; c++) {
         const long long base = (long long)c * g.plane + g.off;
+        const double lo = c == 0 ? rhomin : Umin;
         for (long long p = (long long)blockIdx.x * blockDim.x + threadIdx.x; p < g.nloc; p += stride) {
             const double y0 = Y[base + p], y1 = Y[ystride + base + p], y2 = Y[2 * ystride + base + p],
                          y3 = Y[3 * ystride + base + p];
             const double un = u[base + p] + (bt0 * y0 + bt1 * y1 + bt2 * y2 + bt3 * y3);
-            const double er = e0 * y0 + e1 * y1 + e2 * y2 + e3 * y3;
+            const double er = ksfd_rosw_err(e0, e1, e2, e3, y0, y1, y2, y3);
             const double tol = atol + rtol * fmax(fabs(un), fabs(un + er));
             const double q = er / tol;
             acc += q * q;
-            u[base + p] = un;
+            below += (un >= lo) ? 0.0 : 1.0;
+            unew_out[base + p] = un;
             if (errout) errout[base + p] = er;
         }
     }
     acc = ksfd_wave_sum(acc);
-    if ((threadIdx.x & (KSFD_WAVE - 1)) == 0) red[threadIdx.x / KSFD_WAVE] = acc;
-    __syncthreads();
-    if (threadIdx.x == 0) {
+    below = ksfd_wave_sum(below);
+    if ((threadIdx.x & (KSFD_WAVE - 1)) == 0) { red[0][threadIdx.x / KSFD_WAVE] = acc; red[1][threadIdx.x / KSFD_WAVE] = below; }
+    __syncthreads();
+    if (threadIdx.x < 2) {
         double t = 0.0;
-        for (int q = 0; q < KSFD_BLOCK / KSFD_WAVE; q++) t += red[q];
-        part[blockIdx.x] = t;
-    }
-}
-
-__global__ void __launch_bounds__(KSFD_BLOCK) k_groom(KVec g, double *__restrict__ u, double rhomin, double Umin, double *__restrict__ copy = nullptr)
+        for (int q = 0; q < KSFD_BLOCK / KSFD_WAVE; q++) t += red[threadIdx.x][q];
+        part[(long long)threadIdx.x * gridDim.x + blockIdx.x] = t;
+    }
+}
+
+__global__ void __launch_bounds__(KSFD_BLOCK) k_rosw_error(KVec g, const double *__restrict__ Y, long long ystride,
+                                                           double e0, double e1, double e2, double e3, double *__restrict__ errout)
+{
+    const long long base = (long long)blockIdx.y * g.plane + g.off;
+    const long long stride = (long long)gridDim.x * blockDim.x;
+    for (long long p = (long long)blockIdx.x * blockDim.x + threadIdx.x; p < g.nloc; p += stride)
+        errout[base + p] = ksfd_rosw_err(e0, e1, e2, e3, Y[base + p], Y[ystride + base + p], Y[2 * ystride + base + p], Y[3 * ystride + base + p]);
+}
+
+__global__ void __launch_bounds__(KSFD_BLOCK) k_groom(KVec g, double *__restrict__ u, double rhomin, double Umin)
 {
     const long long base = (long long)blockIdx.y * g.plane + g.off;
     const double lo = blockIdx.y == 0 ? rhomin : Umin;
     const long long stride = (long long)gridDim.x * blockDim.x;
-    for (long long p = (long long)blockIdx.x * blockDim.x + threadIdx.x; p < g.nloc; p += stride) {
-        const double v = ksfd_clamp(u[base + p], lo);
-        u[base + p] = v;
-        if (copy) copy[base + p] = v;
+    for (long long p = (long long)blockIdx.x * blockDim.x + threadIdx.x; p < g.nloc; p += stride)
+        u[base + p] = ksfd_clamp(u[base + p], lo);
+}
+
+__global__ void __launch_bounds__(KSFD_BLOCK) k_coef32(long long n, const double *__restrict__ C, float *__restrict__ C32)
+{
+    const long long stride = (long long)gridDim.x * blockDim.x * 2;
+    for (long long e = ((long long)blockIdx.x * blockDim.x + threadIdx.x) * 2; e < n; e += stride) {
+        const double2 c = *reinterpret_cast<const double2 *>(C + e);
+        *reinterpret_cast<float2 *>(C32 + e) = make_float2((float)c.x, (float)c.y);
     }
 }
 
diff --git a/ksfd_amd/csrc/stencil.hip.h b/ksfd_amd/csrc/stencil.hip.h
--- a/ksfd_amd/csrc/stencil.hip.h
+++ b/ksfd_amd/csrc/stencil.hip.h
@@ -490,16 +490,18 @@
     return J;
 }
 
-template <int NL, bool CARRY = false>
+template <int NL, bool CARRY = false, bool GPLANE = false>
 __global__ void __launch_bounds__(KSFD_BLOCK) k_rhs2d_fused(KGeom G, KPhys P, KStrips S, const double *__restrict__ u,
                                                             KSrc src, double *__restrict__ out, KComb cmb = KComb{},
-                                                            double *__restrict__ normpart = nullptr, KDots dots = KDots{})
+                                                            double *__restrict__ normpart = nullptr, KDots dots = KDots{},
+                                                            const double *__restrict__ Gp = nullptr)
 {
     const KWaveJob J = ksfd_wave_job(G, S);
     if (!J.valid) return;
     double nacc = 0.0, dacc[2] = { 0.0, 0.0 };
     double rw[5][2], gw[5][2], uw[NL][5][2];
     double nr[2], nu[NL][2];
+    double ng[2];
     __shared__ double2 cring[CARRY ? KSFD_BLOCK / KSFD_WAVE : 1][CARRY ? 4 : 1][CARRY ? NL + 1 : 1][CARRY ? KSFD_WAVE : 1];
     const int cw = CARRY ? (threadIdx.x >> 6) : 0, cl = CARRY ? (threadIdx.x & (KSFD_WAVE - 1)) : 0;
     int nload = 0;
@@ -508,6 +510,7 @@
         const long long o = ksfd_rowoff(G, r) + J.c0;
         double2 t = ksfd_ld2(u + o);
         nr[0] = t.x; nr[1] = t.y;
+        if (GPLANE) { const double2 gq = ksfd_ld2(Gp + o); ng[0] = gq.x; ng[1] = gq.y; }
 #pragma unroll
         for (int l = 0; l < NL; l++) {
             double2 q = ksfd_ld2(u + (long long)(l + 1) * G.plane + o);
@@ -551,7 +554,8 @@
             double rho = ksfd_clamp(nr[e], P.rhomin);
 #pragma unroll
             for (int l = 0; l < NL; l++) { U[l] = ksfd_clamp(nu[l][e], P.Umin); uw[l][4][e] = U[l]; }
-            ksfd_G<NL, false>(P, rho, U, gw[4][e], gr, GU);
+            if (GPLANE) gw[4][e] = ng[e];
+            else ksfd_G<NL, false>(P, rho, U, gw[4][e], gr, GU);
             rw[4][e] = rho;
         }
     };
diff --git a/ksfd_amd/csrc/step.hip.h b/ksfd_amd/csrc/step.hip.h
--- a/ksfd_amd/csrc/step.hip.h
+++ b/ksfd_amd/csrc/step.hip.h
@@ -222,19 +222,34 @@
     return rc;
 }
 
-static int step_finish(ksfd_handle *h, const ksfd_step_opts *opts, double *wrms)
-{
-    int rc;
+static int err_materialize(ksfd_handle *h)
+{
+    if (!h->err_pending) return KSFD_OK;
     {
-        Scope sc(h, KC_FINISH, vbytes(h, 7));
-        hipLaunchKernelGGL(k_rosw_finish, dim3(h->nblk_vec), dim3(KSFD_BLOCK), 0, h->st, h->kv, h->u, h->Y, h->vlen,
+        Scope sc(h, KC_FINISH, vbytes(h, 5));
+        hipLaunchKernelGGL(k_rosw_error, vgrid(h), dim3(KSFD_BLOCK), 0, h->st, h->kv, (const double *)h->Y, h->vlen, h->b2t[0] - h->bt[0],
+                           h->b2t[1] - h->bt[1], h->b2t[2] - h->bt[2], h->b2t[3] - h->bt[3], h->errv);
+    }
+    HIPCHK(h, hipGetLastError());
+    h->err_pending = false;
+    return KSFD_OK;
+}
+
+static int step_finish(ksfd_handle *h, const ksfd_step_opts *opts, double *wrms, double *below)
+{
+    int rc;
+    {
+        Scope sc(h, KC_FINISH, vbytes(h, h->old_boundary ? 7 : 6));
+        hipLaunchKernelGGL(k_rosw_finish, dim3(h->nblk_vec), dim3(KSFD_BLOCK), 0, h->st, h->kv, (const double *)h->u, h->usave, h->Y, h->vlen,
                            h->bt[0], h->bt[1], h->bt[2], h->bt[3], h->b2t[0] - h->bt[0], h->b2t[1] - h->bt[1],
-                           h->b2t[2] - h->bt[2], h->b2t[3] - h->bt[3], opts->atol, opts->rtol, h->errv, h->part);
+                           h->b2t[2] - h->bt[2], h->b2t[3] - h->bt[3], opts->atol, opts->rtol, h->P.rhomin, h->P.Umin,
+                           h->old_boundary ? h->errv : (double *)nullptr, h->part);
     }
     h->have_err = true;
-    h->coef_fresh = false;
-    if ((rc = reduce_rows(h, 1, h->nblk_vec, 0))) return rc;
+    h->err_pending = !h->old_boundary;
+    if ((rc = reduce_rows(h, 2, h->nblk_vec, 0))) return rc;
     const double ntot = (double)h->G.F * (double)h->cfg.n[0] * (double)h->cfg.n[1] * (double)h->cfg.n[2];
     *wrms = sqrt(h->hres[0] / ntot);
-    return KSFD_OK;
-}
+    *below = h->hres[1];
+    return KSFD_OK;
+}
```

New measurement: 1.810 billion (median of 6 runs). 2.2% higher.
